# INK-USC/RE-Net

Measured on AMD Instinct MI355X. Metric: RGCN+GRU encoder triples/s at bs=1024 n_hidden=200 (full training step, both directions), higher is better.
Workload: dtype f32; 1 GPU; ICEWS18-shaped synthetic stream (seed 999), n_hidden=200, seq_len=10, batch=1024 per GPU, dropout=0.50, fwd+bwd both directions + clip + Adam; parallelism=dp1, global_batch=1024, nodes=99312, edges=288792

## Files before the change

### include/renet_hip.h

```cpp
#ifndef RENET_HIP_H
#define RENET_HIP_H

#include <stddef.h>
#include <stdint.h>

#ifdef __cplusplus
extern "C" {
#endif

#define RENET_OK 0
#define RENET_ERR_BADARG (-1)
#define RENET_ERR_UNSUPPORTED (-2)
#define RENET_ERR_WORKSPACE (-3)

#define RENET_ABI_VERSION 1
int renet_version(void);

int renet_gather_rows(const float* table, const int32_t* idx, int n, int D, float* out, void* stream);
int renet_segment_add(const float* src, const int32_t* order, const int32_t* seg_ptr,
                      const int32_t* seg_target, int U, int D, float* dst, void* stream);
int renet_segment_add2(const float* src0, const float* src1, const int32_t* order, const int32_t* seg_ptr,
                       const int32_t* seg_target, int U, int D, float* dst0, float* dst1, void* stream);

int renet_rgcn_gather(const float* x, int D, const int32_t* row_ptr, const int32_t* col,
                      const int32_t* etype, const float* scale, const float* W, int T, int type_shift,
                      int transpose_w, const float* addend, float drop_p, uint64_t seed, int relu,
                      float* out, int N, const int32_t* heavy_rows, int n_heavy, int heavy_thresh,
                      int src_limit, int addend_rows, void* stream);

int renet_rgcn_gather_items(const float* x, int D, const int32_t* it_src, const int32_t* it_type,
                            const int32_t* grp_ptr, int n_groups, const int32_t* row_ptr, const int32_t* col,
                            const int32_t* etype, const float* scale, const float* W, int T, int type_shift,
                            int transpose_w, const float* addend, float drop_p, uint64_t seed, int relu,
                            float* out, int N, const int32_t* heavy_rows, int n_heavy, int src_limit,
                            int addend_rows, int pruned, void* stream);

int renet_rgcn_gather_items_table(const float* table, int table_rows, int D, const int32_t* it_src_t,
                                  const int32_t* it_type_t, const int32_t* grp_ptr, int n_groups,
                                  const int32_t* row_ptr, const int32_t* col_t, const int32_t* etype,
                                  const int32_t* row_map, const float* scale, const float* W, int T, int type_shift,
                                  const float* addend_table, float drop_p, uint64_t seed, int relu, float* out, int N,
                                  const int32_t* heavy_rows, int n_heavy, void* stream);

int renet_rgcn_gather_items_bf16(const float* x, int D, const int32_t* it_src, const int32_t* it_type,
                                 const int32_t* grp_ptr, int n_groups, const int32_t* row_ptr, const int32_t* col,
                                 const int32_t* etype, const float* scale, const void* W_bf16, int w_ld, int T,
                                 int type_shift, int transpose_w, const float* addend, float drop_p, uint64_t seed,
                                 int relu, float* out, int N, const int32_t* heavy_rows, int n_heavy, int src_limit,
                                 int addend_rows, int pruned, void* stream);
int renet_rgcn_gather_items_table_bf16(const void* table_bf16, int table_ld, int table_rows, int D,
                                       const int32_t* it_src_t, const int32_t* it_type_t, const int32_t* grp_ptr,
                                       int n_groups, const int32_t* row_ptr, const int32_t* col_t, const int32_t* etype,
                                       const int32_t* row_map, const float* scale, const void* W_bf16, int w_ld, int T,
                                       int type_shift, const float* addend_table, float drop_p, uint64_t seed, int relu,
                                       float* out, int N, const int32_t* heavy_rows, int n_heavy, void* stream);
int renet_compose_table_items(const int32_t* row_map, const int32_t* it_src, const int32_t* it_type, int n_items,
                              const int32_t* col, const int32_t* e_src, int E, int32_t* it_src_t,
                              int32_t* it_type_t, int32_t* col_t, int32_t* e_src_t, void* stream);

int renet_rgcn_bwd_prep(const float* g_out, const float* out, const float* norm, int relu,
                        float drop_p, uint64_t seed, int N, int D, float* gn, float* g_loop,
                        void* stream);
int renet_rgcn_bwd_prep_bounds(const float* g_out, const float* out, const float* norm, int relu,
                               float drop_p, uint64_t seed, int N, int D, float* gn, float* g_loop,
                               float* bound_part, void* stream);

size_t renet_rgcn_bwd_w_workspace(int n_chunks, int D);
int renet_rgcn_bwd_w(const float* x, const float* gn, const int32_t* e_src, const int32_t* e_dst,
                     const int32_t* chunk_ptr, const int32_t* chunk_type, int n_chunks,
                     const int32_t* type_chunk_ptr, int T, int type_shift, int D, float* dW, float beta,
                     float* workspace, size_t workspace_bytes, void* stream);
int renet_rgcn_bwd_w64(const float* x, const float* gn, const int32_t* e_src, const int32_t* e_dst,
                       const int32_t* chunk_ptr, const int32_t* chunk_type, int n_chunks,
                       const int32_t* type_chunk_ptr, int T, int type_shift, int D, float* dW, float beta,
                       float* workspace, size_t workspace_bytes, void* stream);

size_t renet_gemm_workspace(int M, int N, int split_k);
int renet_gemm_f32(int ta, int tb, int M, int N, int K, float alpha, const float* A, int lda,
                   const float* B, int ldb, float beta, float* C, int ldc, const float* bias,
                   int split_k, float* workspace, size_t workspace_bytes, void* stream);

int renet_gemm_f32_split(int ta, int tb, int M, int N, int K, float alpha, const float* A, int lda,
                         const float* B, int ldb, float beta, float* C, int ldc, const float* bias,
                         int split_k, float* workspace, size_t workspace_bytes, void* stream);

int renet_gemm_split_plan(int ta, int tb, int M, int N, int K, const float* A, int lda, const float* B, int ldb,
                          int split_k, int* plan);

int renet_maxabs_blocks(int rows, int cols, int ld);
int renet_maxabs_partials(const float* x, int rows, int cols, int ld, float* part, void* stream);
int renet_maxabs_partials_multi(const void* jobs, int n_jobs, void* stream);
int renet_gemm_f32_h3(int ta, int tb, int M, int N, int K, float alpha, const float* A, int lda, const float* B,
                      int ldb, float beta, float* C, int ldc, const float* bias, int split_k, float* workspace,
                      size_t workspace_bytes, const float* maxA, int nA, const float* maxB, int nB, void* stream);

int renet_gemm_bf16(int ta, int tb, int M, int N, int K, float alpha, const float* A, int lda,
                    const float* B, int ldb, float beta, float* C, int ldc, const float* bias,
                    int split_k, float* workspace, size_t workspace_bytes, void* stream);

size_t renet_bf16_bytes(int R, int C);
int renet_pack_bf16(const float* X, int R, int C, int ldx, void* out, void* stream);
int renet_gemm_bf16s(int a_tr, int b_tr, int M, int N, int K, float alpha, const void* Ap, int lda, const void* Bp,
                     int ldb, float beta, float* C, int ldc, const float* bias, int split_k, float* workspace,
                     size_t workspace_bytes, void* stream);
int renet_bf16_zero_padding(void* P, int rows, int C, int ld, int rows_alloc, void* stream);
int renet_seq_assemble_fwd_bf16(const float* h2, const float* ent, const float* rel, const float* glob,
                                const int32_t* subj_row, const int32_t* row_ent, const int32_t* row_rel,
                                const int32_t* glob_row, int S, int D, float drop_p, uint64_t seed_x,
                                uint64_t seed_xr, void* X, int ldx, void* Xr, int ldxr, int rows_alloc,
                                void* stream);
int renet_softmax_ce_bf16(const float* logits, const int32_t* target, int B, int C, int ld, float grad_scale,
                          float* row_loss, void* dlogits_bf16, int ld16, int rows16, void* stream);
int renet_gru_bwd_layouts_bf16out(int n, const float* const* dh_last, const int32_t* const* step_off, const int* L,
                                  int H, const float* const* Whh, const float* const* saved, void* const* dGi16,
                                  void* const* dGh16, int out_ld, float* workspace, size_t workspace_bytes,
                                  void* stream);
int renet_colsum_bf16(const void* X, int M, int N, int ldx, float* out, float beta, float* workspace,
                      size_t workspace_bytes, void* stream);
int renet_scale_bf16_by_device_scalar(void* x, size_t n, const float* scale, void* stream);

size_t renet_planes_elems(int R, int C);
int renet_pack_planes(const float* X, int R, int C, int ldx, int ones_col, void* out, void* stream);
int renet_gemm_planes(int a_tr, int b_tr, int M, int N, int K, float alpha, const float* alpha_dev, const void* Ap,
                      int lda, size_t a_plane, const void* Bp, int ldb, size_t b_plane, float beta, float* C, int ldc,
                      const float* bias, float* col_out, int split_k, float* workspace, size_t workspace_bytes,
                      void* stream);
int renet_softmax_ce_planes(const float* logits, const int32_t* target, int B, int C, int ld, float grad_scale,
                            float* row_loss, void* dl_planes, size_t plane, int ld16, int rows16, void* stream);

size_t renet_colsum_workspace(int M, int N);
int renet_colsum(const float* X, int M, int N, int ldx, float* out, float beta, float* workspace,
                 size_t workspace_bytes, void* stream);

int renet_scale_by_device_scalar(float* x, size_t n, const float* scale, void* stream);
int renet_scale_by_device_scalar_bound(float* x, size_t n, const float* scale, float bound_in, float* bound_out,
                                       void* stream);

int renet_seq_assemble_fwd(const float* h2, const float* ent, const float* rel, const float* glob,
                           const int32_t* subj_row, const int32_t* row_ent, const int32_t* row_rel,
                           const int32_t* glob_row, int S, int D, float drop_p, uint64_t seed_x,
                           uint64_t seed_xr, float* X, float* Xr, void* stream);
int renet_bound_parts(size_t total4);
int renet_seq_assemble_fwd_bounds(const float* h2, const float* ent, const float* rel, const float* glob,
                                  const int32_t* subj_row, const int32_t* row_ent, const int32_t* row_rel,
                                  const int32_t* glob_row, int S, int D, float drop_p, uint64_t seed_x,
                                  uint64_t seed_xr, float* X, float* Xr, float* partX, float* partXr, void* stream);
int renet_seq_assemble_bwd(const float* dX, const float* dXr, const int32_t* step_off, int L, int S,
                           int B, int D, float drop_p, uint64_t seed_x, uint64_t seed_xr, float* dRows,
                           float* dEntSeq, float* dRelSeq, void* stream);

size_t renet_gru_workspace(int B, int H);
int renet_gru_fwd(const float* Gi, const int32_t* step_off, int L, int H, const float* Whh,
                  const float* bhh, float* h_last, int out_rows, float* saved, float* workspace,
                  size_t workspace_bytes, void* stream);
int renet_gru_bwd(const float* dh_last, const int32_t* step_off, int L, int H, const float* Whh,
                  const float* saved, float* dGi, float* dGh, float* workspace,
                  size_t workspace_bytes, void* stream);
int renet_gru_fwd_multi(int n, const float* const* Gi, const int32_t* step_off, int L, int H,
                        const float* const* Whh, const float* const* bhh, float* const* h_last, int out_rows,
                        float* const* saved, float* workspace, size_t workspace_bytes, void* stream);
int renet_gru_bwd_multi(int n, const float* const* dh_last, const int32_t* step_off, int L, int H,
                        const float* const* Whh, const float* const* saved, float* const* dGi,
                        float* const* dGh, float* workspace, size_t workspace_bytes, void* stream);
int renet_gru_fwd_layouts(int n, const float* const* Gi, const int32_t* const* step_off, const int* L, int H,
                          const float* const* Whh, const float* const* bhh, float* const* h_last,
                          const int* out_rows, float* const* saved, float* workspace, size_t workspace_bytes,
                          void* stream);
int renet_gru_bwd_layouts(int n, const float* const* dh_last, const int32_t* const* step_off, const int* L, int H,
                          const float* const* Whh, const float* const* saved, float* const* dGi,
                          float* const* dGh, float* workspace, size_t workspace_bytes, void* stream);
int renet_gru_bound_parts(int max_rows);
int renet_gru_bwd_layouts_bounds(int n, const float* const* dh_last, const int32_t* const* step_off, const int* L, int H,
                                 const float* const* Whh, const float* const* saved, float* const* dGi,
                                 float* const* dGh, float* const* bounds, float* workspace, size_t workspace_bytes,
                                 void* stream);
int renet_gru_fwd_layouts_f32(int n, const float* const* Gi, const int32_t* const* step_off, const int* L, int H,
                              const float* const* Whh, const float* const* bhh, float* const* h_last,
                              const int* out_rows, float* const* saved, float* workspace, size_t workspace_bytes,
                              void* stream);
int renet_gru_bwd_layouts_f32(int n, const float* const* dh_last, const int32_t* const* step_off, const int* L, int H,
                              const float* const* Whh, const float* const* saved, float* const* dGi,
                              float* const* dGh, float* workspace, size_t workspace_bytes, void* stream);
int renet_gru_fwd_layouts_bf16(int n, const float* const* Gi, const int32_t* const* step_off, const int* L, int H,
                               const float* const* Whh, const float* const* bhh, float* const* h_last,
                               const int* out_rows, float* const* saved, float* workspace, size_t workspace_bytes,
                               void* stream);
int renet_gru_bwd_layouts_bf16(int n, const float* const* dh_last, const int32_t* const* step_off, const int* L, int H,
                               const float* const* Whh, const float* const* saved, float* const* dGi,
                               float* const* dGh, float* workspace, size_t workspace_bytes, void* stream);

int renet_concat3_fwd(const float* a, const int32_t* ia, const float* hmid, const float* c,
                      const int32_t* ic, int B, int D, float drop_p, uint64_t seed, float* feat,
                      void* stream);
int renet_concat3_fwd_bounds(const float* a, const int32_t* ia, const float* hmid, const float* c,
                             const int32_t* ic, int B, int D, float drop_p, uint64_t seed, float* feat,
                             float* bound_part, void* stream);
int renet_concat3_bwd(const float* dfeat, int B, int D, int parts, float drop_p, uint64_t seed,
                      float* da_rows, float* dhmid, float* dc_rows, void* stream);
int renet_dropout(const float* x, size_t n, float drop_p, uint64_t seed, float* y, void* stream);
int renet_softmax_ce(const float* logits, const int32_t* target, int B, int C, int ld,
                     float grad_scale, float* row_loss, float* dlogits, void* stream);

int renet_segment_pool_fwd(const float* h, const int32_t* seg_ptr, int G, int D, int is_max,
                           float* out, int32_t* argmax, void* stream);
int renet_segment_pool_bwd(const float* dout, const int32_t* seg_ptr, const int32_t* argmax, int G,
                           int D, int is_max, int N, float* dh, void* stream);

int renet_nbr_pool_fwd(const float* E, const float* R, const float* P, const float* q, const float* v,
                       const int32_t* nbr, const int32_t* seg_ptr, const int32_t* seg_ptr_host, const int32_t* seg_s,
                       const int32_t* seg_r, const int32_t* seg_q, const int32_t* out_row, int S, int D, int attn,
                       float* out, float* stats, float* w, void* stream);
int renet_nbr_pool_bwd(const float* dOut, const float* out, const float* E, const float* P, const float* q,
                       const float* v, const float* w, const int32_t* nbr, const int32_t* seg_ptr,
                       const int32_t* seg_ptr_host, const int32_t* seg_q, const int32_t* out_row, int S, int D, int attn,
                       float* cE, float* cP, float* dq_rows, float* dv_rows, float* ds_rows, float* dr_rows,
                       void* stream);

size_t renet_adam_workspace(size_t n);
int renet_adam_step(float* p, float* g, float* m, float* v, size_t n, float lr, float beta1, float beta2,
                    float eps, float weight_decay, float max_norm, int step, int zero_grad, float* workspace,
                    size_t workspace_bytes, float* grad_norm_out, void* stream);
int renet_adam_step_scaled(float* p, float* g, float* m, float* v, size_t n, float lr, float beta1, float beta2,
                           float eps, float weight_decay, float max_norm, float grad_scale, int step,
                           int zero_grad, float* workspace, size_t workspace_bytes, float* grad_norm_out,
                           void* stream);

int renet_sumsq_partials(const float* g, size_t n, float* partial, int n_slots, void* stream);
int renet_adam_step_presummed(float* p, float* g, float* m, float* v, size_t n, float lr, float beta1, float beta2,
                              float eps, float weight_decay, float max_norm, float grad_scale, int step, int zero_grad,
                              const float* partial, int n_partial, float* grad_norm_out, void* stream);

int renet_joint_softmax(float* logits, int ld, int n, int R, int N, const float* logits_r, int ld_r,
                        const float* prob_e, void* stream);
size_t renet_topk_workspace(int n);
int renet_topk_positive(const float* x, size_t ldx, int n, int M, int k, float* out_val, int64_t* out_idx,
                        void* workspace, size_t workspace_bytes, void* stream);

int renet_rank_rows(const float* scores, int ld, int n, int C, const int32_t* label, const int32_t* filt_ptr,
                    const int32_t* filt_col, int filtered, int32_t* greater, int32_t* equal, float* row_loss,
                    void* stream);

int renet_rank_rows3(const float* scores, int ld, int n, int C, const int32_t* label, const int32_t* cols_a,
                     const int32_t* start_a, const int32_t* count_a, int len_a, const int32_t* cols_t,
                     const int32_t* start_t, const int32_t* count_t, int len_t, int32_t* counts, float* row_loss,
                     void* stream);

typedef struct {
    const int32_t *q_s, *q_r, *q_o;
    const int32_t* h_first[2];
    const int32_t* h_count[2];
    const int32_t* snap_t[2];
    const int32_t* snap_ptr[2];
    const int32_t* nbr_o[2];
    const int32_t* times;
    const int32_t* trip_ptr;
    const int32_t *trip_s, *trip_r, *trip_o;
    const int32_t* glob_times;
    int T, n_glob, n_facts, num_ent, num_rels;
} RenetStoreDev;

typedef struct {
    int32_t *node_ent, *node_slot, *row_ptr, *col, *etype;
    float* norm;
    int32_t *heavy_rows, *e_src, *e_dst, *chunk_ptr, *chunk_type, *type_chunk_ptr;
    int32_t *e_src2, *e_dst2, *chunk_ptr2, *chunk_type2, *type_chunk_ptr2;
    int32_t *it_src, *it_type, *grp_ptr;
    int32_t *subj_row, *row_seq, *row_ent, *row_rel, *glob_row;
    int32_t *s_sorted, *r_sorted, *rel_label, *ent_label, *perm, *step_off;
    int32_t* plan_order[4];
    int32_t* plan_seg[4];
    int32_t* plan_target[4];
    int32_t* counts;
    int cap_nodes, cap_edges;
    int32_t* seg_ptr;
} RenetBatchOut;

enum {
    RENET_BB_NNZ = 0, RENET_BB_S, RENET_BB_L, RENET_BB_TB, RENET_BB_FACTS, RENET_BB_N, RENET_BB_NA, RENET_BB_E2,
    RENET_BB_E, RENET_BB_NHEAVY, RENET_BB_NHEAVY_OUT, RENET_BB_NCHUNKS, RENET_BB_NCHUNKS2, RENET_BB_NITEMS,
    RENET_BB_NGROUPS, RENET_BB_NGROUPS_OUT, RENET_BB_NSEG0, RENET_BB_NSEG1, RENET_BB_NSEG2, RENET_BB_NSEG3,
    RENET_BB_ERR, RENET_BB_EOUT,
    RENET_BB_STEP_OFF = 24,
    RENET_BB_NCOUNTS = 64
};
enum { RENET_BB_ERR_TIME = 1, RENET_BB_ERR_GLOB = 2, RENET_BB_ERR_NODES = 4, RENET_BB_ERR_EDGES = 8 };

size_t renet_build_batch_workspace(const RenetStoreDev* store, int B, int cap_nodes, int cap_edges);
int renet_build_batch_both(const RenetStoreDev* store, const int32_t* idx_dev, int B, int seq_len, int heavy_thresh,
                           int group_budget, int chunk, const RenetBatchOut* out, void* workspace,
                           size_t workspace_bytes, void* stream);

typedef struct {
    const int32_t* node_ptr;
    const int32_t* node_ent_all;
    const int32_t* trip_ptr;
    const int32_t *trip_ls, *trip_r, *trip_lo;
    int T, n_nodes, n_facts, num_ent, num_rels;
} RenetFullStoreDev;

size_t renet_build_full_graphs_workspace(const RenetFullStoreDev* store, int G, int cap_nodes, int cap_edges);
int renet_build_full_graphs(const RenetFullStoreDev* store, const int32_t* tidx_dev, int G, int heavy_thresh,
                            int group_items, int chunk, RenetBatchOut* out, void* workspace, size_t workspace_bytes,
                            void* stream);

typedef struct {
    const int32_t *s, *r, *group;
    const int32_t *h_first, *h_count;
    const int32_t* step_t;
    const int32_t* nbr_ptr;
    const int32_t* nbr_o;
    const int32_t* times;
    const int32_t* trip_ptr;
    const int32_t *trip_s, *trip_r, *trip_o;
    const int32_t* glob_times;
    const int32_t *by_subj, *subj_sorted;
    int n_steps, n_nbr, T, n_glob, n_facts, num_ent, num_rels;
} RenetGroupedStoreDev;

size_t renet_build_batch_grouped_workspace(const RenetGroupedStoreDev* store, int B, int cap_nodes, int cap_edges);
int renet_build_batch_grouped(const RenetGroupedStoreDev* store, const int32_t* idx_dev, int B, int seq_len,
                              int heavy_thresh, int group_budget, int chunk, const RenetBatchOut* out, void* workspace,
                              size_t workspace_bytes, void* stream);

typedef struct { const int32_t *order, *seg_ptr, *target; int num_segments; } RenetSegPlan;
typedef struct {
    int D, num_ent, T, C2;
    float drop_p;
    const float *ent, *rel;
    const float *w1, *loop1, *w2, *loop2;
    const float *wih, *whh, *bih, *bhh;
    const float *wih_r, *whh_r, *bih_r, *bhh_r;
    const float *lin_w, *lin_b;
    const float *linr_w, *linr_b;
    float *g_ent, *g_rel, *g_w1, *g_loop1, *g_w2, *g_loop2, *g_wih, *g_whh, *g_bih, *g_bhh, *g_wih_r, *g_whh_r, *g_bih_r,
          *g_bhh_r, *g_lin_w, *g_lin_b, *g_linr_w, *g_linr_b;
    const float* glob;
    const void* lin_w_planes;
    size_t lin_w_plane;
    int lin_w_ld;
} RenetStepModel;
typedef struct {
    int N, E, nA, S, B, L, n_items;
    int n_groups, n_groups_out, n_heavy, n_heavy_out, n_chunks, n_chunks2;
    const int32_t* step_off_host;
    const int32_t *node_ent, *row_ptr, *col, *etype;
    const float* norm;
    const int32_t *it_src, *it_type, *grp_ptr, *heavy_rows, *heavy_rows_out;
    const int32_t *it_src_t, *it_type_t, *col_t, *e_src_t;
    const int32_t *e_src, *e_dst, *chunk_ptr, *chunk_type, *type_chunk_ptr;
    const int32_t *e_src2, *e_dst2, *chunk_ptr2, *chunk_type2, *type_chunk_ptr2;
    const int32_t *subj_row, *row_ent, *row_rel, *glob_row, *step_off;
    const int32_t *s_idx, *r_idx, *ent_label, *rel_label;
    RenetSegPlan plan_node_ent, plan_subj_row, plan_s, plan_r;
} RenetStepBatch;
typedef struct {
    uint64_t seed_rgcn1, seed_rgcn2, seed_x, seed_xr, seed_head1, seed_head2;
    float scale_ent, scale_rel;
    void* workspace;
    size_t workspace_bytes;
    void *stream, *side_stream;
} RenetStepRun;
size_t renet_step_workspace(const RenetStepModel* m, const RenetStepBatch* b);
int renet_step_forward(const RenetStepModel* m, const RenetStepBatch* b, const RenetStepRun* r, float* row_loss,
                       int* n_launches);
int renet_step_backward(const RenetStepModel* m, const RenetStepBatch* b, const RenetStepRun* r, const float* g,
                        int defer_side, void* ev_head_done, void* ev_gru_done, int* n_launches);
int renet_add_inplace(float* x, const float* y, size_t n, void* stream);
int renet_zero(float* x, size_t n, void* stream);

int64_t renet_host_filter_edges(const int64_t* trip_ptr, const int64_t* trip_s, const int64_t* trip_r,
                                const int64_t* trip_o, const int64_t* ti, int64_t Tb, int64_t num_ent,
                                const int64_t* keys, const int32_t* new_id, int64_t N, int32_t* table,
                                int64_t* out_ls, int64_t* out_lo, int64_t* out_rr);
int64_t renet_host_filter_edges_sparse(const int64_t* trip_ptr, const int64_t* trip_s, const int64_t* trip_r,
                                       const int64_t* trip_o, const int64_t* by_subj,
                                       const int64_t* subj_sorted, const int64_t* ti, int64_t Tb,
                                       int64_t num_ent, const int64_t* keys, const int32_t* new_id, int64_t N,
                                       int32_t* table, int64_t* out_ls, int64_t* out_lo, int64_t* out_rr);
int64_t renet_host_type_chunks(int64_t E, const int64_t* src, const int64_t* dst, const int64_t* et, int64_t T,
                               int64_t chunk, int64_t n_out, int32_t* e_src, int32_t* e_dst,
                               int32_t* type_chunk_ptr, int32_t* chunk_type, int32_t* chunk_ptr,
                               int64_t* n_chunks);
int64_t renet_host_node_sets(int64_t S, const int64_t* slot_k, const int64_t* subj_ent, const int64_t* nbr_begin,
                             const int64_t* nbr_cnt, const int64_t* nbr_o, int64_t Tb, int64_t num_ent,
                             int32_t* table, int64_t* keys, int64_t* subj_pos, int64_t* new_id,
                             int32_t* node_ent, int64_t* node_slot, int64_t* n_a);
void renet_host_edge_layouts(int64_t n, int64_t E, const int64_t* src, const int64_t* dst, const int64_t* et,
                             int64_t T, int64_t chunk, int64_t heavy, int32_t* col, int32_t* etype,
                             int32_t* row_ptr, float* norm, int32_t* heavy_rows, int64_t* n_heavy,
                             int32_t* e_src, int32_t* e_dst, int32_t* type_chunk_ptr, int32_t* chunk_type,
                             int32_t* chunk_ptr, int64_t* n_chunks);
int64_t renet_host_segplan(const int64_t* idx, int64_t n, int64_t bound, int32_t* order, int32_t* seg_ptr,
                           int32_t* target);
int64_t renet_host_gather_items(int64_t N, const int32_t* row_ptr, const int32_t* col, const int32_t* etype,
                                int64_t heavy, int64_t budget, int64_t n_out, int32_t* it_src, int32_t* it_type,
                                int32_t* grp_ptr, int64_t* n_items, int64_t* n_groups_out);

#ifdef __cplusplus
}
#endif
#endif
```

### re-net_amd/csrc/gru.hip

```cpp
#include "gru_common.h"

namespace {

bool use_f32() {
    static const bool v = renet_env_is("RENET_GEMM", "f32");
    return v;
}

bool use_persistent() { return !renet_env_is("RENET_GRU", "steps"); }

bool fill_offsets(const int32_t* step_off, int L, StepOff& so, int& B) {
    if (L < 1 || L > MAXL || !step_off) return false;
    for (int j = 0; j <= L; ++j) so.off[j] = step_off[j];
    for (int j = L + 1; j <= MAXL; ++j) so.off[j] = step_off[L];
    B = step_off[1] - step_off[0];
    for (int j = 1; j < L; ++j)
        if (step_off[j + 1] - step_off[j] > step_off[j] - step_off[j - 1]) return false;
    return B >= 0;
}

inline size_t align256(size_t x) { return (x + 255) & ~(size_t)255; }
inline int nub(int H) { return (H + 15) / 16; }
inline size_t fwd_plane_bytes(int H) { return (size_t)nub(H) * ((H + 31) / 32) * 9 * 1024; }
inline size_t bwd_t_bytes(int H) { return align256((size_t)3 * H * H * sizeof(float)); }
inline size_t bwd_plane_bytes(int H) { return (size_t)nub(H) * ((3 * H + 31) / 32) * 3 * 1024; }

size_t slice_bytes(int B, int H) {
    size_t m = fwd_plane_bytes(H);
    if (bwd_t_bytes(H) > m) m = bwd_t_bytes(H);
    if (bwd_plane_bytes(H) > m) m = bwd_plane_bytes(H);
    m = align256(m);
    if (B > 0) {
        const size_t rp = (size_t)rows_pad_of(B);
        m += align256((size_t)2 * 3 * rp * kp_of(3 * H) * sizeof(__bf16)) + align256(rp * H * sizeof(float));
    }
    return m;
}

int make_layouts(int n, const int32_t* const* step_off, const int* Ls, const int* rows_in, bool fwd, Layouts& ly,
                 int* B_of) {
    if (n < 1 || n > MAXP) return RENET_ERR_BADARG;
    const int32_t* seen[MAXLAY] = {nullptr, nullptr};
    int nl = 0;
    for (int i = 0; i < MAXLAY; ++i) {
        ly.L[i] = 0; ly.rows[i] = 0;
        for (int j = 0; j <= MAXL; ++j) ly.so[i].off[j] = 0;
    }
    for (int k = 0; k < MAXP; ++k) ly.lay_of[k] = 0;
    static const int rot_mod = renet_env_int("RENET_GRU_ROT", 0, 0, 0x7fffffff);
    ly.rot_mod = rot_mod;
    for (int k = 0; k < n; ++k) {
        int l = -1;
        for (int i = 0; i < nl; ++i)
            if (seen[i] == step_off[k] && ly.L[i] == Ls[k]) l = i;
        if (l < 0) {
            if (nl == MAXLAY) return RENET_ERR_BADARG;
            l = nl++;
            seen[l] = step_off[k];
            ly.L[l] = Ls[k];
            int B = 0;
            if (Ls[k] > 0 && !fill_offsets(step_off[k], Ls[k], ly.so[l], B)) return RENET_ERR_BADARG;
            ly.rows[l] = fwd ? 0 : B;
        }
        const int B = ly.L[l] > 0 ? ly.so[l].off[1] - ly.so[l].off[0] : 0;
        if (fwd) {
            if (rows_in[k] < B) return RENET_ERR_BADARG;
            if (ly.rows[l] != 0 && ly.rows[l] != rows_in[k]) return RENET_ERR_BADARG;
            ly.rows[l] = rows_in[k];
        }
        ly.lay_of[k] = l;
        B_of[k] = B;
    }
    return RENET_OK;
}

StepState carve_state(char* slice, int H, int Bmax, size_t kp) {
    StepState t;
    const size_t rp = (size_t)rows_pad_of(Bmax);
    char* base = slice + align256(slice_bytes(0, H));
    t.plane_stride = rp * kp;
    t.A[0] = reinterpret_cast<__bf16*>(base);
    t.A[1] = t.A[0] + 3 * t.plane_stride;
    t.dh = reinterpret_cast<float*>(base + align256((size_t)2 * 3 * rp * kp_of(3 * H) * sizeof(__bf16)));
    return t;
}

int plane_slot(int k, const float* const* W) {
    for (int i = 0; i < k; ++i)
        if (W[i] == W[k]) return i;
    return k;
}

int max_batch(int n, const int* B_of) {
    int Bmax = 0;
    for (int k = 0; k < n; ++k) Bmax = B_of[k] > Bmax ? B_of[k] : Bmax;
    return Bmax;
}

int gru_fwd_impl(int npl, int n, const float* const* Gi, const int32_t* const* step_off, const int* L, int H,
                 const float* const* Whh, const float* const* bhh, float* const* h_last, const int* out_rows,
                 float* const* saved, float* workspace, size_t workspace_bytes, void* stream) {
    Layouts ly;
    int B_of[MAXP];
    const int e0 = make_layouts(n, step_off, L, out_rows, true, ly, B_of);
    if (e0 != RENET_OK) return e0;
    if (max_rows(ly) == 0) return RENET_OK;
    if (!renet_dim_ok(H) || (npl == 1 && H == 300)) return RENET_ERR_UNSUPPORTED;
    hipStream_t st = (hipStream_t)stream;
    if (npl == 0 || (use_f32() && npl == 3)) {
        FwdProbs ps;
        for (int i = 0; i < MAXP; ++i) {
            const int k = i < n ? i : 0;
            ps.p[i] = {Gi[k], Whh[k], bhh[k], h_last[k], saved[k]};
        }
        return renet_gru_f32_fwd(H, &ps, n, &ly, st);
    }
    const bool steps = npl == 3 && !use_persistent();
    const int Bmax = max_batch(n, B_of);
    const size_t per = slice_bytes(steps ? Bmax : 0, H);
    if (!workspace || workspace_bytes < (size_t)n * per) return RENET_ERR_WORKSPACE;
    char* ws = reinterpret_cast<char*>(workspace);
    FwdProbsB ps;
    for (int i = 0; i < MAXP; ++i) {
        const int k = i < n ? i : 0;
        const int slot = plane_slot(k, Whh);
        bf16x8* planes = reinterpret_cast<bf16x8*>(ws + (size_t)slot * per);
        if (i < n && slot == k) {
            const int e = renet_gru_split_frag(Whh[k], H, H, 3, (size_t)H * H, (size_t)H, 1, planes, st, npl);
            if (e != RENET_OK) return e;
        }
        ps.p[i] = {Gi[k], planes, bhh[k], h_last[k], saved[k]};
    }
    if (steps) {
        StepState stt[MAXP];
        for (int i = 0; i < n; ++i) stt[i] = carve_state(ws + (size_t)i * per, H, Bmax, kp_of(H));
        return renet_gru_steps_fwd(H, n, &ps, &ly, stt, Bmax, st);
    }
    return renet_gru_planes_fwd(H, npl, &ps, n, &ly, st);
}

int gru_bwd_impl(int npl, int n, const float* const* dh_last, const int32_t* const* step_off, const int* L, int H,
                 const float* const* Whh, const float* const* saved, float* const* dGi, float* const* dGh,
                 float* workspace, size_t workspace_bytes, void* stream, int out_ld = 0,
                 float* const* bounds = nullptr) {
    Layouts ly;
    int B_of[MAXP];
    const int e0 = make_layouts(n, step_off, L, nullptr, false, ly, B_of);
    if (e0 != RENET_OK) return e0;
    if (max_rows(ly) == 0) return RENET_OK;
    if (!renet_dim_ok(H) || (npl == 1 && H == 300)) return RENET_ERR_UNSUPPORTED;
    hipStream_t st = (hipStream_t)stream;
    const bool f32 = npl == 0 || (use_f32() && npl == 3);
    const bool steps = npl == 3 && !f32 && !use_persistent();
    if (bounds && (f32 || steps || npl != 3)) return RENET_ERR_UNSUPPORTED;
    const int Bmax = max_batch(n, B_of);
    const size_t per = slice_bytes(steps ? Bmax : 0, H);
    if (!workspace || workspace_bytes < (size_t)n * per) return RENET_ERR_WORKSPACE;
    char* ws = reinterpret_cast<char*>(workspace);
    char* wt[MAXP];
    for (int i = 0; i < MAXP; ++i) {
        const int k = i < n ? i : 0;
        const int slot = plane_slot(k, Whh);
        wt[i] = ws + (size_t)slot * per;
        if (i < n && slot == k) {
            const int e = f32 ? renet_gru_transpose(Whh[k], 3 * H, H, reinterpret_cast<float*>(wt[i]), st)
                              : renet_gru_split_frag(Whh[k], H, 3 * H, 1, 0, 1, (size_t)H, wt[i], st, npl);
            if (e != RENET_OK) return e;
        }
    }
    if (f32) {
        BwdProbs ps;
        for (int i = 0; i < MAXP; ++i) {
            const int k = i < n ? i : 0;
            ps.p[i] = {dh_last[k], reinterpret_cast<float*>(wt[i]), saved[k], dGi[k], dGh[k]};
        }
        return renet_gru_f32_bwd(H, &ps, n, &ly, st);
    }
    BwdProbsB pb;
    for (int i = 0; i < MAXP; ++i) {
        const int k = i < n ? i : 0;
        pb.p[i] = {dh_last[k], reinterpret_cast<bf16x8*>(wt[i]), saved[k], dGi[k], dGh[k], out_ld, bounds ? bounds[k] : nullptr};
    }
    if (steps) {
        StepState stt[MAXP];
        for (int i = 0; i < n; ++i) stt[i] = carve_state(ws + (size_t)i * per, H, Bmax, kp_of(3 * H));
        return renet_gru_steps_bwd(H, n, &pb, &ly, stt, B_of, Bmax, st);
    }
    return renet_gru_planes_bwd(H, npl, out_ld > 0, &pb, n, &ly, st);
}

}

extern "C" {

size_t renet_gru_workspace(int B, int H) { return slice_bytes(B, H); }

#define GRU_FWD_PARAMS                                                                                                \
    int n, const float* const* Gi, const int32_t* const* step_off, const int* L, int H, const float* const* Whh,      \
    const float* const* bhh, float* const* h_last, const int* out_rows, float* const* saved, float* workspace,        \
    size_t workspace_bytes, void* stream
#define GRU_FWD_ARGS n, Gi, step_off, L, H, Whh, bhh, h_last, out_rows, saved, workspace, workspace_bytes, stream
int renet_gru_fwd_layouts(GRU_FWD_PARAMS) { return gru_fwd_impl(3, GRU_FWD_ARGS); }
int renet_gru_fwd_layouts_f32(GRU_FWD_PARAMS) { return gru_fwd_impl(0, GRU_FWD_ARGS); }
int renet_gru_fwd_layouts_bf16(GRU_FWD_PARAMS) { return gru_fwd_impl(1, GRU_FWD_ARGS); }

#define GRU_BWD_PARAMS                                                                                                \
    int n, const float* const* dh_last, const int32_t* const* step_off, const int* L, int H, const float* const* Whh, \
    const float* const* saved, float* const* dGi, float* const* dGh, float* workspace, size_t workspace_bytes,        \
    void* stream
#define GRU_BWD_ARGS n, dh_last, step_off, L, H, Whh, saved, dGi, dGh, workspace, workspace_bytes, stream
int renet_gru_bwd_layouts(GRU_BWD_PARAMS) { return gru_bwd_impl(3, GRU_BWD_ARGS); }
int renet_gru_bwd_layouts_f32(GRU_BWD_PARAMS) { return gru_bwd_impl(0, GRU_BWD_ARGS); }
int renet_gru_bwd_layouts_bf16(GRU_BWD_PARAMS) { return gru_bwd_impl(1, GRU_BWD_ARGS); }

int renet_gru_bound_parts(int max_rows) { return max(1, (max_rows + MT - 1) / MT); }

int renet_gru_bwd_layouts_bounds(int n, const float* const* dh_last, const int32_t* const* step_off, const int* L, int H,
                                 const float* const* Whh, const float* const* saved, float* const* dGi,
                                 float* const* dGh, float* const* bounds, float* workspace, size_t workspace_bytes,
                                 void* stream) {
    if (!bounds) return RENET_ERR_BADARG;
    return gru_bwd_impl(3, n, dh_last, step_off, L, H, Whh, saved, dGi, dGh, workspace, workspace_bytes, stream, 0,
                        bounds);
}

int renet_gru_bwd_layouts_bf16out(int n, const float* const* dh_last, const int32_t* const* step_off, const int* L,
                                  int H, const float* const* Whh, const float* const* saved, void* const* dGi16,
                                  void* const* dGh16, int out_ld, float* workspace, size_t workspace_bytes,
                                  void* stream) {
    if (out_ld < 3 * H) return RENET_ERR_BADARG;
    return gru_bwd_impl(1, n, dh_last, step_off, L, H, Whh, saved, reinterpret_cast<float* const*>(dGi16),
                        reinterpret_cast<float* const*>(dGh16), workspace, workspace_bytes, stream, out_ld);
}

int renet_gru_fwd_multi(int n, const float* const* Gi, const int32_t* step_off, int L, int H,
                        const float* const* Whh, const float* const* bhh, float* const* h_last, int out_rows,
                        float* const* saved, float* workspace, size_t workspace_bytes, void* stream) {
    if (n < 1 || n > MAXP) return RENET_ERR_BADARG;
    const int32_t* so[MAXP];
    int Ls[MAXP], rows[MAXP];
    for (int k = 0; k < n; ++k) { so[k] = step_off; Ls[k] = L; rows[k] = out_rows; }
    return renet_gru_fwd_layouts(n, Gi, so, Ls, H, Whh, bhh, h_last, rows, saved, workspace, workspace_bytes, stream);
}

int renet_gru_fwd(const float* Gi, const int32_t* step_off, int L, int H, const float* Whh,
                  const float* bhh, float* h_last, int out_rows, float* saved, float* workspace,
                  size_t workspace_bytes, void* stream) {
    return renet_gru_fwd_multi(1, &Gi, step_off, L, H, &Whh, &bhh, &h_last, out_rows, &saved, workspace,
                               workspace_bytes, stream);
}

int renet_gru_bwd_multi(int n, const float* const* dh_last, const int32_t* step_off, int L, int H,
                        const float* const* Whh, const float* const* saved, float* const* dGi,
                        float* const* dGh, float* workspace, size_t workspace_bytes, void* stream) {
    if (n < 1 || n > MAXP) return RENET_ERR_BADARG;
    const int32_t* so[MAXP];
    int Ls[MAXP];
    for (int k = 0; k < n; ++k) { so[k] = step_off; Ls[k] = L; }
    return renet_gru_bwd_layouts(n, dh_last, so, Ls, H, Whh, saved, dGi, dGh, workspace, workspace_bytes, stream);
}

int renet_gru_bwd(const float* dh_last, const int32_t* step_off, int L, int H, const float* Whh,
                  const float* saved, float* dGi, float* dGh, float* workspace,
                  size_t workspace_bytes, void* stream) {
    return renet_gru_bwd_multi(1, &dh_last, step_off, L, H, &Whh, &saved, &dGi, &dGh, workspace,
                               workspace_bytes, stream);
}

}
```

### re-net_amd/csrc/step.cpp

```cpp
#include <hip/hip_runtime.h>
#include <algorithm>
#include <cstdint>
#include <cstdlib>
#include <vector>
#include "../../include/renet_hip.h"

namespace {

int auto_split_k(int m, int n, int k) {
    const long tiles = (long)((m + 127) / 128) * ((n + 127) / 128);
    const int ktiles = (k + 31) / 32;
    if (tiles >= 256 || ktiles < 8) return 1;
    const int smax = std::max(1, std::min(128, ktiles / 4));
    const double per_slice = (double)m * (double)n * 2.7e-6;
    int best = 1;
    double best_t = -1.0;
    for (int s = 1; s <= smax; ++s) {
        const long rounds = (tiles * s + 511) / 512;
        const double t = (double)rounds * ((double)ktiles / (double)s + 6.0) + (s > 1 ? per_slice * s : 0.0);
        if (best_t < 0.0 || t < best_t - 1e-9) { best = s; best_t = t; }
    }
    return best;
}

int auto_split_k_planes(int m, int n, int k) {
    const long tiles = (long)((m + 255) / 256) * ((n + 127) / 128);
    const int ktiles = (k + 31) / 32;
    if (tiles >= 128 || ktiles < 8) return 1;
    const int smax = std::max(1, std::min(64, ktiles / 4));
    const double per_slice = (double)m * (double)n * 2.7e-6;
    int best = 1;
    double best_t = -1.0;
    for (int s = 1; s <= smax; ++s) {
        const long rounds = (tiles * s + 255) / 256;
        const double t = (double)rounds * ((double)ktiles / (double)s + 6.0) + (s > 1 ? per_slice * s : 0.0);
        if (best_t < 0.0 || t < best_t - 1e-9) { best = s; best_t = t; }
    }
    return best;
}

inline size_t up(size_t x) { return (x + 255) & ~(size_t)255; }
inline size_t fbytes(size_t rows, size_t cols) { return up(rows * cols * sizeof(float)); }

struct Lay {
    size_t out1, out2, X, Xr, sv0, sv1, feat1, feat2, dl1, dl2, featp1;
    size_t ew, gi0, gi1, hs0, hs1, logits, featp;
    size_t dfeat1, dfeat2, da1, da2, dh1, dh2, dc1, dgi0, dgi1, dgh0, dgh1, dX, dXr, d_rows, d_ent_seq, d_rel_seq, d_h2, gn2,
        gl2, dhN, gn1, gl1, dh1N, gs;
    size_t gru_ws, gemm_ws_main, gemm_ws_side, bwdw_ws, colsum_ws;
    size_t gru_ws_bytes, gemm_ws_bytes, bwdw_ws_bytes, colsum_ws_bytes;
    size_t dl_plane, dl_ld, dl_rows, featp_plane, featp_ld, featp1_plane, featp1_ld, logits_ld;
    size_t total;
};

bool use_planes(const RenetStepModel& m) { return m.lin_w_planes != nullptr; }

Lay layout(const RenetStepModel& m, const RenetStepBatch& b) {
    Lay L{};
    size_t o = 0;
    auto take = [&](size_t bytes) { const size_t at = o; o += up(bytes); return at; };
    const size_t D = m.D, N = b.N, nA = b.nA, S = b.S, B = b.B, NE = m.num_ent, C2 = m.C2;
    const bool pl = use_planes(m);
    L.out1 = take(fbytes(N, D));
    L.out2 = take(fbytes(nA, D));
    L.X = take(fbytes(S, 4 * D));
    L.Xr = take(fbytes(S, 3 * D));
    L.sv0 = take(fbytes(S, 5 * D));
    L.sv1 = take(fbytes(S, 5 * D));
    L.feat1 = take(fbytes(B, 3 * D));
    L.feat2 = take(fbytes(B, 2 * D));
    L.dl2 = take(fbytes(B, C2));
    if (pl) {
        L.dl_rows = (B + 255) & ~(size_t)255;
        L.dl_ld = (NE + 255) & ~(size_t)255;
        L.dl_plane = L.dl_rows * L.dl_ld;
        L.dl1 = take(3 * L.dl_plane * 2);
        L.featp_ld = (3 * D + 255) & ~(size_t)255;
        L.featp_plane = L.dl_rows * L.featp_ld;
        L.featp1_ld = (3 * D + 1 + 255) & ~(size_t)255;
        L.featp1_plane = L.dl_rows * L.featp1_ld;
        L.featp1 = take(3 * L.featp1_plane * 2);
        L.logits_ld = (NE + 3) & ~(size_t)3;
        L.logits = take(fbytes(B, L.logits_ld));
    } else {
        L.dl1 = take(fbytes(B, NE));
        L.logits_ld = NE;
    }
    L.ew = take(fbytes(NE, D));
    L.gi0 = take(fbytes(S, 3 * D));
    L.gi1 = take(fbytes(S, 3 * D));
    L.hs0 = take(fbytes(B, D));
    L.hs1 = take(fbytes(B, D));
    L.dfeat1 = take(fbytes(B, 3 * D));
    L.dfeat2 = take(fbytes(B, 2 * D));
    L.da1 = take(fbytes(B, D));
    L.da2 = take(fbytes(B, D));
    L.dh1 = take(fbytes(B, D));
    L.dh2 = take(fbytes(B, D));
    L.dc1 = take(fbytes(B, D));
    L.dgi0 = take(fbytes(S, 3 * D));
    L.dgi1 = take(fbytes(S, 3 * D));
    L.dgh0 = take(fbytes(S, 3 * D));
    L.dgh1 = take(fbytes(S, 3 * D));
    L.dX = take(fbytes(S, 4 * D));
    L.dXr = take(fbytes(S, 3 * D));
    L.d_rows = take(fbytes(S, D));
    L.d_ent_seq = take(fbytes(B, D));
    L.d_rel_seq = take(fbytes(B, D));
    L.d_h2 = take(fbytes(nA, D));
    L.gn2 = take(fbytes(nA, D));
    L.gl2 = take(fbytes(nA, D));
    L.dhN = take(fbytes(N, D));
    L.gn1 = take(fbytes(N, D));
    L.gl1 = take(fbytes(N, D));
    L.dh1N = take(fbytes(N, D));
    L.gs = take(fbytes(NE, D));
    const int bmax = b.L > 0 ? b.step_off_host[1] - b.step_off_host[0] : 0;
    L.gru_ws_bytes = 2 * renet_gru_workspace(bmax, m.D);
    L.gru_ws = take(std::max<size_t>(L.gru_ws_bytes, 4));
    size_t need = 4;
    auto g_ = [&](int mm, int nn, int kk) { need = std::max(need, renet_gemm_workspace(mm, nn, auto_split_k(mm, nn, kk))); };
    const int Di = m.D, Si = b.S, Bi = b.B, NEi = m.num_ent, nAi = b.nA, C2i = m.C2;
    g_(NEi, Di, Di); g_(nAi, Di, Di); g_(Si, 3 * Di, 4 * Di); g_(Si, 3 * Di, 3 * Di); g_(Bi, NEi, 3 * Di); g_(Bi, C2i, 2 * Di);
    g_(Bi, 3 * Di, NEi); g_(NEi, 3 * Di, Bi); g_(Bi, 2 * Di, C2i); g_(C2i, 2 * Di, Bi);
    g_(3 * Di, 4 * Di, Si); g_(3 * Di, 3 * Di, Si); g_(3 * Di, Di, Si); g_(Si, 3 * Di, 3 * Di); g_(Si, 2 * Di, 3 * Di);
    g_(Di, Di, nAi); g_(Di, Di, NEi);
    if (pl) {
        need = std::max(need, renet_gemm_workspace(Bi, 3 * Di, auto_split_k_planes(Bi, 3 * Di, NEi)));
        need = std::max(need, renet_gemm_workspace(NEi, 3 * Di + 1, auto_split_k_planes(NEi, 3 * Di + 1, Bi)));
        need = std::max(need, renet_gemm_workspace(Bi, NEi, auto_split_k_planes(Bi, NEi, 3 * Di)));
    }
    L.gemm_ws_bytes = need;
    L.gemm_ws_main = take(need);
    L.gemm_ws_side = take(need);
    L.bwdw_ws_bytes = std::max<size_t>(renet_rgcn_bwd_w_workspace(std::max(b.n_chunks, b.n_chunks2), m.D), 4);
    L.bwdw_ws = take(L.bwdw_ws_bytes);
    size_t cs = 4;
    cs = std::max(cs, renet_colsum_workspace(Bi, NEi));
    cs = std::max(cs, renet_colsum_workspace(Bi, C2i));
    cs = std::max(cs, renet_colsum_workspace(Si, 3 * Di));
    L.colsum_ws_bytes = cs;
    L.colsum_ws = take(cs);
    L.total = o;
    return L;
}

bool args_ok(const RenetStepModel* m, const RenetStepBatch* b) {
    if (!m || !b) return false;
    if (!(m->D == 100 || m->D == 200 || m->D == 300 || m->D == 400) || m->num_ent < 1 || m->T < 2 || m->C2 < 1) return false;
    if (b->N < 1 || b->nA < 1 || b->nA > b->N || b->S < 1 || b->B < 1 || b->L < 1 || !b->step_off_host) return false;
    const size_t big = (size_t)std::max(b->N, m->num_ent) * m->D * 4;
    return big < ((size_t)1 << 31);
}

hipEvent_t step_event(int i) {
    thread_local std::vector<hipEvent_t> ev;
    while ((int)ev.size() <= i) {
        hipEvent_t e = nullptr;
        if (hipEventCreateWithFlags(&e, hipEventDisableTiming) != hipSuccess) return nullptr;
        ev.push_back(e);
    }
    return ev[i];
}

struct Streams {
    hipStream_t main, side;
    int next_ev = 0, rc = 0;
    bool two() const { return side != main; }
    void order(hipStream_t first, hipStream_t then) {
        if (!two() || rc) return;
        hipEvent_t e = step_event(next_ev++ & 7);
        if (!e) { rc = (int)hipErrorOutOfMemory; return; }
        hipError_t x = hipEventRecord(e, first);
        if (x == hipSuccess) x = hipStreamWaitEvent(then, e, 0);
        if (x != hipSuccess) rc = (int)x;
    }
    void fork() { order(main, side); }
    void join() { order(side, main); }
};

#define CK(call)                      \
    do {                              \
        const int rc__ = (call);      \
        ++launches;                   \
        if (rc__ != 0) return rc__;   \
    } while (0)

int gemm(hipStream_t st, float* ws, size_t ws_bytes, int ta, int tb, int M, int N, int K, const float* A, int lda, const float* B,
         int ldb, float beta, float* C, int ldc, const float* bias) {
    const int sk = auto_split_k(M, N, K);
    return renet_gemm_f32_split(ta, tb, M, N, K, 1.f, A, lda, B, ldb, beta, C, ldc, bias, sk, sk > 1 ? ws : nullptr,
                                sk > 1 ? ws_bytes : 0, st);
}

}

extern "C" {

size_t renet_step_workspace(const RenetStepModel* m, const RenetStepBatch* b) {
    if (!args_ok(m, b)) return 0;
    return layout(*m, *b).total;
}

int renet_step_forward(const RenetStepModel* mp, const RenetStepBatch* bp, const RenetStepRun* r, float* row_loss,
                       int* n_launches) {
    if (!args_ok(mp, bp) || !r || !r->workspace || !row_loss) return RENET_ERR_BADARG;
    const RenetStepModel& m = *mp;
    const RenetStepBatch& b = *bp;
    const Lay L = layout(m, b);
    if (r->workspace_bytes < L.total) return RENET_ERR_WORKSPACE;
    char* W = (char*)r->workspace;
    auto F = [&](size_t off) { return (float*)(W + off); };
    Streams s{(hipStream_t)r->stream, (hipStream_t)(r->side_stream ? r->side_stream : r->stream)};
    int launches = 0;
    const int D = m.D, N = b.N, nA = b.nA, S = b.S, B = b.B, NE = m.num_ent, T = m.T;
    const float p = m.drop_p;
    const bool pruned = nA < N;
    float* wsm = F(L.gemm_ws_main);
    float* wss = F(L.gemm_ws_side);

    CK(gemm(s.main, wsm, L.gemm_ws_bytes, 0, 0, NE, D, D, m.ent, D, m.loop1, D, 0.f, F(L.ew), D, nullptr));
    CK(renet_rgcn_gather_items_table(m.ent, NE, D, b.it_src_t, b.it_type_t, b.grp_ptr, b.n_groups, b.row_ptr, b.col_t, b.etype,
                                     b.node_ent, b.norm, m.w1, T, 0, F(L.ew), p, r->seed_rgcn1, 1, F(L.out1), N,
                                     b.n_heavy ? b.heavy_rows : nullptr, b.n_heavy, s.main));
    CK(gemm(s.main, wsm, L.gemm_ws_bytes, 0, 0, nA, D, D, F(L.out1), D, m.loop2, D, 0.f, F(L.out2), D, nullptr));
    CK(renet_rgcn_gather_items(F(L.out1), D, b.it_src, b.it_type, b.grp_ptr, pruned ? b.n_groups_out : b.n_groups, b.row_ptr,
                               b.col, b.etype, b.norm, m.w2, T, 0, 0, F(L.out2), p, r->seed_rgcn2, 0, F(L.out2), nA,
                               pruned ? (b.n_heavy_out ? b.heavy_rows_out : nullptr) : (b.n_heavy ? b.heavy_rows : nullptr),
                               pruned ? b.n_heavy_out : b.n_heavy, 0, 0, pruned ? 1 : 0, s.main));
    CK(renet_seq_assemble_fwd(F(L.out2), m.ent, m.rel, m.glob, b.subj_row, b.row_ent, b.row_rel, b.glob_row, S, D, p, r->seed_x,
                              r->seed_xr, F(L.X), F(L.Xr), s.main));
    s.fork();
    CK(gemm(s.side, wss, L.gemm_ws_bytes, 0, 1, S, 3 * D, 3 * D, F(L.Xr), 3 * D, m.wih_r, 3 * D, 0.f, F(L.gi1), 3 * D, m.bih_r));
    CK(gemm(s.main, wsm, L.gemm_ws_bytes, 0, 1, S, 3 * D, 4 * D, F(L.X), 4 * D, m.wih, 4 * D, 0.f, F(L.gi0), 3 * D, m.bih));
    s.join();
    {
        const float* gi[2] = {F(L.gi0), F(L.gi1)};
        const int32_t* so[2] = {b.step_off_host, b.step_off_host};
        const int ls[2] = {b.L, b.L};
        const float* whh[2] = {m.whh, m.whh_r};
        const float* bhh[2] = {m.bhh, m.bhh_r};
        float* hl[2] = {F(L.hs0), F(L.hs1)};
        const int bmax = b.step_off_host[1] - b.step_off_host[0];
        const int rows[2] = {std::max(B, bmax), std::max(B, bmax)};
        float* sv[2] = {F(L.sv0), F(L.sv1)};
        if (rows[0] != B) return RENET_ERR_BADARG;
        CK(renet_gru_fwd_layouts(2, gi, so, ls, D, whh, bhh, hl, rows, sv, F(L.gru_ws), L.gru_ws_bytes, s.main));
    }
    s.fork();
    CK(renet_concat3_fwd(m.ent, b.s_idx, F(L.hs1), nullptr, nullptr, B, D, p, r->seed_head2, F(L.feat2), s.side));
    CK(gemm(s.side, wss, L.gemm_ws_bytes, 0, 1, B, m.C2, 2 * D, F(L.feat2), 2 * D, m.linr_w, 2 * D, 0.f, F(L.dl2), m.C2, m.linr_b));
    CK(renet_softmax_ce(F(L.dl2), b.rel_label, B, m.C2, m.C2, r->scale_rel, row_loss + B, F(L.dl2), s.side));
    CK(renet_concat3_fwd(m.ent, b.s_idx, F(L.hs0), m.rel, b.r_idx, B, D, p, r->seed_head1, F(L.feat1), s.main));
    if (use_planes(m)) {
        CK(renet_pack_planes(F(L.feat1), B, 3 * D, 3 * D, 1, W + L.featp1, s.main));
        const int sk = auto_split_k_planes(B, NE, 3 * D);
        CK(renet_gemm_planes(0, 0, B, NE, 3 * D, 1.f, nullptr, W + L.featp1, (int)L.featp1_ld, L.featp1_plane, m.lin_w_planes,
                             m.lin_w_ld, m.lin_w_plane, 0.f, F(L.logits), (int)L.logits_ld, m.lin_b, nullptr, sk,
                             sk > 1 ? wsm : nullptr, sk > 1 ? L.gemm_ws_bytes : 0, s.main));
        CK(renet_softmax_ce_planes(F(L.logits), b.ent_label, B, NE, (int)L.logits_ld, r->scale_ent, row_loss, W + L.dl1, L.dl_plane,
                                   (int)L.dl_ld, (int)L.dl_rows, s.main));
    } else {
        CK(gemm(s.main, wsm, L.gemm_ws_bytes, 0, 1, B, NE, 3 * D, F(L.feat1), 3 * D, m.lin_w, 3 * D, 0.f, F(L.dl1), NE, m.lin_b));
        CK(renet_softmax_ce(F(L.dl1), b.ent_label, B, NE, NE, r->scale_ent, row_loss, F(L.dl1), s.main));
    }
    s.join();
    if (n_launches) *n_launches = launches;
    return s.rc;
}

int renet_step_backward(const RenetStepModel* mp, const RenetStepBatch* bp, const RenetStepRun* r, const float* g,
                        int defer_side, void* ev_head_done, void* ev_gru_done, int* n_launches) {
    if (!args_ok(mp, bp) || !r || !r->workspace || !g) return RENET_ERR_BADARG;
    const RenetStepModel& m = *mp;
    const RenetStepBatch& b = *bp;
    const Lay L = layout(m, b);
    if (r->workspace_bytes < L.total) return RENET_ERR_WORKSPACE;
    char* W = (char*)r->workspace;
    auto F = [&](size_t off) { return (float*)(W + off); };
    Streams s{(hipStream_t)r->stream, (hipStream_t)(r->side_stream ? r->side_stream : r->stream)};
    int launches = 0;
    const int D = m.D, N = b.N, nA = b.nA, S = b.S, B = b.B, NE = m.num_ent, T = m.T, C2 = m.C2;
    const float p = m.drop_p;
    const bool pruned = nA < N;
    const bool pl = use_planes(m);
    float* wsm = F(L.gemm_ws_main);
    float* wss = F(L.gemm_ws_side);
    float* csw = L.colsum_ws_bytes > 4 ? F(L.colsum_ws) : nullptr;
    auto colsum = [&](const float* X, int M_, int N_, float* out, hipStream_t st) {
        const size_t need = renet_colsum_workspace(M_, N_);
        return renet_colsum(X, M_, N_, N_, out, 1.f, need ? csw : nullptr, need, st);
    };

    if (!pl) CK(renet_scale_by_device_scalar(F(L.dl1), (size_t)B * NE, g, s.main));
    s.fork();
    CK(renet_scale_by_device_scalar(F(L.dl2), (size_t)B * C2, g, s.side));
    CK(gemm(s.side, wss, L.gemm_ws_bytes, 0, 0, B, 2 * D, C2, F(L.dl2), C2, m.linr_w, 2 * D, 0.f, F(L.dfeat2), 2 * D, nullptr));
    CK(gemm(s.side, wss, L.gemm_ws_bytes, 1, 0, C2, 2 * D, B, F(L.dl2), C2, F(L.feat2), 2 * D, 1.f, m.g_linr_w, 2 * D, nullptr));
    CK(colsum(F(L.dl2), B, C2, m.g_linr_b, s.side));
    CK(renet_concat3_bwd(F(L.dfeat2), B, D, 2, p, r->seed_head2, F(L.da2), F(L.dh2), nullptr, s.side));
    if (pl) {
        const int sk1 = auto_split_k_planes(B, 3 * D, NE);
        CK(renet_gemm_planes(0, 1, B, 3 * D, NE, 1.f, g, W + L.dl1, (int)L.dl_ld, L.dl_plane, m.lin_w_planes, m.lin_w_ld,
                             m.lin_w_plane, 0.f, F(L.dfeat1), 3 * D, nullptr, nullptr, sk1, sk1 > 1 ? wsm : nullptr,
                             sk1 > 1 ? L.gemm_ws_bytes : 0, s.main));
        const int sk2 = auto_split_k_planes(NE, 3 * D + 1, B);
        CK(renet_gemm_planes(1, 1, NE, 3 * D + 1, B, 1.f, g, W + L.dl1, (int)L.dl_ld, L.dl_plane, W + L.featp1, (int)L.featp1_ld,
                             L.featp1_plane, 1.f, m.g_lin_w, 3 * D, nullptr, m.g_lin_b, sk2, sk2 > 1 ? wsm : nullptr,
                             sk2 > 1 ? L.gemm_ws_bytes : 0, s.main));
    } else {
        CK(colsum(F(L.dl1), B, NE, m.g_lin_b, s.side));
        CK(gemm(s.main, wsm, L.gemm_ws_bytes, 0, 0, B, 3 * D, NE, F(L.dl1), NE, m.lin_w, 3 * D, 0.f, F(L.dfeat1), 3 * D, nullptr));
        CK(gemm(s.main, wsm, L.gemm_ws_bytes, 1, 0, NE, 3 * D, B, F(L.dl1), NE, F(L.feat1), 3 * D, 1.f, m.g_lin_w, 3 * D, nullptr));
    }
    CK(renet_concat3_bwd(F(L.dfeat1), B, D, 3, p, r->seed_head1, F(L.da1), F(L.dh1), F(L.dc1), s.main));
    s.join();
    if (ev_head_done) {
        const hipError_t e = hipEventRecord((hipEvent_t)ev_head_done, s.main);
        if (e != hipSuccess) return (int)e;
    }
    CK(renet_add_inplace(F(L.da1), F(L.da2), (size_t)B * D, s.main));
    CK(renet_segment_add(F(L.da1), b.plan_s.order, b.plan_s.seg_ptr, b.plan_s.target, b.plan_s.num_segments, D, m.g_ent, s.main));
    CK(renet_segment_add(F(L.dc1), b.plan_r.order, b.plan_r.seg_ptr, b.plan_r.target, b.plan_r.num_segments, D, m.g_rel, s.main));

    {
        const float* dhl[2] = {F(L.dh1), F(L.dh2)};
        const int32_t* so[2] = {b.step_off_host, b.step_off_host};
        const int ls[2] = {b.L, b.L};
        const float* whh[2] = {m.whh, m.whh_r};
        const float* sv[2] = {F(L.sv0), F(L.sv1)};
        float* dgi[2] = {F(L.dgi0), F(L.dgi1)};
        float* dgh[2] = {F(L.dgh0), F(L.dgh1)};
        CK(renet_gru_bwd_layouts(2, dhl, so, ls, D, whh, sv, dgi, dgh, F(L.gru_ws), L.gru_ws_bytes, s.main));
    }
    auto gru_param_grads = [&]() -> int {
        const float* xs[2] = {F(L.X), F(L.Xr)};
        const int in[2] = {4 * D, 3 * D};
        const size_t dgi[2] = {L.dgi0, L.dgi1}, dgh[2] = {L.dgh0, L.dgh1}, sv[2] = {L.sv0, L.sv1};
        float* gwih[2] = {m.g_wih, m.g_wih_r};
        float* gwhh[2] = {m.g_whh, m.g_whh_r};
        float* gbih[2] = {m.g_bih, m.g_bih_r};
        float* gbhh[2] = {m.g_bhh, m.g_bhh_r};
        for (int k = 0; k < 2; ++k) {
            CK(gemm(s.side, wss, L.gemm_ws_bytes, 1, 0, 3 * D, in[k], S, F(dgi[k]), 3 * D, xs[k], in[k], 1.f, gwih[k], in[k], nullptr));
            CK(gemm(s.side, wss, L.gemm_ws_bytes, 1, 0, 3 * D, D, S, F(dgh[k]), 3 * D, F(sv[k]) + 4 * D, 5 * D, 1.f, gwhh[k], D, nullptr));
            CK(colsum(F(dgi[k]), S, 3 * D, gbih[k], s.side));
            CK(colsum(F(dgh[k]), S, 3 * D, gbhh[k], s.side));
        }
        return 0;
    };
    auto gru_done = [&]() -> int {
        if (!ev_gru_done) return 0;
        return (int)hipEventRecord((hipEvent_t)ev_gru_done, s.side);
    };
    {
        s.fork();
        int rc_ = gru_param_grads();
        if (!rc_) rc_ = gru_done();
        if (rc_) return rc_;
    }
    CK(gemm(s.main, wsm, L.gemm_ws_bytes, 0, 0, S, 3 * D, 3 * D, F(L.dgi0), 3 * D, m.wih, 4 * D, 0.f, F(L.dX), 4 * D, nullptr));
    CK(gemm(s.main, wsm, L.gemm_ws_bytes, 0, 0, S, 2 * D, 3 * D, F(L.dgi1), 3 * D, m.wih_r, 3 * D, 0.f, F(L.dXr), 3 * D, nullptr));

    CK(renet_seq_assemble_bwd(F(L.dX), F(L.dXr), b.step_off, b.L, S, B, D, p, r->seed_x, r->seed_xr, F(L.d_rows), F(L.d_ent_seq),
                              F(L.d_rel_seq), s.main));
    CK(renet_zero(F(L.d_h2), (size_t)nA * D, s.main));
    CK(renet_segment_add(F(L.d_rows), b.plan_subj_row.order, b.plan_subj_row.seg_ptr, b.plan_subj_row.target,
                         b.plan_subj_row.num_segments, D, F(L.d_h2), s.main));
    CK(renet_segment_add(F(L.d_ent_seq), b.plan_s.order, b.plan_s.seg_ptr, b.plan_s.target, b.plan_s.num_segments, D, m.g_ent, s.main));
    CK(renet_segment_add(F(L.d_rel_seq), b.plan_r.order, b.plan_r.seg_ptr, b.plan_r.target, b.plan_r.num_segments, D, m.g_rel, s.main));

    const int pair_shift = (T / 2) % T;
    CK(renet_rgcn_bwd_prep(F(L.d_h2), F(L.out2), b.norm, 0, p, r->seed_rgcn2, nA, D, F(L.gn2), F(L.gl2), s.main));
    CK(renet_rgcn_gather_items(F(L.gn2), D, b.it_src, b.it_type, b.grp_ptr, b.n_groups, b.row_ptr, b.col, b.etype, nullptr, m.w2, T,
                               pair_shift, 1, nullptr, 0.f, 0, 0, F(L.dhN), N, b.n_heavy ? b.heavy_rows : nullptr, b.n_heavy,
                               pruned ? nA : 0, 0, pruned ? 1 : 0, s.main));
    CK(gemm(s.main, wsm, L.gemm_ws_bytes, 0, 1, nA, D, D, F(L.gl2), D, m.loop2, D, 1.f, F(L.dhN), D, nullptr));
    s.fork();
    if (pruned)
        CK(renet_rgcn_bwd_w(F(L.out1), F(L.gn2), b.e_src2, b.e_dst2, b.chunk_ptr2, b.chunk_type2, b.n_chunks2, b.type_chunk_ptr2, T,
                            0, D, m.g_w2, 1.f, F(L.bwdw_ws), renet_rgcn_bwd_w_workspace(b.n_chunks2, D), s.side));
    else
        CK(renet_rgcn_bwd_w(F(L.out1), F(L.gn2), b.e_src, b.e_dst, b.chunk_ptr, b.chunk_type, b.n_chunks, b.type_chunk_ptr, T, 0, D,
                            m.g_w2, 1.f, F(L.bwdw_ws), renet_rgcn_bwd_w_workspace(b.n_chunks, D), s.side));
    CK(gemm(s.side, wss, L.gemm_ws_bytes, 1, 0, D, D, nA, F(L.out1), D, F(L.gl2), D, 1.f, m.g_loop2, D, nullptr));

    CK(renet_rgcn_bwd_prep(F(L.dhN), F(L.out1), b.norm, 1, p, r->seed_rgcn1, N, D, F(L.gn1), F(L.gl1), s.main));
    CK(renet_rgcn_gather_items(F(L.gn1), D, b.it_src, b.it_type, b.grp_ptr, b.n_groups, b.row_ptr, b.col, b.etype, nullptr, m.w1, T,
                               pair_shift, 1, nullptr, 0.f, 0, 0, F(L.dh1N), N, b.n_heavy ? b.heavy_rows : nullptr, b.n_heavy, 0, 0,
                               0, s.main));
    s.fork();
    CK(renet_rgcn_bwd_w(m.ent, F(L.gn1), b.e_src_t, b.e_dst, b.chunk_ptr, b.chunk_type, b.n_chunks, b.type_chunk_ptr, T, 0, D,
                        m.g_w1, 1.f, F(L.bwdw_ws), renet_rgcn_bwd_w_workspace(b.n_chunks, D), s.side));
    CK(renet_zero(F(L.gs), (size_t)NE * D, s.main));
    CK(renet_segment_add2(F(L.dh1N), F(L.gl1), b.plan_node_ent.order, b.plan_node_ent.seg_ptr, b.plan_node_ent.target,
                          b.plan_node_ent.num_segments, D, m.g_ent, F(L.gs), s.main));
    CK(gemm(s.main, wsm, L.gemm_ws_bytes, 0, 1, NE, D, D, F(L.gs), D, m.loop1, D, 1.f, m.g_ent, D, nullptr));
    CK(gemm(s.main, wsm, L.gemm_ws_bytes, 1, 0, D, D, NE, m.ent, D, F(L.gs), D, 1.f, m.g_loop1, D, nullptr));
    if (!defer_side) s.join();
    if (n_launches) *n_launches = launches;
    return s.rc;
}

}
```

### re-net_amd/pipeline.py

```python
import multiprocessing as mp
import os

_job = {}


def worker_budget(world=1, cpus=None, cap=24):
    cpus = cpus or os.cpu_count() or 2
    return max(1, min(int(cap), cpus // (2 * max(int(world), 1))))


def _run(step):
    return _job['fn'](step)


class BatchPrefetcher(object):

    def __init__(self, fn, steps, num_workers=None, chunksize=1, threads=False):
        self.fn, self.steps = fn, list(steps)
        self.num_workers = num_workers or max(1, min(32, (os.cpu_count() or 2) // 2))
        self.chunksize = chunksize
        self.threads = threads
        self.pool = None

    def _iter_threads(self):
        from concurrent.futures import ThreadPoolExecutor
        ahead = 2 * self.num_workers
        with ThreadPoolExecutor(self.num_workers) as ex:
            pending = []
            it = iter(self.steps)
            for s in it:
                pending.append(ex.submit(self.fn, s))
                if len(pending) >= ahead:
                    break
            while pending:
                item = pending.pop(0).result()
                nxt = next(it, None)
                if nxt is not None:
                    pending.append(ex.submit(self.fn, nxt))
                yield item

    def __iter__(self):
        if self.num_workers <= 1:
            for s in self.steps:
                yield self.fn(s)
            return
        if self.threads:
            for item in self._iter_threads():
                yield item
            return
        _job['fn'] = self.fn
        ctx = mp.get_context('fork')
        self.pool = ctx.Pool(self.num_workers)
        try:
            for item in self.pool.imap(_run, self.steps, self.chunksize):
                yield item
        finally:
            self.pool.terminate()
            self.pool.join()
            self.pool = None
            _job.pop('fn', None)


class Uploader(object):

    def __init__(self, net):
        import torch
        self.torch = torch
        self.net = net
        self.stream = torch.cuda.Stream()

    def __call__(self, hbatch):
        torch = self.torch
        main = torch.cuda.current_stream()
        with torch.cuda.stream(self.stream):
            prep = self.net.prepare_from_host(hbatch)
        main.wait_stream(self.stream)
        g = prep.g
        ts = [prep.o_idx, prep.s_idx, prep.r_idx]
        if g is not None:
            ts += [g._buf, g.norm, getattr(g, 'glob', None)]
        for pl in (prep.plan_s, prep.plan_r):
            if pl is not None:
                ts += [pl.order, pl.seg_ptr, pl.target]
        for t in ts:
            if t is not None and torch.is_tensor(t) and t.is_cuda:
                t.record_stream(main)
        return prep
```

### re-net_amd/renet_hip.py

```python
import contextlib
import ctypes
import functools
import os
import threading
import weakref

import torch

_HERE = os.path.dirname(os.path.abspath(__file__))
LIB_PATH = os.environ.get('RENET_HIP_LIB', os.path.join(_HERE, 'csrc', 'librenet_hip.so'))

_lib = None

c_int = ctypes.c_int
c_float = ctypes.c_float
c_void_p = ctypes.c_void_p
c_size_t = ctypes.c_size_t
c_u64 = ctypes.c_uint64

_GEMM_ARGS = [c_int, c_int, c_int, c_int, c_int, c_float, c_void_p, c_int, c_void_p, c_int,
              c_float, c_void_p, c_int, c_void_p, c_int, c_void_p, c_size_t, c_void_p]
_RGCN_BWD_W_ARGS = [c_void_p, c_void_p, c_void_p, c_void_p, c_void_p, c_void_p, c_int,
                    c_void_p, c_int, c_int, c_int, c_void_p, c_float, c_void_p, c_size_t, c_void_p]
_GRU_FWD_LAYOUTS_ARGS = [c_int, c_void_p, c_void_p, c_void_p, c_int, c_void_p, c_void_p, c_void_p,
                         c_void_p, c_void_p, c_void_p, c_size_t, c_void_p]
_GRU_BWD_LAYOUTS_ARGS = [c_int, c_void_p, c_void_p, c_void_p, c_int, c_void_p, c_void_p, c_void_p,
                         c_void_p, c_void_p, c_size_t, c_void_p]

_SIGNATURES = {
    'renet_version': (c_int, []),
    'renet_gather_rows': (c_int, [c_void_p, c_void_p, c_int, c_int, c_void_p, c_void_p]),
    'renet_segment_add': (c_int, [c_void_p, c_void_p, c_void_p, c_void_p, c_int, c_int, c_void_p, c_void_p]),
    'renet_segment_add2': (c_int, [c_void_p, c_void_p, c_void_p, c_void_p, c_void_p, c_int, c_int, c_void_p, c_void_p,
                                   c_void_p]),
    'renet_rgcn_gather': (c_int, [c_void_p, c_int, c_void_p, c_void_p, c_void_p, c_void_p, c_void_p, c_int,
                                  c_int, c_int, c_void_p, c_float, c_u64, c_int, c_void_p, c_int, c_void_p,
                                  c_int, c_int, c_int, c_int, c_void_p]),
    'renet_rgcn_gather_items': (c_int, [c_void_p, c_int, c_void_p, c_void_p, c_void_p, c_int, c_void_p, c_void_p,
                                        c_void_p, c_void_p, c_void_p, c_int, c_int, c_int, c_void_p, c_float, c_u64,
                                        c_int, c_void_p, c_int, c_void_p, c_int, c_int, c_int, c_int, c_void_p]),
    'renet_rgcn_gather_items_bf16': (c_int, [c_void_p, c_int, c_void_p, c_void_p, c_void_p, c_int, c_void_p, c_void_p,
                                             c_void_p, c_void_p, c_void_p, c_int, c_int, c_int, c_int, c_void_p,
                                             c_float, c_u64, c_int, c_void_p, c_int, c_void_p, c_int, c_int, c_int,
                                             c_int, c_void_p]),
    'renet_rgcn_gather_items_table_bf16': (c_int, [c_void_p, c_int, c_int, c_int, c_void_p, c_void_p, c_void_p, c_int,
                                                   c_void_p, c_void_p, c_void_p, c_void_p, c_void_p, c_void_p, c_int,
                                                   c_int, c_int, c_void_p, c_float, c_u64, c_int, c_void_p, c_int,
                                                   c_void_p, c_int, c_void_p]),
    'renet_rgcn_gather_items_table': (c_int, [c_void_p, c_int, c_int, c_void_p, c_void_p, c_void_p, c_int, c_void_p,
                                              c_void_p, c_void_p, c_void_p, c_void_p, c_void_p, c_int, c_int, c_void_p,
                                              c_float, c_u64, c_int, c_void_p, c_int, c_void_p, c_int, c_void_p]),
    'renet_compose_table_items': (c_int, [c_void_p, c_void_p, c_void_p, c_int, c_void_p, c_void_p, c_int, c_void_p,
                                          c_void_p, c_void_p, c_void_p, c_void_p]),
    'renet_rgcn_bwd_prep': (c_int, [c_void_p, c_void_p, c_void_p, c_int, c_float, c_u64, c_int, c_int,
                                    c_void_p, c_void_p, c_void_p]),
    'renet_rgcn_bwd_prep_bounds': (c_int, [c_void_p, c_void_p, c_void_p, c_int, c_float, c_u64, c_int, c_int,
                                           c_void_p, c_void_p, c_void_p, c_void_p]),
    'renet_bound_parts': (c_int, [c_size_t]),
    'renet_rgcn_bwd_w_workspace': (c_size_t, [c_int, c_int]),
    'renet_rgcn_bwd_w': (c_int, _RGCN_BWD_W_ARGS),
    'renet_rgcn_bwd_w64': (c_int, _RGCN_BWD_W_ARGS),
    'renet_gemm_workspace': (c_size_t, [c_int, c_int, c_int]),
    'renet_gemm_f32': (c_int, _GEMM_ARGS),
    'renet_gemm_f32_split': (c_int, _GEMM_ARGS),
    'renet_gemm_bf16': (c_int, _GEMM_ARGS),
    'renet_gemm_split_plan': (c_int, [c_int, c_int, c_int, c_int, c_int, c_void_p, c_int, c_void_p, c_int, c_int, c_void_p]),
    'renet_maxabs_blocks': (c_int, [c_int, c_int, c_int]),
    'renet_maxabs_partials_multi': (c_int, [c_void_p, c_int, c_void_p]),
    'renet_maxabs_partials': (c_int, [c_void_p, c_int, c_int, c_int, c_void_p, c_void_p]),
    'renet_gemm_f32_h3': (c_int, [c_int, c_int, c_int, c_int, c_int, c_float, c_void_p, c_int, c_void_p, c_int,
                                  c_float, c_void_p, c_int, c_void_p, c_int, c_void_p, c_size_t, c_void_p, c_int,
                                  c_void_p, c_int, c_void_p]),
    'renet_bf16_bytes': (c_size_t, [c_int, c_int]),
    'renet_pack_bf16': (c_int, [c_void_p, c_int, c_int, c_int, c_void_p, c_void_p]),
    'renet_gemm_bf16s': (c_int, _GEMM_ARGS),
    'renet_bf16_zero_padding': (c_int, [c_void_p, c_int, c_int, c_int, c_int, c_void_p]),
    'renet_seq_assemble_fwd_bf16': (c_int, [c_void_p, c_void_p, c_void_p, c_void_p, c_void_p, c_void_p, c_void_p,
                                            c_void_p, c_int, c_int, c_float, c_u64, c_u64, c_void_p, c_int, c_void_p,
                                            c_int, c_int, c_void_p]),
    'renet_softmax_ce_bf16': (c_int, [c_void_p, c_void_p, c_int, c_int, c_int, c_float, c_void_p, c_void_p, c_int, c_int,
                                      c_void_p]),
    'renet_gru_bwd_layouts_bf16out': (c_int, [c_int, c_void_p, c_void_p, c_void_p, c_int, c_void_p, c_void_p, c_void_p,
                                              c_void_p, c_int, c_void_p, c_size_t, c_void_p]),
    'renet_colsum_bf16': (c_int, [c_void_p, c_int, c_int, c_int, c_void_p, c_float, c_void_p, c_size_t, c_void_p]),
    'renet_scale_bf16_by_device_scalar': (c_int, [c_void_p, c_size_t, c_void_p, c_void_p]),
    'renet_planes_elems': (c_size_t, [c_int, c_int]),
    'renet_pack_planes': (c_int, [c_void_p, c_int, c_int, c_int, c_int, c_void_p, c_void_p]),
    'renet_gemm_planes': (c_int, [c_int, c_int, c_int, c_int, c_int, c_float, c_void_p, c_void_p, c_int, c_size_t,
                                  c_void_p, c_int, c_size_t, c_float, c_void_p, c_int, c_void_p, c_void_p, c_int,
                                  c_void_p, c_size_t, c_void_p]),
    'renet_softmax_ce_planes': (c_int, [c_void_p, c_void_p, c_int, c_int, c_int, c_float, c_void_p, c_void_p, c_size_t,
                                        c_int, c_int, c_void_p]),
    'renet_step_workspace': (c_size_t, [c_void_p, c_void_p]),
    'renet_step_forward': (c_int, [c_void_p, c_void_p, c_void_p, c_void_p, c_void_p]),
    'renet_step_backward': (c_int, [c_void_p, c_void_p, c_void_p, c_void_p, c_int, c_void_p, c_void_p, c_void_p]),
    'renet_add_inplace': (c_int, [c_void_p, c_void_p, c_size_t, c_void_p]),
    'renet_zero': (c_int, [c_void_p, c_size_t, c_void_p]),
    'renet_colsum_workspace': (c_size_t, [c_int, c_int]),
    'renet_colsum': (c_int, [c_void_p, c_int, c_int, c_int, c_void_p, c_float, c_void_p, c_size_t, c_void_p]),
    'renet_scale_by_device_scalar': (c_int, [c_void_p, c_size_t, c_void_p, c_void_p]),
    'renet_scale_by_device_scalar_bound': (c_int, [c_void_p, c_size_t, c_void_p, c_float, c_void_p, c_void_p]),
    'renet_seq_assemble_fwd': (c_int, [c_void_p, c_void_p, c_void_p, c_void_p, c_void_p, c_void_p, c_void_p,
                                       c_void_p, c_int, c_int, c_float, c_u64, c_u64, c_void_p, c_void_p,
                                       c_void_p]),
    'renet_seq_assemble_fwd_bounds': (c_int, [c_void_p, c_void_p, c_void_p, c_void_p, c_void_p, c_void_p, c_void_p,
                                              c_void_p, c_int, c_int, c_float, c_u64, c_u64, c_void_p, c_void_p,
                                              c_void_p, c_void_p, c_void_p]),
    'renet_seq_assemble_bwd': (c_int, [c_void_p, c_void_p, c_void_p, c_int, c_int, c_int, c_int, c_float,
                                       c_u64, c_u64, c_void_p, c_void_p, c_void_p, c_void_p]),
    'renet_gru_workspace': (c_size_t, [c_int, c_int]),
    'renet_gru_fwd': (c_int, [c_void_p, c_void_p, c_int, c_int, c_void_p, c_void_p, c_void_p, c_int, c_void_p,
                              c_void_p, c_size_t, c_void_p]),
    'renet_gru_bwd': (c_int, [c_void_p, c_void_p, c_int, c_int, c_void_p, c_void_p, c_void_p, c_void_p,
                              c_void_p, c_size_t, c_void_p]),
    'renet_gru_fwd_multi': (c_int, [c_int, c_void_p, c_void_p, c_int, c_int, c_void_p, c_void_p, c_void_p,
                                    c_int, c_void_p, c_void_p, c_size_t, c_void_p]),
    'renet_gru_bwd_multi': (c_int, [c_int, c_void_p, c_void_p, c_int, c_int, c_void_p, c_void_p, c_void_p,
                                    c_void_p, c_void_p, c_size_t, c_void_p]),
    'renet_gru_fwd_layouts': (c_int, _GRU_FWD_LAYOUTS_ARGS),
    'renet_gru_bwd_layouts': (c_int, _GRU_BWD_LAYOUTS_ARGS),
    'renet_gru_bound_parts': (c_int, [c_int]),
    'renet_gru_bwd_layouts_bounds': (c_int, [c_int, c_void_p, c_void_p, c_void_p, c_int, c_void_p, c_void_p, c_void_p,
                                             c_void_p, c_void_p, c_void_p, c_size_t, c_void_p]),
    'renet_gru_fwd_layouts_f32': (c_int, _GRU_FWD_LAYOUTS_ARGS),
    'renet_gru_bwd_layouts_f32': (c_int, _GRU_BWD_LAYOUTS_ARGS),
    'renet_gru_fwd_layouts_bf16': (c_int, _GRU_FWD_LAYOUTS_ARGS),
    'renet_gru_bwd_layouts_bf16': (c_int, _GRU_BWD_LAYOUTS_ARGS),
    'renet_concat3_fwd': (c_int, [c_void_p, c_void_p, c_void_p, c_void_p, c_void_p, c_int, c_int, c_float,
                                  c_u64, c_void_p, c_void_p]),
    'renet_concat3_fwd_bounds': (c_int, [c_void_p, c_void_p, c_void_p, c_void_p, c_void_p, c_int, c_int, c_float,
                                         c_u64, c_void_p, c_void_p, c_void_p]),
    'renet_concat3_bwd': (c_int, [c_void_p, c_int, c_int, c_int, c_float, c_u64, c_void_p, c_void_p,
                                  c_void_p, c_void_p]),
    'renet_dropout': (c_int, [c_void_p, c_size_t, c_float, c_u64, c_void_p, c_void_p]),
    'renet_softmax_ce': (c_int, [c_void_p, c_void_p, c_int, c_int, c_int, c_float, c_void_p, c_void_p,
                                 c_void_p]),
    'renet_joint_softmax': (c_int, [c_void_p, c_int, c_int, c_int, c_int, c_void_p, c_int, c_void_p, c_void_p]),
    'renet_rank_rows': (c_int, [c_void_p, c_int, c_int, c_int, c_void_p, c_void_p, c_void_p, c_int, c_void_p, c_void_p,
                                c_void_p, c_void_p]),
    'renet_rank_rows3': (c_int, [c_void_p, c_int, c_int, c_int, c_void_p, c_void_p, c_void_p, c_void_p, c_int, c_void_p,
                                 c_void_p, c_void_p, c_int, c_void_p, c_void_p, c_void_p]),
    'renet_topk_workspace': (c_size_t, [c_int]),
    'renet_topk_positive': (c_int, [c_void_p, c_size_t, c_int, c_int, c_int, c_void_p, c_void_p, c_void_p, c_size_t,
                                    c_void_p]),
    'renet_build_batch_workspace': (c_size_t, [c_void_p, c_int, c_int, c_int]),
    'renet_build_batch_both': (c_int, [c_void_p, c_void_p, c_int, c_int, c_int, c_int, c_int, c_void_p, c_void_p, c_size_t,
                                       c_void_p]),
    'renet_build_full_graphs_workspace': (c_size_t, [c_void_p, c_int, c_int, c_int]),
    'renet_build_full_graphs': (c_int, [c_void_p, c_void_p, c_int, c_int, c_int, c_int, c_void_p, c_void_p, c_size_t,
                                        c_void_p]),
    'renet_build_batch_grouped_workspace': (c_size_t, [c_void_p, c_int, c_int, c_int]),
    'renet_build_batch_grouped': (c_int, [c_void_p, c_void_p, c_int, c_int, c_int, c_int, c_int, c_void_p, c_void_p, c_size_t,
                                          c_void_p]),
    'renet_adam_workspace': (c_size_t, [c_size_t]),
    'renet_adam_step': (c_int, [c_void_p, c_void_p, c_void_p, c_void_p, c_size_t, c_float, c_float, c_float, c_float,
                                c_float, c_float, c_int, c_int, c_void_p, c_size_t, c_void_p, c_void_p]),
    'renet_adam_step_scaled': (c_int, [c_void_p, c_void_p, c_void_p, c_void_p, c_size_t, c_float, c_float, c_float,
                                       c_float, c_float, c_float, c_float, c_int, c_int, c_void_p, c_size_t, c_void_p,
                                       c_void_p]),
    'renet_sumsq_partials': (c_int, [c_void_p, c_size_t, c_void_p, c_int, c_void_p]),
    'renet_adam_step_presummed': (c_int, [c_void_p, c_void_p, c_void_p, c_void_p, c_size_t, c_float, c_float, c_float,
                                          c_float, c_float, c_float, c_float, c_int, c_int, c_void_p, c_int, c_void_p,
                                          c_void_p]),
    'renet_host_filter_edges': (ctypes.c_int64, [c_void_p] * 5 + [ctypes.c_int64, ctypes.c_int64, c_void_p, c_void_p,
                                                 ctypes.c_int64, c_void_p, c_void_p, c_void_p, c_void_p]),
    'renet_host_filter_edges_sparse': (ctypes.c_int64, [c_void_p] * 7 + [ctypes.c_int64, ctypes.c_int64, c_void_p,
                                                        c_void_p, ctypes.c_int64, c_void_p, c_void_p, c_void_p,
                                                        c_void_p]),
    'renet_host_node_sets': (ctypes.c_int64, [ctypes.c_int64] + [c_void_p] * 5 + [ctypes.c_int64, ctypes.c_int64]
                             + [c_void_p] * 7),
    'renet_host_type_chunks': (ctypes.c_int64, [ctypes.c_int64, c_void_p, c_void_p, c_void_p, ctypes.c_int64,
                                                ctypes.c_int64, ctypes.c_int64] + [c_void_p] * 6),
    'renet_host_edge_layouts': (None, [ctypes.c_int64, ctypes.c_int64, c_void_p, c_void_p, c_void_p, ctypes.c_int64,
                                       ctypes.c_int64, ctypes.c_int64] + [c_void_p] * 12),
    'renet_host_segplan': (ctypes.c_int64, [c_void_p, ctypes.c_int64, ctypes.c_int64, c_void_p, c_void_p, c_void_p]),
    'renet_host_gather_items': (ctypes.c_int64, [ctypes.c_int64, c_void_p, c_void_p, c_void_p, ctypes.c_int64,
                                                 ctypes.c_int64, ctypes.c_int64] + [c_void_p] * 5),
    'renet_segment_pool_fwd': (c_int, [c_void_p, c_void_p, c_int, c_int, c_int, c_void_p, c_void_p, c_void_p]),
    'renet_segment_pool_bwd': (c_int, [c_void_p, c_void_p, c_void_p, c_int, c_int, c_int, c_int, c_void_p,
                                       c_void_p]),
    'renet_nbr_pool_fwd': (c_int, [c_void_p] * 12 + [c_int, c_int, c_int, c_void_p, c_void_p, c_void_p, c_void_p]),
    'renet_nbr_pool_bwd': (c_int, [c_void_p] * 12 + [c_int, c_int, c_int] + [c_void_p] * 7),
}

EXPORTS = sorted(_SIGNATURES)


class RenetHipError(RuntimeError):
    pass


class _Bound(object):
    """The bound entry points (attribute per symbol)."""


def _exact_arity(fn, name, n):
    def call(*a):
        if len(a) != n:
            raise RenetHipError('%s takes %d arguments, %d given' % (name, n, len(a)))
        return fn(*a)
    call.__name__ = name
    return call


def lib():
    global _lib
    if _lib is None:
        if not os.path.isfile(LIB_PATH):
            raise RenetHipError('librenet_hip.so not built (%s); run `python re-net_amd/build.py` '
                                '-- there is no fallback path' % LIB_PATH)
        L = ctypes.CDLL(LIB_PATH)
        ns = _Bound()
        for name, (res, args) in _SIGNATURES.items():
            fn = getattr(L, name)
            fn.restype = res
            fn.argtypes = args
            setattr(ns, name, _exact_arity(fn, name, len(args)))
        if ns.renet_version() != 1:
            raise RenetHipError('ABI version mismatch')
        ns._cdll = L
        _lib = ns
    return _lib


def _check(rc, what):
    if rc != 0:
        raise RenetHipError('%s failed with code %d' % (what, rc))


def _dev_ptr(dtype, default_name, t, name=None):
    if t is None:
        return None
    if not (t.is_cuda and t.dtype == dtype and t.is_contiguous()):
        raise RenetHipError('%s must be a contiguous %s device tensor' % (name or default_name, str(dtype)[6:]))
    return t.data_ptr()


_f32 = functools.partial(_dev_ptr, torch.float32, 'tensor')
_i32 = functools.partial(_dev_ptr, torch.int32, 'index')


_raw_stream = getattr(torch._C, '_cuda_getCurrentRawStream', None)


def _stream():
    if _raw_stream is not None:
        return _raw_stream(torch.cuda.current_device())
    return torch.cuda.current_stream().cuda_stream


class KernelTimer(object):

    def __init__(self):
        self.recs = {}

    def begin(self):
        e = torch.cuda.Event(enable_timing=True)
        e.record()
        return e

    def end(self, name, e0, flops=0.0, nbytes=0.0, tag=None):
        e1 = torch.cuda.Event(enable_timing=True)
        e1.record()
        self.recs.setdefault(name, []).append((e0, e1, flops, nbytes, tag))

    def summary(self):
        torch.cuda.synchronize()
        out = {}
        for name, rs in self.recs.items():
            out[name] = {'calls': len(rs), 'ms': sum(r[0].elapsed_time(r[1]) for r in rs),
                         'flops': sum(r[2] for r in rs), 'bytes': sum(r[3] for r in rs)}
        return out

    def by_tag(self, name):
        torch.cuda.synchronize()
        out = {}
        for r in self.recs.get(name, []):
            o = out.setdefault(r[4], {'calls': 0, 'ms': 0.0, 'flops': 0.0})
            o['calls'] += 1
            o['ms'] += r[0].elapsed_time(r[1])
            o['flops'] += r[2]
        return out


_timer = None


def _timed():
    return _timer.begin() if _timer is not None else None


def _timed_end(t0, name, flops=0.0, nbytes=0.0, tag=None):
    if t0 is not None:
        _timer.end(name, t0, flops=flops, nbytes=nbytes, tag=tag)

GLUE = ('softmax_ce_planes', 'gather_rows', 'segment_add', 'segment_add2', 'compose_table_items', 'rgcn_bwd_prep', 'colsum',
        'scale_by_device_scalar', 'seq_assemble_fwd', 'seq_assemble_fwd_bf16', 'softmax_ce_bf16', 'seq_assemble_bwd',
        'concat3_fwd', 'concat3_bwd', 'dropout', 'softmax_ce', 'adam_step', 'segment_pool_fwd', 'segment_pool_bwd',
        'pack_bf16_glue')
_glue_saved = {}


def _timed_glue(name, fn):
    @functools.wraps(fn)
    def call(*a, **k):
        t = _timer
        if t is None:
            return fn(*a, **k)
        e0 = t.begin()
        try:
            return fn(*a, **k)
        finally:
            t.end('glue:' + name, e0)
    return call


def set_timer(t, glue=False):
    global _timer
    _timer = t
    g = globals()
    for name, fn in _glue_saved.items():
        g[name] = fn
    _glue_saved.clear()
    if t is not None and glue:
        for name in GLUE:
            if name in g and callable(g[name]):
                _glue_saved[name] = g[name]
                g[name] = _timed_glue(name, g[name])


def gather_rows(table, idx, out=None):
    n, d = idx.numel(), table.shape[1]
    if out is None:
        out = torch.empty(n, d, device=table.device, dtype=torch.float32)
    _check(lib().renet_gather_rows(_f32(table), _i32(idx), n, d, _f32(out), _stream()), 'gather_rows')
    return out


def segment_add(src, plan, dst):
    _check(lib().renet_segment_add(_f32(src), _i32(plan.order), _i32(plan.seg_ptr), _i32(plan.target),
                                   plan.num_segments, src.shape[1], _f32(dst), _stream()), 'segment_add')
    return dst


def segment_add2(src0, src1, plan, dst0, dst1):
    _check(lib().renet_segment_add2(_f32(src0), _f32(src1), _i32(plan.order), _i32(plan.seg_ptr), _i32(plan.target),
                                    plan.num_segments, src0.shape[1], _f32(dst0), _f32(dst1), _stream()), 'segment_add2')


def _heavy(rows):
    return (_i32(rows), rows.numel()) if rows is not None else (None, 0)


def _gather_timed_end(t0, name, n_edges, n_rows, d, weight, has_addend, x_bytes=4, w_bytes=4):
    if t0 is not None:
        _timed_end(t0, name, nbytes=float(gather_bytes(n_edges, n_rows, d, weight.numel(), has_addend, x_bytes, w_bytes)),
                   tag=float(gather_bytes(n_edges, n_rows, d, weight.numel(), False, x_bytes, w_bytes)))


def rgcn_gather(x, row_ptr, col, etype, scale, weight, type_shift, transpose_w, addend, drop_p, seed,
                relu, out, heavy_rows=None, heavy_thresh=0, src_limit=0, addend_rows=0, n_edges=None):
    d = x.shape[1]
    t0 = _timed()
    _check(lib().renet_rgcn_gather(_f32(x), d, _i32(row_ptr), _i32(col), _i32(etype), _f32(scale),
                                   _f32(weight), weight.shape[0], type_shift, int(transpose_w),
                                   _f32(addend), float(drop_p), int(seed), int(relu), _f32(out),
                                   out.shape[0], *_heavy(heavy_rows), int(heavy_thresh),
                                   int(src_limit), int(addend_rows), _stream()), 'rgcn_gather')
    if t0 is not None:
        e = col.numel() if n_edges is None else int(n_edges)
        _timed_end(t0, 'rgcn_gather' if n_edges is None else 'rgcn_gather_pruned',
                   nbytes=float(gather_bytes(e, out.shape[0], d, weight.numel(), addend is not None)))
    return out


def gather_bytes(n_edges, n_rows, d, weight_numel, has_addend, x_bytes=4, w_bytes=4):
    return (n_edges * (d * x_bytes + 8) + n_rows * (d * 4 + 8) + weight_numel * w_bytes +
            (n_rows * d * 4 if has_addend else 0))


def _item_args(it_src, it_type, g, n_groups, col):
    return (_i32(it_src), _i32(it_type), _i32(g.grp_ptr), int(n_groups), _i32(g.row_ptr), _i32(col), _i32(g.etype))


def rgcn_gather_items(x, g, weight, type_shift, transpose_w, addend, drop_p, seed, relu, out, use_norm=True,
                      pruned=False, src_limit=0, addend_rows=0, w16=None):
    d = x.shape[1]
    n_rows = out.shape[0]
    prefix = n_rows < g.N
    n_groups = g.n_groups_out if prefix else g.n_groups
    heavy = g.heavy_rows_out if prefix else g.heavy_rows
    if max(x.numel(), out.numel()) * 4 >= (1 << 31):
        return rgcn_gather(x, g.row_ptr, g.col, g.etype, g.norm if use_norm else None, weight, type_shift,
                           transpose_w, addend, drop_p, seed, relu, out, heavy, g.heavy_thresh, src_limit,
                           addend_rows, n_edges=g.E_out if pruned else None)
    t0 = _timed()
    head = (_f32(x), d) + _item_args(g.it_src, g.it_type, g, n_groups, g.col) + (_f32(g.norm) if use_norm else None,)
    tail = (weight.shape[0], int(type_shift), int(transpose_w), _f32(addend), float(drop_p), int(seed), int(relu),
            _f32(out), n_rows) + _heavy(heavy) + (int(src_limit), int(addend_rows), int(pruned), _stream())
    if w16 is not None:
        _check(lib().renet_rgcn_gather_items_bf16(*head, w16.p.data_ptr(), w16.p.shape[1], *tail),
               'rgcn_gather_items_bf16')
    else:
        _check(lib().renet_rgcn_gather_items(*head, _f32(weight), *tail), 'rgcn_gather_items')
    _gather_timed_end(t0, 'rgcn_gather_%s_%s' % ('bwdh' if transpose_w else 'fwd', 'pruned' if pruned else 'full'),
                      g.E_out if pruned else g.E, n_rows, d, weight, addend is not None, 4, 2 if w16 is not None else 4)
    return out


def gather_weight_bf16(weight):
    if current_mode() != 'bf16s' or os.environ.get('RENET_BF16_GATHER', '1') == '0':
        return None
    if weight.numel() * 2 >= (1 << 31):
        return None
    return _as_bf16(weight)[0]


def compose_table_items(g):
    ni, e = g.it_src.numel(), g.col.numel()
    buf = torch.empty(2 * ni + 2 * e + 16, device=g.col.device, dtype=torch.int32)
    a0, a1, a2 = (ni + 3) & ~3, 2 * ((ni + 3) & ~3), 2 * ((ni + 3) & ~3) + ((e + 3) & ~3)
    it_src_t, it_type_t, col_t, e_src_t = buf[:ni], buf[a0:a0 + ni], buf[a1:a1 + e], buf[a2:a2 + e]
    _check(lib().renet_compose_table_items(_i32(g.node_ent), _i32(g.it_src), _i32(g.it_type), ni, _i32(g.col),
                                           _i32(g.e_src), e, it_src_t.data_ptr(), it_type_t.data_ptr(),
                                           col_t.data_ptr(), e_src_t.data_ptr(), _stream()), 'compose_table_items')
    return it_src_t, it_type_t, col_t, e_src_t


def rgcn_gather_items_table(table, g, weight, type_shift, addend_table, drop_p, seed, relu, out, table16=None,
                            w16=None):
    d = table.shape[1]
    n_rows = out.shape[0]
    it_src_t, it_type_t, col_t, _ = g.table_items()
    b16 = table16 is not None and w16 is not None
    t0 = _timed()
    items = (table.shape[0], d) + _item_args(it_src_t, it_type_t, g, g.n_groups, col_t) + (_i32(g.node_ent), _f32(g.norm))
    tail = (weight.shape[0], int(type_shift), _f32(addend_table), float(drop_p), int(seed), int(relu), _f32(out),
            n_rows) + _heavy(g.heavy_rows) + (_stream(),)
    if b16:
        _check(lib().renet_rgcn_gather_items_table_bf16(table16.p.data_ptr(), table16.p.shape[1], *items,
                                                        w16.p.data_ptr(), w16.p.shape[1], *tail),
               'rgcn_gather_items_table_bf16')
    else:
        _check(lib().renet_rgcn_gather_items_table(_f32(table), *items, _f32(weight), *tail), 'rgcn_gather_items_table')
    eb = 2 if b16 else 4
    _gather_timed_end(t0, 'rgcn_gather_fwd_full', g.E, n_rows, d, weight, addend_table is not None, eb, eb)
    return out


def rgcn_bwd_prep(g_out, out, norm, relu, drop_p, seed, gn, g_loop):
    n, d = g_out.shape
    args = (_f32(g_out), _f32(out), _f32(norm), int(relu), float(drop_p), int(seed), n, d, _f32(gn), _f32(g_loop))
    if _fused_bounds(g_loop):
        _call_with_bounds('rgcn_bwd_prep_bounds', args, n * (d // 4), (g_loop,))
        return
    _check(lib().renet_rgcn_bwd_prep(*args, _stream()), 'rgcn_bwd_prep')


def rgcn_bwd_w(x, gn, e_src, e_dst, chunk_ptr, chunk_type, n_chunks, type_chunk_ptr, num_types, type_shift,
               dW, beta=0.0):
    d = x.shape[1]
    big = max(x.numel(), gn.numel()) * 4 >= (1 << 31) or os.environ.get('RENET_BWDW_64') == '1'
    nbytes = lib().renet_rgcn_bwd_w_workspace(n_chunks, d)
    ws = torch.empty(max(nbytes // 4, 1), device=x.device, dtype=torch.float32)
    t0 = _timed()
    fn = lib().renet_rgcn_bwd_w64 if big else lib().renet_rgcn_bwd_w
    _check(fn(_f32(x), _f32(gn), _i32(e_src), _i32(e_dst), _i32(chunk_ptr), _i32(chunk_type), n_chunks,
              _i32(type_chunk_ptr), num_types, type_shift, d, _f32(dW), float(beta), ws.data_ptr(), nbytes, _stream()),
           'rgcn_bwd_w')
    _timed_end(t0, 'rgcn_bwd_w', nbytes=float(e_src.numel() * (2 * d * 4 + 8) + dW.numel() * 4))
    return dW


def _ld(t):
    if t.dim() != 2 or t.stride(1) != 1:
        raise RenetHipError('GEMM operands must be 2-D with unit inner stride')
    return t.stride(0)


def gemm_split_plan(ta, tb, m, n, k, lda=None, ldb=None, split_k=1, a_ptr=0, b_ptr=0):
    lda = (m if ta else k) if lda is None else lda
    ldb = (k if tb else n) if ldb is None else ldb
    out = (ctypes.c_int * 8)()
    _check(lib().renet_gemm_split_plan(int(ta), int(tb), m, n, k, a_ptr, lda, b_ptr, ldb, split_k,
                                       ctypes.cast(out, ctypes.c_void_p)), 'renet_gemm_split_plan')
    names = {0: 'fused', 1: 'two_phase_128', 2: 'two_phase_256', 3: 'weight_resident', 4: 'bf16'}
    return {'kernel': names[out[0]], 'raw': bool(out[1]), 'xcd_order': out[2], 'grid': (out[3], out[4], out[5]),
            'split_k': out[6]}


def auto_split_k(m, n, k):
    return _split_k_model(m, n, k, tile_m=128, slots=512, full=256, smax=128)


def _split_k_model(m, n, k, tile_m, slots, full, smax):
    tiles = ((m + tile_m - 1) // tile_m) * ((n + 127) // 128)
    ktiles = (k + 31) // 32
    if tiles >= full or ktiles < 8:
        return 1
    per_slice = m * n * 2.7e-6
    best, best_t = 1, None
    for s in range(1, max(1, min(smax, ktiles // 4)) + 1):
        rounds = (tiles * s + slots - 1) // slots
        t = rounds * (ktiles / float(s) + 6.0) + (per_slice * s if s > 1 else 0.0)
        if best_t is None or t < best_t - 1e-9:
            best, best_t = s, t
    return best


def _gemm_front(what, m, n, k, k2, out, beta, split_k, device, n_out=None, planes=False):
    if k != k2:
        raise RenetHipError('%s inner dimensions differ: %d vs %d' % (what, k, k2))
    if out is None:
        if beta != 0.0:
            raise RenetHipError('beta != 0 needs an output tensor')
        out = torch.empty(m, n if n_out is None else n_out, device=device, dtype=torch.float32)
    if split_k is None:
        split_k = (auto_split_k_planes if planes else auto_split_k)(m, n, k)
    ws, ws_bytes = None, 0
    if split_k > 1:
        ws_bytes = lib().renet_gemm_workspace(m, n, split_k)
        ws = torch.empty(ws_bytes // 4, device=device, dtype=torch.float32)
    return out, split_k, ws, ws_bytes


def _gemm_timed_end(t0, ta, tb, m, n, k, split_k):
    if t0 is not None:
        _timed_end(t0, 'gemm_f32', flops=2.0 * m * n * k, tag=(int(ta), int(tb), m, n, k, split_k))


GEMM_MODE = os.environ.get('RENET_GEMM', 'bf16x6')

_mode_override = threading.local()
_PER_MODEL_MODES = ('bf16x6', 'f16x3', 'f32')


def current_mode():
    return getattr(_mode_override, 'mode', None) or GEMM_MODE


@contextlib.contextmanager
def gemm_mode(mode):
    if mode is None or mode == current_mode():
        yield
        return
    if mode not in _PER_MODEL_MODES or GEMM_MODE not in _PER_MODEL_MODES:
        raise RenetHipError('gemm_mode(%r): only %s can be chosen per model, and only in a process whose default is one '
                            'of them (RENET_GEMM=%s)' % (mode, ' / '.join(_PER_MODEL_MODES), GEMM_MODE))
    old = getattr(_mode_override, 'mode', None)
    _mode_override.mode = mode
    try:
        yield
    finally:
        _mode_override.mode = old


class BF16Mat(object):
    __slots__ = ('p', 'R', 'C')

    def __init__(self, p, R, C):
        self.p, self.R, self.C = p, R, C

    @property
    def shape(self):
        return (self.R, self.C)


def bf16_empty(r, c, device):
    return BF16Mat(torch.empty((r + 255) & ~255, (c + 255) & ~255, device=device, dtype=torch.bfloat16), r, c)


def pack_bf16(x):
    if not (x.is_cuda and x.dtype == torch.float32 and x.dim() == 2 and x.stride(1) == 1):
        raise RenetHipError('pack_bf16 needs a 2-D float32 device tensor with unit inner stride')
    r, c = x.shape
    rp, cp = (r + 255) & ~255, (c + 255) & ~255
    p = torch.empty(rp, cp, device=x.device, dtype=torch.bfloat16)
    t0 = _timed()
    _check(lib().renet_pack_bf16(x.data_ptr(), r, c, x.stride(0), p.data_ptr(), _stream()), 'pack_bf16')
    _timed_end(t0, 'pack_bf16', nbytes=float(r * c * 4 + rp * cp * 2))
    return BF16Mat(p, r, c)


class _StreamGuard(object):
    __slots__ = ('stream', 'event')

    def __init__(self, device):
        self.stream = torch.cuda.current_stream(device)
        self.event = torch.cuda.Event()
        self.event.record(self.stream)

    def wait(self, device):
        cur = torch.cuda.current_stream(device)
        if cur != self.stream:
            cur.wait_event(self.event)


class _Weight(object):
    __slots__ = ('shape', 'ref', 'bf16', 'planes', 'maxima')

    def __init__(self):
        self.bf16 = self.planes = self.maxima = None


_weights = {}
_weight_epoch = [0]


def register_weights(tensors):
    for t in tensors:
        if t.dim() == 2 and t.is_contiguous():
            rec = _weights.setdefault(t.data_ptr(), _Weight())
            rec.shape, rec.ref = tuple(t.shape), weakref.ref(t)


def unregister_weights(tensors):
    for t in tensors:
        _weights.pop(t.data_ptr(), None)


def weights_changed():
    _weight_epoch[0] += 1


def _weight_stamp(t):
    return (_weight_epoch[0], t._version)


def _registered(x, whole=False):
    rec = _weights.get(x.data_ptr())
    if rec is None or x.dim() != 2:
        return None
    if whole:
        return rec if tuple(x.shape) == rec.shape and x.is_contiguous() else None
    rows, cols = rec.shape
    return rec if x.stride(1) == 1 and x.stride(0) == cols and x.shape[0] <= rows and x.shape[1] <= cols else None


def _whole(x, rec):
    return torch.as_strided(x, rec.shape, (rec.shape[1], 1))


def _derived(rec, form, x, make, guarded=True):
    ent, stamp = getattr(rec, form), _weight_stamp(x)
    if ent is None or ent[0] != stamp:
        ent = (stamp, make(), _StreamGuard(x.device) if guarded else None)
        setattr(rec, form, ent)
    if ent[2] is not None:
        ent[2].wait(x.device)
    return ent[1]


def _as_bf16(x):
    if isinstance(x, BF16Mat):
        return x, x.R, x.C
    rec = _registered(x)
    if rec is not None:
        return _derived(rec, 'bf16', x, lambda: pack_bf16(_whole(x, rec)), guarded=False), x.shape[0], x.shape[1]
    m = pack_bf16(x)
    return m, m.R, m.C


PLANES = os.environ.get('RENET_PLANES', '1') != '0'
PLANES_MIN_CLASSES = int(os.environ.get('RENET_PLANES_MIN_CLASSES', '2048'))


class PlanesMat(object):
    __slots__ = ('p', 'R', 'C')

    def __init__(self, p, R, C):
        self.p, self.R, self.C = p, R, C

    @property
    def shape(self):
        return (self.R, self.C)

    @property
    def plane(self):
        return self.p.shape[1] * self.p.shape[2]


def planes_to_dense(m):
    rp, cp = m.p.shape[1], m.p.shape[2]
    dev = m.p.device
    r = torch.arange(rp, device=dev).view(-1, 1)
    c = torch.arange(cp, device=dev).view(1, -1)
    i, j, tc = r & 15, c & 15, c >> 4
    idx = ((r >> 4) * (cp // 16) + tc) * 256 + (i ^ ((tc & 1) << 2)) * 16 + ((j >> 3) ^ ((i >> 3) & 1)) * 8 + (j & 7)
    return m.p.reshape(3, -1)[:, idx.reshape(-1)].reshape(3, rp, cp).float()


def planes_empty(r, c, device, zero=False):
    rp, cp = (r + 255) & ~255, (c + 255) & ~255
    mk = torch.zeros if zero else torch.empty
    return PlanesMat(mk(3, rp, cp, device=device, dtype=torch.bfloat16), r, c)


def pack_planes(x, ones_col=False):
    if not (x.is_cuda and x.dtype == torch.float32 and x.dim() == 2 and x.stride(1) == 1):
        raise RenetHipError('pack_planes needs a 2-D float32 device tensor with unit inner stride')
    r, c = x.shape
    m = planes_empty(r, c + (1 if ones_col else 0), x.device)
    t0 = _timed()
    _check(lib().renet_pack_planes(x.data_ptr(), r, c, x.stride(0), int(bool(ones_col)), m.p.data_ptr(), _stream()),
           'pack_planes')
    _timed_end(t0, 'pack_planes', nbytes=float(r * c * 4 + 3 * m.plane * 2))
    return m


def weight_planes(w):
    rec = _registered(w, whole=True)
    return _derived(rec, 'planes', w, lambda: pack_planes(w)) if rec is not None else pack_planes(w)


def note_weight_planes(w, mat):
    rec = _registered(w, whole=True)
    if rec is not None:
        rec.planes = (_weight_stamp(w), mat, _StreamGuard(w.device))


def use_planes(weight, n_classes):
    return (PLANES and current_mode() == 'bf16x6' and weight.is_cuda and n_classes >= PLANES_MIN_CLASSES and
            weight.dim() == 2 and weight.is_contiguous())


def auto_split_k_planes(m, n, k):
    return _split_k_model(m, n, k, tile_m=256, slots=256, full=128, smax=64)


def gemm_planes(a, b, ta=False, tb=False, out=None, bias=None, alpha=1.0, alpha_dev=None, beta=0.0, col_out=None,
                split_k=None):
    if not (isinstance(a, PlanesMat) and isinstance(b, PlanesMat)):
        raise RenetHipError('gemm_planes needs PlanesMat operands')
    m, k = (a.C, a.R) if ta else (a.R, a.C)
    n, k2 = (b.R, b.C) if tb else (b.C, b.R)
    n_main = n - 1 if col_out is not None else n
    out, split_k, ws, ws_bytes = _gemm_front('gemm_planes', m, n, k, k2, out, beta, split_k, a.p.device, n_out=n_main,
                                             planes=True)
    if tuple(out.shape) != (m, n_main):
        raise RenetHipError('gemm_planes: output shape %r, expected %r' % (tuple(out.shape), (m, n_main)))
    if col_out is not None and (col_out.numel() != m or not col_out.is_contiguous()):
        raise RenetHipError('gemm_planes: col_out must be a contiguous vector of M floats')
    t0 = _timed()
    _check(lib().renet_gemm_planes(int(ta), int(not tb), m, n, k, float(alpha), _f32(alpha_dev), a.p.data_ptr(),
                                   a.p.shape[2], a.plane, b.p.data_ptr(), b.p.shape[2], b.plane, float(beta),
                                   out.data_ptr(), _ld(out), _f32(bias), _f32(col_out), split_k, _f32(ws), ws_bytes,
                                   _stream()), 'gemm_planes')
    _gemm_timed_end(t0, ta, tb, m, n_main, k, split_k)
    return out


def softmax_ce_planes(logits, target, grad_scale, row_loss=None):
    b, c = logits.shape
    if row_loss is None:
        row_loss = torch.empty(b, device=logits.device, dtype=torch.float32)
    dl = planes_empty(b, c, logits.device)
    _check(lib().renet_softmax_ce_planes(logits.data_ptr(), _i32(target), b, c, _ld(logits), float(grad_scale),
                                         _f32(row_loss), dl.p.data_ptr(), dl.plane, dl.p.shape[2], dl.p.shape[1],
                                         _stream()), 'softmax_ce_planes')
    return row_loss, dl


class F32Op(object):
    __slots__ = ('t', 'part', 'n')

    def __init__(self, t, part=None, n=0):
        self.t, self.part, self.n = t, part, n

    @property
    def shape(self):
        return self.t.shape

    def bound(self):
        if self.part is None:
            self.part, self.n = _weight_or_measured_max(self.t)
        return self.part, self.n


def is_handle(x):
    return isinstance(x, (BF16Mat, F32Op, PlanesMat))


def maxabs_partials(x):
    if not (x.is_cuda and x.dtype == torch.float32 and x.dim() == 2 and x.stride(1) == 1):
        raise RenetHipError('maxabs_partials needs a 2-D float32 device tensor with unit inner stride')
    rows, cols = x.shape
    n = lib().renet_maxabs_blocks(rows, cols, _ld(x))
    part = torch.empty(n, device=x.device, dtype=torch.float32)
    t0 = _timed()
    _check(lib().renet_maxabs_partials(x.data_ptr(), rows, cols, _ld(x), part.data_ptr(), _stream()),
           'maxabs_partials')
    _timed_end(t0, 'maxabs', nbytes=float(rows * cols * 4))
    return part, n


_weight_jobs = {'key': None, 'table': None, 'parts': {}}


def _measure_all_weights(device):
    live = {p: rec.ref() for p, rec in _weights.items()}
    ptrs = sorted(p for p, t in live.items() if t is not None and t.is_cuda and t.device == device
                  and t.numel() % 4 == 0 and p % 16 == 0 and t.data_ptr() == p)
    key = (tuple(ptrs), str(device))
    if _weight_jobs['key'] != key:
        rows, parts = [], {}
        for p in ptrs:
            shp = _weights[p].shape
            nb = lib().renet_maxabs_blocks(shp[0], shp[1], shp[1])
            part = torch.empty(nb, device=device, dtype=torch.float32)
            parts[p] = (part, nb)
            rows.append([p, shp[0] * shp[1] // 4, part.data_ptr(), nb])
        _weight_jobs.update(key=key, parts=parts,
                            table=torch.tensor(rows, dtype=torch.int64).to(device) if rows else None)
    if _weight_jobs['table'] is None:
        return
    t0 = _timed()
    _check(lib().renet_maxabs_partials_multi(_weight_jobs['table'].data_ptr(), len(ptrs), _stream()),
           'maxabs_partials_multi')
    if t0 is not None:
        _timed_end(t0, 'maxabs', nbytes=float(sum(_weights[p].shape[0] * _weights[p].shape[1] * 4 for p in ptrs)))
    guard = _StreamGuard(device)
    for p, bound in _weight_jobs['parts'].items():
        _weights[p].maxima = (_weight_stamp(live[p]), bound, guard)


def prefetch_weight_bounds(device):
    if current_mode() == 'f16x3' and _weights:
        _measure_all_weights(device)


def _weight_or_measured_max(x):
    rec = _registered(x)
    if rec is None:
        return maxabs_partials(x)
    if rec.maxima is None or rec.maxima[0][0] != _weight_epoch[0]:
        _measure_all_weights(x.device)
    return _derived(rec, 'maxima', x, lambda: maxabs_partials(_whole(x, rec)))


def _f32op(x, bound=None):
    if isinstance(x, F32Op):
        return x
    return F32Op(x, bound, 1) if bound is not None else F32Op(x)


_const_bounds = {}


def const_bound(value, device):
    key = (float(value), str(device))
    ent = _const_bounds.get(key)
    if ent is None:
        t = torch.full((1,), float(value), device=device, dtype=torch.float32)
        ent = (t, _StreamGuard(device) if t.is_cuda else None)
        _const_bounds[key] = ent
    if ent[1] is not None:
        ent[1].wait(device)
    return ent[0]


def operand_like(x, other):
    if current_mode() != 'f16x3' or not isinstance(other, F32Op):
        return operand(x)
    part, n = other.bound()
    return F32Op(x, part, n)


def _skinny_shape(ta, m, n, k, a, b, split_k):
    return (not ta and split_k == 1 and n <= 256 and 16 <= k <= 208 and k % 4 == 0 and m >= 256 and
            a.stride(0) % 4 == 0 and a.data_ptr() % 16 == 0 and b.data_ptr() % 16 == 0 and
            os.environ.get('RENET_GEMM_SKINNY', '1') != '0')


def _fused_bounds(t):
    return current_mode() == 'f16x3' and t.is_cuda and t.numel() > 0 and os.environ.get('RENET_FUSED_BOUNDS', '1') != '0'


def _note_bound(t, part, n):
    t._renet_bound = (part, n)


def _call_with_bounds(entry, args, elems, outs):
    nparts = lib().renet_bound_parts(elems)
    parts = torch.empty(len(outs), nparts, device=outs[0].device, dtype=torch.float32)
    _check(getattr(lib(), 'renet_' + entry)(*args, *[p.data_ptr() for p in parts], _stream()), entry)
    for t, p in zip(outs, parts):
        _note_bound(t, p, nparts)


_lazy_shells = {}


def lazy_shell(mat, device):
    x = torch.empty(mat.R, mat.C, device=device, dtype=torch.float32)
    x._renet_bf16 = mat
    key = (x.data_ptr(), (mat.R, mat.C))
    _lazy_shells[key] = mat
    weakref.finalize(x, _drop_lazy_shell, key, mat)
    return x


def _drop_lazy_shell(key, mat):
    if _lazy_shells.get(key) is mat:
        del _lazy_shells[key]


def operand(x, bound=None):
    if isinstance(x, (BF16Mat, F32Op)):
        return x
    lazy = getattr(x, '_renet_bf16', None)
    if lazy is None:
        lazy = _lazy_shells.pop((x.data_ptr(), tuple(x.shape)), None)
    else:
        _lazy_shells.pop((x.data_ptr(), tuple(x.shape)), None)
    if lazy is not None:
        return lazy
    if current_mode() == 'bf16s':
        return pack_bf16(x)
    if current_mode() == 'f16x3' and x.is_cuda and x.dim() == 2:
        noted = getattr(x, '_renet_bound', None)
        if noted is not None and bound is None:
            return F32Op(x, noted[0], noted[1])
        return _f32op(x, bound)
    return x


def gemm_bf16s(a, b, ta=False, tb=False, out=None, bias=None, alpha=1.0, beta=0.0, split_k=None):
    def prep(x, k_axis):
        m, r, c = _as_bf16(x)
        klen, kfull = (r, m.R) if k_axis == 0 else (c, m.C)
        if klen != kfull and (klen % 64) != 0:
            m = pack_bf16(x)
            r, c = m.R, m.C
        return m, r, c
    pa, ar, ac = prep(a, 0 if ta else 1)
    pb, br, bc = prep(b, 1 if tb else 0)
    m, k = (ac, ar) if ta else (ar, ac)
    n, k2 = (br, bc) if tb else (bc, br)
    out, split_k, ws, ws_bytes = _gemm_front('gemm', m, n, k, k2, out, beta, split_k, pa.p.device)
    t0 = _timed()
    _check(lib().renet_gemm_bf16s(int(ta), int(not tb), m, n, k, float(alpha), pa.p.data_ptr(), pa.p.shape[1],
                                  pb.p.data_ptr(), pb.p.shape[1], float(beta), out.data_ptr(), _ld(out), _f32(bias),
                                  split_k, _f32(ws), ws_bytes, _stream()), 'gemm_bf16s')
    _gemm_timed_end(t0, ta, tb, m, n, k, split_k)
    return out


def gemm(a, b, ta=False, tb=False, out=None, bias=None, alpha=1.0, beta=0.0, split_k=None, mode=None):
    if (mode or current_mode()) == 'bf16s' or isinstance(a, BF16Mat) or isinstance(b, BF16Mat):
        return gemm_bf16s(a, b, ta=ta, tb=tb, out=out, bias=bias, alpha=alpha, beta=beta, split_k=split_k)
    md = mode or current_mode()
    opa, opb = a, b
    if isinstance(a, F32Op):
        a = a.t
    if isinstance(b, F32Op):
        b = b.t
    if not (a.is_cuda and b.is_cuda and a.dtype == torch.float32 and b.dtype == torch.float32):
        raise RenetHipError('gemm operands must be float32 device tensors')
    m, k = (a.shape[1], a.shape[0]) if ta else (a.shape[0], a.shape[1])
    k2, n = (b.shape[1], b.shape[0]) if tb else (b.shape[0], b.shape[1])
    out, split_k, ws, ws_bytes = _gemm_front('gemm', m, n, k, k2, out, beta, split_k, a.device)
    if md == 'f16x3' and _skinny_shape(ta, m, n, k, a, b, split_k):
        md = 'bf16x6'
    if md == 'f16x3':
        (pa, na), (pb, nb) = _f32op(opa).bound(), _f32op(opb).bound()
    t0 = _timed()
    if md == 'f16x3':
        _check(lib().renet_gemm_f32_h3(int(ta), int(tb), m, n, k, float(alpha), a.data_ptr(), _ld(a), b.data_ptr(),
                                       _ld(b), float(beta), out.data_ptr(), _ld(out), _f32(bias), split_k, _f32(ws),
                                       ws_bytes, pa.data_ptr(), na, pb.data_ptr(), nb, _stream()),
               'gemm_f32_h3')
    else:
        fn = lib().renet_gemm_f32_split if md == 'bf16x6' else lib().renet_gemm_bf16 if md == 'bf16' else \
            lib().renet_gemm_f32
        _check(fn(int(ta), int(tb), m, n, k, float(alpha), a.data_ptr(), _ld(a), b.data_ptr(),
                  _ld(b), float(beta), out.data_ptr(), _ld(out), _f32(bias), split_k, _f32(ws),
                  ws_bytes, _stream()), 'gemm_f32')
    _gemm_timed_end(t0, ta, tb, m, n, k, split_k)
    return out


def colsum(x, out=None, beta=0.0):
    fn, what, t = (lib().renet_colsum_bf16, 'colsum_bf16', x.p) if isinstance(x, BF16Mat) else \
        (lib().renet_colsum, 'colsum', x)
    m, n = x.shape
    if out is None:
        if beta != 0.0:
            raise RenetHipError('beta != 0 needs an output tensor')
        out = torch.empty(n, device=t.device, dtype=torch.float32)
    nbytes = lib().renet_colsum_workspace(m, n)
    ws = torch.empty(nbytes // 4, device=t.device, dtype=torch.float32) if nbytes else None
    _check(fn(t.data_ptr(), m, n, _ld(t), _f32(out), float(beta), _f32(ws), nbytes, _stream()), what)
    return out


def scale_by_device_scalar(x, g, bound_in=None):
    if bound_in is not None and not isinstance(x, BF16Mat):
        if not x.is_contiguous():
            raise RenetHipError('scale_by_device_scalar needs a contiguous tensor')
        out = torch.empty(1, device=x.device, dtype=torch.float32)
        _check(lib().renet_scale_by_device_scalar_bound(_f32(x), x.numel(), _f32(g), float(bound_in), out.data_ptr(),
                                                        _stream()), 'scale_by_device_scalar_bound')
        return out
    if isinstance(x, BF16Mat):
        _check(lib().renet_scale_bf16_by_device_scalar(x.p.data_ptr(), x.p.numel(), _f32(g), _stream()),
               'scale_bf16_by_device_scalar')
        return x
    if not x.is_contiguous():
        raise RenetHipError('scale_by_device_scalar needs a contiguous tensor')
    _check(lib().renet_scale_by_device_scalar(_f32(x), x.numel(), _f32(g), _stream()), 'scale_by_device_scalar')
    return x


def seq_assemble_fwd(h2, ent, rel, glob, subj_row, row_ent, row_rel, glob_row, drop_p, seed_x, seed_xr):
    s, d = subj_row.numel(), h2.shape[1]
    x = torch.empty(s, 4 * d, device=h2.device, dtype=torch.float32)
    xr = torch.empty(s, 3 * d, device=h2.device, dtype=torch.float32)
    args = (_f32(h2), _f32(ent), _f32(rel), _f32(glob), _i32(subj_row), _i32(row_ent), _i32(row_rel), _i32(glob_row), s, d,
            float(drop_p), int(seed_x), int(seed_xr), _f32(x), _f32(xr))
    if _fused_bounds(x):
        _call_with_bounds('seq_assemble_fwd_bounds', args, s * d, (x, xr))
    else:
        _check(lib().renet_seq_assemble_fwd(*args, _stream()), 'seq_assemble_fwd')
    return x, xr


def seq_assemble_fwd_bf16(h2, ent, rel, glob, subj_row, row_ent, row_rel, glob_row, drop_p, seed_x, seed_xr):
    s, d = subj_row.numel(), h2.shape[1]
    x, xr = bf16_empty(s, 4 * d, h2.device), bf16_empty(s, 3 * d, h2.device)
    _check(lib().renet_seq_assemble_fwd_bf16(_f32(h2), _f32(ent), _f32(rel), _f32(glob), _i32(subj_row), _i32(row_ent),
                                             _i32(row_rel), _i32(glob_row), s, d, float(drop_p), int(seed_x),
                                             int(seed_xr), x.p.data_ptr(), x.p.shape[1], xr.p.data_ptr(),
                                             xr.p.shape[1], x.p.shape[0], _stream()), 'seq_assemble_fwd_bf16')
    return x, xr


def softmax_ce_bf16(logits, target, grad_scale, row_loss=None):
    b, c = logits.shape
    if row_loss is None:
        row_loss = torch.empty(b, device=logits.device, dtype=torch.float32)
    dl = bf16_empty(b, c, logits.device)
    _check(lib().renet_softmax_ce_bf16(logits.data_ptr(), _i32(target), b, c, _ld(logits), float(grad_scale),
                                       _f32(row_loss), dl.p.data_ptr(), dl.p.shape[1], min((b + 63) & ~63, dl.p.shape[0]),
                                       _stream()), 'softmax_ce_bf16')
    return row_loss, dl


def seq_assemble_bwd(dx, dxr, step_off, num_steps, num_seq, d, drop_p, seed_x, seed_xr):
    s = dx.shape[0]
    d_rows = torch.empty(s, d, device=dx.device, dtype=torch.float32)
    d_ent = torch.empty(num_seq, d, device=dx.device, dtype=torch.float32)
    d_rel = torch.empty(num_seq, d, device=dx.device, dtype=torch.float32)
    _check(lib().renet_seq_assemble_bwd(_f32(dx), _f32(dxr), _i32(step_off), num_steps, s, num_seq, d,
                                        float(drop_p), int(seed_x), int(seed_xr), _f32(d_rows), _f32(d_ent),
                                        _f32(d_rel), _stream()), 'seq_assemble_bwd')
    return d_rows, d_ent, d_rel


def gru_fwd(gi, step_off_host, hdim, w_hh, b_hh, out_rows=0):
    hs, svs = gru_fwd_layouts([gi], [step_off_host], hdim, [w_hh], [b_hh], [out_rows])
    return hs[0], svs[0]


def gru_bwd(dh_last, step_off_host, hdim, w_hh, saved):
    d_gis, d_ghs = gru_bwd_layouts([dh_last], [step_off_host], hdim, [w_hh], [saved])
    return d_gis[0], d_ghs[0]


def _ptrs(tensors):
    return (ctypes.c_void_p * len(tensors))(*[t.data_ptr() for t in tensors])


def _offs(step_offs):
    return ((ctypes.c_void_p * len(step_offs))(*[ctypes.cast(o, c_void_p).value for o in step_offs]),
            (ctypes.c_int * len(step_offs))(*[len(o) - 1 for o in step_offs]))


def _seqs(o):
    return (o[1] - o[0]) if len(o) > 1 else 0


_GRU_SUFFIX = {'bf16s': '_bf16', 'f32': '_f32'}


def _gru_call(n, step_offs, hdim, operands):
    for t in operands:
        _f32(t)
    bmax = max([_seqs(o) for o in step_offs] + [0])
    nbytes = n * lib().renet_gru_workspace(int(bmax), hdim)
    ws = torch.empty(max(nbytes // 4, 1), device=operands[0].device, dtype=torch.float32)
    return (bmax, ws, nbytes) + _offs(step_offs)


def _gru_timed_end(t0, hdim, packed):
    if t0 is not None:
        _timed_end(t0, 'gru_recurrence', flops=sum(2.0 * 3 * hdim * hdim * t.shape[0] for t in packed))


def gru_fwd_multi(gis, step_off_host, hdim, w_hhs, b_hhs, out_rows=0):
    L = len(step_off_host) - 1
    out_rows = max(int(out_rows), _seqs(step_off_host))
    dev = gis[0].device
    hs = [torch.empty(out_rows, hdim, device=dev, dtype=torch.float32) for _ in gis]
    svs = [torch.empty(g.shape[0], 5 * hdim, device=dev, dtype=torch.float32) for g in gis]
    _, ws, nbytes, _, _ = _gru_call(len(gis), [step_off_host], hdim, list(gis) + list(w_hhs) + list(b_hhs))
    t0 = _timed()
    _check(lib().renet_gru_fwd_multi(len(gis), _ptrs(gis), ctypes.cast(step_off_host, c_void_p), L, hdim,
                                     _ptrs(w_hhs), _ptrs(b_hhs), _ptrs(hs), out_rows, _ptrs(svs), ws.data_ptr(),
                                     nbytes, _stream()), 'gru_fwd_multi')
    _gru_timed_end(t0, hdim, gis)
    return hs, svs


def gru_bwd_multi(dh_lasts, step_off_host, hdim, w_hhs, saveds):
    L = len(step_off_host) - 1
    n = len(dh_lasts)
    dev = saveds[0].device
    d_gis = [torch.empty(s.shape[0], 3 * hdim, device=dev, dtype=torch.float32) for s in saveds]
    d_ghs = [torch.empty(s.shape[0], 3 * hdim, device=dev, dtype=torch.float32) for s in saveds]
    _, ws, nbytes, _, _ = _gru_call(n, [step_off_host], hdim, list(dh_lasts) + list(w_hhs) + list(saveds))
    t0 = _timed()
    _check(lib().renet_gru_bwd_multi(n, _ptrs(dh_lasts), ctypes.cast(step_off_host, c_void_p), L, hdim,
                                     _ptrs(w_hhs), _ptrs(saveds), _ptrs(d_gis), _ptrs(d_ghs), ws.data_ptr(),
                                     nbytes, _stream()), 'gru_bwd_multi')
    _gru_timed_end(t0, hdim, saveds)
    return d_gis, d_ghs


def gru_fwd_layouts(gis, step_offs, hdim, w_hhs, b_hhs, out_rows):
    n = len(gis)
    dev = gis[0].device
    rows = [max(int(r), _seqs(o)) for r, o in zip(out_rows, step_offs)]
    hs = [torch.empty(r, hdim, device=dev, dtype=torch.float32) for r in rows]
    svs = [torch.empty(g.shape[0], 5 * hdim, device=dev, dtype=torch.float32) for g in gis]
    _, ws, nbytes, so, ls = _gru_call(n, step_offs, hdim, list(gis) + list(w_hhs) + list(b_hhs))
    fn = getattr(lib(), 'renet_gru_fwd_layouts' + _GRU_SUFFIX.get(current_mode(), ''))
    t0 = _timed()
    _check(fn(n, _ptrs(gis), so, ls, hdim, _ptrs(w_hhs), _ptrs(b_hhs), _ptrs(hs), (ctypes.c_int * n)(*rows),
              _ptrs(svs), ws.data_ptr(), nbytes, _stream()), 'gru_fwd_layouts')
    _gru_timed_end(t0, hdim, gis)
    return hs, svs


def gru_bwd_layouts(dh_lasts, step_offs, hdim, w_hhs, saveds, out_bf16=False):
    n = len(dh_lasts)
    dev = saveds[0].device
    if out_bf16:
        if current_mode() != 'bf16s':
            raise RenetHipError('bf16 GRU gradients exist in bf16-storage mode only')
        d_gis = [bf16_empty(s_.shape[0], 3 * hdim, dev) for s_ in saveds]
        d_ghs = [bf16_empty(s_.shape[0], 3 * hdim, dev) for s_ in saveds]
        lds = {m.p.shape[1] for m in d_gis + d_ghs}
        assert len(lds) == 1
        for m in d_gis + d_ghs:
            _check(lib().renet_bf16_zero_padding(m.p.data_ptr(), m.R, m.C, m.p.shape[1], m.p.shape[0], _stream()),
                   'bf16_zero_padding')
    else:
        d_gis = [torch.empty(s.shape[0], 3 * hdim, device=dev, dtype=torch.float32) for s in saveds]
        d_ghs = [torch.empty(s.shape[0], 3 * hdim, device=dev, dtype=torch.float32) for s in saveds]
    bmax, ws, nbytes, so, ls = _gru_call(n, step_offs, hdim, list(dh_lasts) + list(w_hhs) + list(saveds))
    head = (n, _ptrs(dh_lasts), so, ls, hdim, _ptrs(w_hhs), _ptrs(saveds))
    tail = (ws.data_ptr(), nbytes, _stream())
    t0 = _timed()
    rc = -2
    if out_bf16:
        rc = lib().renet_gru_bwd_layouts_bf16out(*head, _ptrs([m.p for m in d_gis]), _ptrs([m.p for m in d_ghs]),
                                                 lds.pop(), *tail)
        _check(rc, 'gru_bwd_layouts_bf16out')
    elif _fused_bounds(d_gis[0]) and bmax > 0:
        nparts = lib().renet_gru_bound_parts(int(bmax))
        parts = torch.empty(n, nparts, device=dev, dtype=torch.float32)
        rc = lib().renet_gru_bwd_layouts_bounds(*head, _ptrs(d_gis), _ptrs(d_ghs),
                                                _ptrs([parts[k] for k in range(n)]), *tail)
        if rc == 0:
            for k in range(n):
                _note_bound(d_gis[k], parts[k], nparts)
        elif rc != -2:
            _check(rc, 'gru_bwd_layouts_bounds')
    if rc == -2:
        fn = getattr(lib(), 'renet_gru_bwd_layouts' + _GRU_SUFFIX.get(current_mode(), ''))
        _check(fn(*head, _ptrs(d_gis), _ptrs(d_ghs), *tail), 'gru_bwd_layouts')
    _gru_timed_end(t0, hdim, saveds)
    return d_gis, d_ghs


def concat3_fwd(a, ia, hmid, c, ic, drop_p, seed):
    b, d = hmid.shape
    parts = 3 if c is not None else 2
    feat = torch.empty(b, parts * d, device=hmid.device, dtype=torch.float32)
    args = (_f32(a), _i32(ia), _f32(hmid), _f32(c), _i32(ic), b, d, float(drop_p), int(seed), _f32(feat))
    if _fused_bounds(feat):
        _call_with_bounds('concat3_fwd_bounds', args, b * parts * (d // 4), (feat,))
    else:
        _check(lib().renet_concat3_fwd(*args, _stream()), 'concat3_fwd')
    return feat


def concat3_bwd(dfeat, d, parts, drop_p, seed):
    b = dfeat.shape[0]
    da = torch.empty(b, d, device=dfeat.device, dtype=torch.float32)
    dh = torch.empty(b, d, device=dfeat.device, dtype=torch.float32)
    dc = torch.empty(b, d, device=dfeat.device, dtype=torch.float32) if parts == 3 else None
    _check(lib().renet_concat3_bwd(_f32(dfeat), b, d, parts, float(drop_p), int(seed), _f32(da), _f32(dh),
                                   _f32(dc), _stream()), 'concat3_bwd')
    return da, dh, dc


def dropout(x, drop_p, seed):
    y = torch.empty_like(x)
    _check(lib().renet_dropout(_f32(x), x.numel(), float(drop_p), int(seed), _f32(y), _stream()), 'dropout')
    return y


def softmax_ce(logits, target, grad_scale, want_grad, row_loss=None):
    b, c = logits.shape
    if row_loss is None:
        row_loss = torch.empty(b, device=logits.device, dtype=torch.float32)
    _check(lib().renet_softmax_ce(logits.data_ptr(), _i32(target), b, c, _ld(logits), float(grad_scale),
                                  _f32(row_loss), logits.data_ptr() if want_grad else None, _stream()),
           'softmax_ce')
    return row_loss


def rank_rows(scores, label, filt_ptr=None, filt_col=None, filtered=True, want_loss=True):
    if not (scores.is_cuda and scores.dtype == torch.float32 and scores.dim() == 2):
        raise RenetHipError('rank_rows needs a 2-D float32 device tensor')
    n, c = scores.shape
    if label.numel() != n or (filt_ptr is not None and (filt_col is None or filt_ptr.numel() != n + 1)):
        raise RenetHipError('rank_rows: shape mismatch')
    counts = torch.empty(2, n, device=scores.device, dtype=torch.int32)
    row_loss = torch.empty(n, device=scores.device, dtype=torch.float32) if want_loss else None
    t0 = _timed()
    _check(lib().renet_rank_rows(scores.data_ptr(), max(_ld(scores), c) if n == 1 else _ld(scores), n, c, _i32(label),
                                 _i32(filt_ptr), _i32(filt_col), int(bool(filtered)), counts[0].data_ptr(),
                                 counts[1].data_ptr(), _f32(row_loss), _stream()), 'rank_rows')
    _timed_end(t0, 'rank_rows', nbytes=float(n * c * 4))
    return counts, row_loss


def rank_rows3(scores, label, cols_a, start_a, count_a, cols_t, start_t, count_t, want_loss=True):
    if not (scores.is_cuda and scores.dtype == torch.float32 and scores.dim() == 2):
        raise RenetHipError('rank_rows3 needs a 2-D float32 device tensor')
    n, c = scores.shape
    lists = []
    for cols, start, count in ((cols_a, start_a, count_a), (cols_t, start_t, count_t)):
        if cols is None and start is None and count is None:
            lists += [None, None, None, 0]
            continue
        if cols is None or start is None or count is None or start.numel() != n or count.numel() != n:
            raise RenetHipError('rank_rows3: a filter list is (cols, start [n], count [n])')
        lists += [_i32(cols), _i32(start), _i32(count), cols.numel()] if cols.numel() else [None, None, None, 0]
    if label.numel() != n:
        raise RenetHipError('rank_rows3: shape mismatch')
    counts = torch.empty(6, n, device=scores.device, dtype=torch.int32)
    row_loss = torch.empty(n, device=scores.device, dtype=torch.float32) if want_loss else None
    t0 = _timed()
    _check(lib().renet_rank_rows3(scores.data_ptr(), max(_ld(scores), c) if n == 1 else _ld(scores), n, c, _i32(label),
                                  *lists, counts.data_ptr(), _f32(row_loss), _stream()), 'rank_rows3')
    _timed_end(t0, 'rank_rows3', nbytes=float(n * c * 4))
    return counts, row_loss


def joint_softmax(logits, num_rels, logits_r, prob_e):
    nr, n_ent = logits.shape
    n = nr // num_rels
    if nr != n * num_rels or tuple(logits_r.shape) != (n, num_rels) or prob_e.numel() != n:
        raise RenetHipError('joint_softmax: shape mismatch')
    _check(lib().renet_joint_softmax(logits.data_ptr(), _ld(logits), n, num_rels, n_ent, logits_r.data_ptr(),
                                     _ld(logits_r), _f32(prob_e), _stream()), 'joint_softmax')
    return logits


def topk_positive(x, k):
    if not (x.is_cuda and x.dtype == torch.float32 and x.dim() == 2 and x.stride(1) == 1):
        raise RenetHipError('topk_positive needs a 2-D float32 device tensor with unit inner stride')
    n, m = x.shape
    vals = torch.empty(n, k, device=x.device, dtype=torch.float32)
    idx = torch.empty(n, k, device=x.device, dtype=torch.int64)
    nbytes = lib().renet_topk_workspace(n)
    ws = torch.empty(nbytes // 4 + 1, device=x.device, dtype=torch.int32)
    _check(lib().renet_topk_positive(x.data_ptr(), x.stride(0) if n > 1 else m, n, m, int(k), vals.data_ptr(),
                                     idx.data_ptr(), ws.data_ptr(), nbytes, _stream()), 'topk_positive')
    return vals, idx


def segment_pool_fwd(h, seg_ptr, num_graphs, is_max):
    d = h.shape[1]
    out = torch.empty(num_graphs, d, device=h.device, dtype=torch.float32)
    arg = torch.empty(num_graphs, d, device=h.device, dtype=torch.int32)
    _check(lib().renet_segment_pool_fwd(_f32(h), _i32(seg_ptr), num_graphs, d, int(is_max), _f32(out),
                                        _i32(arg), _stream()), 'segment_pool_fwd')
    return out, arg


def segment_pool_bwd(dout, seg_ptr, arg, num_graphs, is_max, n):
    d = dout.shape[1]
    dh = torch.empty(n, d, device=dout.device, dtype=torch.float32)
    _check(lib().renet_segment_pool_bwd(_f32(dout), _i32(seg_ptr), _i32(arg), num_graphs, d, int(is_max), n,
                                        _f32(dh), _stream()), 'segment_pool_bwd')
    return dh


def _host_i32(a):
    if a.dtype.name != 'int32' or not a.flags['C_CONTIGUOUS']:
        raise RenetHipError('host index arrays must be contiguous int32')
    return a.ctypes.data_as(c_void_p)


def nbr_pool_fwd(e, r, p, q, v, nb):
    attn = p is not None
    d = e.shape[1]
    out = torch.empty(nb.S, (3 if attn else 2) * d, device=e.device, dtype=torch.float32)
    stats = torch.empty(nb.S, 2, device=e.device, dtype=torch.float32) if attn else None
    w = torch.empty(nb.nnz, device=e.device, dtype=torch.float32) if attn else None
    t0 = _timed()
    _check(lib().renet_nbr_pool_fwd(_f32(e), _f32(r) if attn else None, _f32(p), _f32(q) if attn else None,
                                    _f32(v) if attn else None, _i32(nb.nbr), _i32(nb.seg_ptr), _host_i32(nb.seg_ptr_host),
                                    _i32(nb.seg_s), _i32(nb.seg_r), _i32(nb.seg_q), _i32(nb.out_row), nb.S, d, int(attn),
                                    _f32(out), _f32(stats), _f32(w), _stream()), 'nbr_pool_fwd')
    _timed_end(t0, 'nbr_pool_fwd', nbytes=float(nb.nnz * d * 4 * (2 if attn else 1) + out.numel() * 4))
    return out, stats, w


def nbr_pool_bwd(dout, out, e, p, q, v, w, nb):
    attn = p is not None
    d = e.shape[1]

    def rows(n, on=True):
        return torch.empty(n, d, device=e.device, dtype=torch.float32) if on else None
    ce, cp = rows(nb.nnz), rows(nb.nnz, attn)
    dq, dv, ds, dr = rows(nb.S, attn), rows(nb.S, attn), rows(nb.S), rows(nb.S, attn)
    t0 = _timed()
    _check(lib().renet_nbr_pool_bwd(_f32(dout), _f32(out) if attn else None, _f32(e), _f32(p), _f32(q) if attn else None,
                                    _f32(v) if attn else None, _f32(w), _i32(nb.nbr), _i32(nb.seg_ptr),
                                    _host_i32(nb.seg_ptr_host), _i32(nb.seg_q), _i32(nb.out_row), nb.S, d, int(attn),
                                    _f32(ce), _f32(cp), _f32(dq), _f32(dv), _f32(ds), _f32(dr), _stream()), 'nbr_pool_bwd')
    _timed_end(t0, 'nbr_pool_bwd', nbytes=float(nb.nnz * d * 4 * (4 if attn else 1) + dout.numel() * 4))
    return ce, cp, dq, dv, ds, dr


def sumsq_partials(g, partial, slot0, n_slots):
    _check(lib().renet_sumsq_partials(_f32(g), g.numel(), partial.data_ptr() + 4 * slot0, int(n_slots), _stream()),
           'sumsq_partials')


def adam_step(p, g, m, v, lr, beta1, beta2, eps, weight_decay, max_norm, step, zero_grad=True, norm_out=None,
              grad_scale=1.0, presummed=None):
    n = p.numel()
    if presummed is not None:
        part, n_part = presummed
        _check(lib().renet_adam_step_presummed(_f32(p), _f32(g), _f32(m), _f32(v), n, float(lr), float(beta1), float(beta2),
                                               float(eps), float(weight_decay), float(max_norm), float(grad_scale),
                                               int(step), int(zero_grad), _f32(part), int(n_part), _f32(norm_out),
                                               _stream()), 'adam_step_presummed')
        return
    nbytes = lib().renet_adam_workspace(n)
    ws = torch.empty(nbytes // 4, device=p.device, dtype=torch.float32)
    _check(lib().renet_adam_step_scaled(_f32(p), _f32(g), _f32(m), _f32(v), n, float(lr), float(beta1), float(beta2),
                                        float(eps), float(weight_decay), float(max_norm), float(grad_scale), int(step),
                                        int(zero_grad), ws.data_ptr(), nbytes, _f32(norm_out), _stream()), 'adam_step')
```

### re-net_amd/step_plan.py

```python
import ctypes
import os
import weakref

import torch
from torch.autograd import Function

import ops
import renet_hip as K

ENABLED = os.environ.get('RENET_STEP_PLAN', '1') != '0'

_cache = weakref.WeakKeyDictionary()


def _slot(net):
    c = _cache.get(net)
    if c is None:
        c = _cache[net] = {}
    return c

_P = ctypes.c_void_p
_I = ctypes.c_int


class SegPlanC(ctypes.Structure):
    _fields_ = [('order', _P), ('seg_ptr', _P), ('target', _P), ('num_segments', _I)]


_PARAMS = ('ent', 'rel', 'w1', 'loop1', 'w2', 'loop2', 'wih', 'whh', 'bih', 'bhh', 'wih_r', 'whh_r', 'bih_r', 'bhh_r', 'lin_w',
           'lin_b', 'linr_w', 'linr_b')


class StepModelC(ctypes.Structure):
    _fields_ = [('D', _I), ('num_ent', _I), ('T', _I), ('C2', _I), ('drop_p', ctypes.c_float)] + \
               [(n, _P) for n in _PARAMS] + [('g_' + n, _P) for n in _PARAMS] + \
               [('glob', _P), ('lin_w_planes', _P), ('lin_w_plane', ctypes.c_size_t), ('lin_w_ld', _I)]


_BATCH_INTS = ('N', 'E', 'nA', 'S', 'B', 'L', 'n_items', 'n_groups', 'n_groups_out', 'n_heavy', 'n_heavy_out', 'n_chunks',
               'n_chunks2')
_BATCH_PTRS = ('step_off_host', 'node_ent', 'row_ptr', 'col', 'etype', 'norm', 'it_src', 'it_type', 'grp_ptr', 'heavy_rows',
               'heavy_rows_out', 'it_src_t', 'it_type_t', 'col_t', 'e_src_t', 'e_src', 'e_dst', 'chunk_ptr', 'chunk_type',
               'type_chunk_ptr', 'e_src2', 'e_dst2', 'chunk_ptr2', 'chunk_type2', 'type_chunk_ptr2', 'subj_row', 'row_ent',
               'row_rel', 'glob_row', 'step_off', 's_idx', 'r_idx', 'ent_label', 'rel_label')


class StepBatchC(ctypes.Structure):
    _fields_ = [(n, _I) for n in _BATCH_INTS] + [(n, _P) for n in _BATCH_PTRS] + \
               [('plan_node_ent', SegPlanC), ('plan_subj_row', SegPlanC), ('plan_s', SegPlanC), ('plan_r', SegPlanC)]


class StepRunC(ctypes.Structure):
    _fields_ = [('seed_rgcn1', ctypes.c_uint64), ('seed_rgcn2', ctypes.c_uint64), ('seed_x', ctypes.c_uint64),
                ('seed_xr', ctypes.c_uint64), ('seed_head1', ctypes.c_uint64), ('seed_head2', ctypes.c_uint64),
                ('scale_ent', ctypes.c_float), ('scale_rel', ctypes.c_float), ('workspace', _P),
                ('workspace_bytes', ctypes.c_size_t), ('stream', _P), ('side_stream', _P)]


def model_params(net):
    c = _slot(net).get('params')
    if c is not None and c[0] is net._parameters.get('ent_embeds') and c[14] is net.linear._parameters.get('weight'):
        return c
    a, e, er = net.aggregator, net.encoder, net.encoder_r
    c = (net.ent_embeds, net.rel_embeds, a.rgcn1.weight, a.rgcn1.loop_weight, a.rgcn2.weight, a.rgcn2.loop_weight,
         e.weight_ih_l0, e.weight_hh_l0, e.bias_ih_l0, e.bias_hh_l0, er.weight_ih_l0, er.weight_hh_l0, er.bias_ih_l0,
         er.bias_hh_l0, net.linear.weight, net.linear.bias, net.linear_r.weight, net.linear_r.bias)
    _slot(net)['params'] = c
    _slot(net).pop('model', None)
    return c


def _grad_ok(p):
    g = p.grad
    return g is not None and g.is_cuda and g.dtype == torch.float32 and g.is_contiguous() and g.shape == p.shape


def _pointers(params):
    return tuple(p.data_ptr() for p in params), tuple(p.grad.data_ptr() if p.grad is not None else 0 for p in params)


def eligible(net, prep, row_tap=None):
    if not ENABLED or prep is None or K._timer is not None or ops.debug_tap is not None or not torch.is_grad_enabled():
        return False
    if K.current_mode() != 'bf16x6' or os.environ.get('RENET_GRU', '') == 'steps':
        return False
    g = prep.g
    if g is None or not hasattr(g, 'grp_ptr') or getattr(g, 'nA', None) is None:
        return False
    ps = model_params(net)
    ptrs = _pointers(ps)
    ent = _slot(net).get('model')
    if ent is None or ent[0] != ptrs:
        if not all(p.is_cuda and p.dtype == torch.float32 and p.is_contiguous() and p.requires_grad and
                   (p.grad is None or _grad_ok(p)) for p in ps):
            return False
        _slot(net)['model'] = (ptrs, None)
    d = net.h_dim
    return max(g.N, net.ent_embeds.shape[0]) * d * 4 < (1 << 31) and g.S > 0 and g.L > 0


def _model_struct(net, params, planes):
    ptrs = _pointers(params)
    ent = _slot(net).get('model')
    m = ent[1] if (ent is not None and ent[0] == ptrs) else None
    if m is None:
        m = StepModelC()
        m.D, m.num_ent, m.T, m.C2 = net.h_dim, net.ent_embeds.shape[0], net.rel_embeds.shape[0], net.linear_r.weight.shape[0]
        for n, pp, gp in zip(_PARAMS, ptrs[0], ptrs[1]):
            setattr(m, n, pp)
            setattr(m, 'g_' + n, gp or None)
        _slot(net)['model'] = (ptrs, m)
    m.drop_p = float(net.drop_p) if net.training else 0.0
    if planes is not None:
        m.lin_w_planes, m.lin_w_plane, m.lin_w_ld = planes.p.data_ptr(), planes.plane, planes.p.shape[2]
    else:
        m.lin_w_planes, m.lin_w_plane, m.lin_w_ld = None, 0, 0
    return m


def _batch_struct(prep):
    ent = getattr(prep, '_step_batch', None)
    if ent is not None:
        return ent[0]
    g = prep.g
    b = StepBatchC()
    it_src_t, it_type_t, col_t, e_src_t = g.table_items()
    heavy, heavy_out = g.heavy_rows, getattr(g, 'heavy_rows_out', None)
    vals = dict(N=g.N, E=g.E, nA=g.nA, S=g.S, B=prep.b, L=g.L, n_items=g.it_src.numel(), n_groups=g.n_groups,
                n_groups_out=g.n_groups_out, n_heavy=heavy.numel() if heavy is not None else 0,
                n_heavy_out=heavy_out.numel() if heavy_out is not None else 0, n_chunks=g.n_chunks, n_chunks2=g.n_chunks2)
    for n, v in vals.items():
        setattr(b, n, int(v))
    tens = dict(node_ent=g.node_ent, row_ptr=g.row_ptr, col=g.col, etype=g.etype, norm=g.norm, it_src=g.it_src,
                it_type=g.it_type, grp_ptr=g.grp_ptr, heavy_rows=heavy, heavy_rows_out=heavy_out, it_src_t=it_src_t,
                it_type_t=it_type_t, col_t=col_t, e_src_t=e_src_t, e_src=g.e_src, e_dst=g.e_dst, chunk_ptr=g.chunk_ptr,
                chunk_type=g.chunk_type, type_chunk_ptr=g.type_chunk_ptr, e_src2=g.e_src2, e_dst2=g.e_dst2,
                chunk_ptr2=g.chunk_ptr2, chunk_type2=g.chunk_type2, type_chunk_ptr2=g.type_chunk_ptr2, subj_row=g.subj_row,
                row_ent=g.row_ent, row_rel=g.row_rel, glob_row=g.glob_row, step_off=g.step_off, s_idx=prep.s_idx,
                r_idx=prep.r_idx, ent_label=prep.o_idx, rel_label=prep.r_label)
    for n, t in tens.items():
        if t is not None:
            if n == 'norm':
                K._f32(t, n)
            else:
                K._i32(t, n)
            setattr(b, n, t.data_ptr())
    b.step_off_host = ctypes.cast(prep.step_off, _P).value
    plans = []
    for n in ('plan_node_ent', 'plan_subj_row', 'plan_s', 'plan_r'):
        p = getattr(prep, n, None) if n in ('plan_s', 'plan_r') else getattr(g, n)
        if p is None:
            p = getattr(g, n)
        c = SegPlanC(K._i32(p.order), K._i32(p.seg_ptr), K._i32(p.target), int(p.num_segments))
        setattr(b, n, c)
        plans.append(p)
    prep._step_batch = (b, tens, plans, (it_src_t, it_type_t, col_t, e_src_t))
    return b


_events = {}
_hook_streams = {}


def _side_stream(device):
    if not (ops.SIDE_STREAM and device.type == 'cuda'):
        return None
    key = device.index if device.index is not None else torch.cuda.current_device()
    st = ops._side_streams.get(key)
    if st is None:
        st = ops._side_streams[key] = torch.cuda.Stream(device=device)
    return st


def _head_event(device, which=0):
    key = (device.index if device.index is not None else torch.cuda.current_device(), which)
    ev = _events.get(key)
    if ev is None:
        ev = torch.cuda.Event()
        ev.record()
        _events[key] = ev
        _hook_streams[key] = torch.cuda.Stream(device=device)
    return ev, _hook_streams[key]


class StepFn(Function):

    @staticmethod
    def forward(ctx, net, prep, row_tap, *params):
        dev = net.ent_embeds.device
        g = prep.g
        p = float(net.drop_p) if net.training else 0.0
        with ops.shared_graph_seeds(getattr(prep, 'sharded', False) or ops.SHARED_GRAPH_SEEDS):
            s_r1 = ops.next_seed(graph_site=True) if p > 0 else 0
            s_r2 = ops.next_seed(graph_site=True) if p > 0 else 0
            s_x, s_xr = (ops.next_seed(), ops.next_seed()) if p > 0 else (0, 0)
        s_h1, s_h2 = (ops.next_seed(), ops.next_seed()) if p > 0 else (0, 0)
        planes = K.weight_planes(params[14]) if K.use_planes(params[14], params[14].shape[0]) else None
        m = _model_struct(net, params, planes)
        m.glob = K._f32(g.glob, 'global embeddings')
        b = _batch_struct(prep)
        lib = K.lib()
        nbytes = lib.renet_step_workspace(ctypes.addressof(m), ctypes.addressof(b))
        if nbytes == 0:
            raise K.RenetHipError('renet_step_workspace rejected the model / batch')
        ws = torch.empty(nbytes, device=dev, dtype=torch.uint8)
        scale = 2.0 * getattr(prep, 'share', 1.0)
        bb = prep.b
        s1, s2 = float(scale) / bb, float(scale) * 0.1 / bb
        rl = torch.empty(2 * bb, device=dev, dtype=torch.float32)
        side = _side_stream(dev)
        r = StepRunC(int(s_r1), int(s_r2), int(s_x), int(s_xr), int(s_h1), int(s_h2), s1, s2, ws.data_ptr(), nbytes,
                     K._stream(), side.cuda_stream if side is not None else None)
        nl = ctypes.c_int(0)
        K._check(lib.renet_step_forward(ctypes.addressof(m), ctypes.addressof(b), ctypes.addressof(r), rl.data_ptr(),
                                        ctypes.addressof(nl)), 'renet_step_forward')
        ctx.net, ctx.prep, ctx.m, ctx.b, ctx.r, ctx.ws, ctx.planes = net, prep, m, b, r, ws, planes
        ctx.consumed = False
        ctx.launches = nl.value
        ctx.gemm_mode = K.current_mode()
        ctx.side = side
        net.aggregator.last_batch = g
        StepFn.last_launches = [nl.value, 0]
        if row_tap is not None:
            row_tap.append((rl.detach(), s1, s2))
        return torch.dot(rl, ops._loss_weight_vector(bb, s1, s2, dev))

    @staticmethod
    def backward(ctx, g):
        if ctx.consumed:
            raise RuntimeError('StepFn: the saved CE gradients were consumed by the first backward pass; a second pass over '
                               'the same graph is not supported')
        ctx.consumed = True
        params = model_params(ctx.net)
        m, b, r = ctx.m, ctx.b, ctx.r
        missing = [i for i, p in enumerate(params) if not _grad_ok(p)]
        fresh = [None] * len(params)
        if missing:
            if any(params[i].grad is not None for i in missing):
                raise RuntimeError('StepFn: a parameter has an unusable .grad (non-contiguous / wrong dtype); set '
                                   'RENET_STEP_PLAN=0')
            offs, tot = [], 0
            for i in missing:
                offs.append(tot)
                tot += (params[i].numel() + 3) & ~3
            flat = torch.zeros(tot, device=params[0].device, dtype=torch.float32)
            for i, o in zip(missing, offs):
                fresh[i] = flat[o:o + params[i].numel()].view_as(params[i])
        for i, (n, p) in enumerate(zip(_PARAMS, params)):
            setattr(m, 'g_' + n, (fresh[i] if fresh[i] is not None else p.grad).data_ptr())
        dev = ctx.net.ent_embeds.device
        side = ctx.side
        r.stream = K._stream()
        r.side_stream = side.cuda_stream if side is not None else None
        defer = bool(ops.DEFER_WEIGHT_GRADS and side is not None and not missing)
        lin_w, lin_b = params[14], params[15]
        hooked = (ops.hooks_wanted(lin_w) or ops.hooks_wanted(lin_b)) and not missing
        ev = hs = ev2 = hs2 = None
        if hooked:
            ev, hs = _head_event(dev)
        gru_params = params[6:14]
        hooked_gru = not missing and any(ops.hooks_wanted(p) for p in gru_params)
        if hooked_gru:
            ev2, hs2 = _head_event(dev, 1)
        g = g.contiguous()
        nl = ctypes.c_int(0)
        lib = K.lib()
        K._check(lib.renet_step_backward(ctypes.addressof(m), ctypes.addressof(b), ctypes.addressof(r), K._f32(g),
                                         int(defer), ev.cuda_event if ev is not None else None,
                                         ev2.cuda_event if ev2 is not None else None, ctypes.addressof(nl)),
                 'renet_step_backward')
        StepFn.last_launches[1] = nl.value
        if hooked_gru:
            hs2.wait_event(ev2)
            with torch.cuda.stream(hs2):
                for p in gru_params:
                    ops.grad_done(p)
        if hooked:
            hs.wait_event(ev)
            with torch.cuda.stream(hs):
                ops.grad_done(lin_w)
                ops.grad_done(lin_b)
        keep = (ctx.ws, ctx.prep, ctx.planes, m, b, g)
        if defer:
            ops._deferred.append((torch.cuda.current_stream(dev), side, keep))
        ctx.ws = None
        return (None, None, None) + tuple(fresh)


StepFn.last_launches = [0, 0]
```

Before: 386,500 triples/s.

## Prepare GRU weight planes on an aux stream and overlap backward head work

Adds a third auxiliary stream to the fused training step. The GRU recurrent-weight fragment planes (forward and backward) are now split once per step on the aux stream, overlapping the RGCN GEMMs, instead of being rebuilt inside each GRU call. The backward head gradient scatter and concat work also moves onto the aux stream, with event marks replacing the fixed ring of ordering events. The data-loader pool freezes the garbage collector before forking. The cost is extra events and workspace, plus more complex cross-stream dependencies that could introduce ordering bugs.

```diff
diff --git a/include/renet_hip.h b/include/renet_hip.h
--- a/include/renet_hip.h
+++ b/include/renet_hip.h
@@ -188,6 +188,16 @@
 int renet_gru_bwd_layouts_bf16(int n, const float* const* dh_last, const int32_t* const* step_off, const int* L, int H,
                                const float* const* Whh, const float* const* saved, float* const* dGi,
                                float* const* dGh, float* workspace, size_t workspace_bytes, void* stream);
+size_t renet_gru_planes_bytes(int H);
+int renet_gru_prepare_planes(int n, int H, const float* const* Whh, void* fwd_planes, void* bwd_planes,
+                             size_t planes_bytes, void* stream);
+int renet_gru_fwd_layouts_prepared(int n, const float* const* Gi, const int32_t* const* step_off, const int* L, int H,
+                                   const float* const* Whh, const float* const* bhh, float* const* h_last,
+                                   const int* out_rows, float* const* saved, const void* fwd_planes, size_t planes_bytes,
+                                   void* stream);
+int renet_gru_bwd_layouts_prepared(int n, const float* const* dh_last, const int32_t* const* step_off, const int* L, int H,
+                                   const float* const* Whh, const float* const* saved, float* const* dGi,
+                                   float* const* dGh, const void* bwd_planes, size_t planes_bytes, void* stream);
 
 int renet_concat3_fwd(const float* a, const int32_t* ia, const float* hmid, const float* c,
                       const int32_t* ic, int B, int D, float drop_p, uint64_t seed, float* feat,
@@ -359,6 +369,7 @@
     void* workspace;
     size_t workspace_bytes;
     void *stream, *side_stream;
+    void* aux_stream;
 } RenetStepRun;
 size_t renet_step_workspace(const RenetStepModel* m, const RenetStepBatch* b);
 int renet_step_forward(const RenetStepModel* m, const RenetStepBatch* b, const RenetStepRun* r, float* row_loss,
diff --git a/re-net_amd/csrc/gru.hip b/re-net_amd/csrc/gru.hip
--- a/re-net_amd/csrc/gru.hip
+++ b/re-net_amd/csrc/gru.hip
@@ -97,9 +97,18 @@
     return Bmax;
 }
 
+int split_fwd(const float* Whh, int H, void* planes, hipStream_t st, int npl) {
+    return renet_gru_split_frag(Whh, H, H, 3, (size_t)H * H, (size_t)H, 1, planes, st, npl);
+}
+int split_bwd(const float* Whh, int H, void* planes, hipStream_t st, int npl) {
+    return renet_gru_split_frag(Whh, H, 3 * H, 1, 0, 1, (size_t)H, planes, st, npl);
+}
+
+bool planes_preparable(int npl) { return npl != 0 && !(use_f32() && npl == 3) && !(npl == 3 && !use_persistent()); }
+
 int gru_fwd_impl(int npl, int n, const float* const* Gi, const int32_t* const* step_off, const int* L, int H,
                  const float* const* Whh, const float* const* bhh, float* const* h_last, const int* out_rows,
-                 float* const* saved, float* workspace, size_t workspace_bytes, void* stream) {
+                 float* const* saved, float* workspace, size_t workspace_bytes, void* stream, bool prepared = false) {
     Layouts ly;
     int B_of[MAXP];
     const int e0 = make_layouts(n, step_off, L, out_rows, true, ly, B_of);
@@ -107,6 +116,7 @@
     if (max_rows(ly) == 0) return RENET_OK;
     if (!renet_dim_ok(H) || (npl == 1 && H == 300)) return RENET_ERR_UNSUPPORTED;
     hipStream_t st = (hipStream_t)stream;
+    if (prepared && !planes_preparable(npl)) return RENET_ERR_UNSUPPORTED;
     if (npl == 0 || (use_f32() && npl == 3)) {
         FwdProbs ps;
         for (int i = 0; i < MAXP; ++i) {
@@ -125,8 +135,8 @@
         const int k = i < n ? i : 0;
         const int slot = plane_slot(k, Whh);
         bf16x8* planes = reinterpret_cast<bf16x8*>(ws + (size_t)slot * per);
-        if (i < n && slot == k) {
-            const int e = renet_gru_split_frag(Whh[k], H, H, 3, (size_t)H * H, (size_t)H, 1, planes, st, npl);
+        if (i < n && slot == k && !prepared) {
+            const int e = split_fwd(Whh[k], H, planes, st, npl);
             if (e != RENET_OK) return e;
         }
         ps.p[i] = {Gi[k], planes, bhh[k], h_last[k], saved[k]};
@@ -142,7 +152,7 @@
 int gru_bwd_impl(int npl, int n, const float* const* dh_last, const int32_t* const* step_off, const int* L, int H,
                  const float* const* Whh, const float* const* saved, float* const* dGi, float* const* dGh,
                  float* workspace, size_t workspace_bytes, void* stream, int out_ld = 0,
-                 float* const* bounds = nullptr) {
+                 float* const* bounds = nullptr, bool prepared = false) {
     Layouts ly;
     int B_of[MAXP];
     const int e0 = make_layouts(n, step_off, L, nullptr, false, ly, B_of);
@@ -152,6 +162,7 @@
     hipStream_t st = (hipStream_t)stream;
     const bool f32 = npl == 0 || (use_f32() && npl == 3);
     const bool steps = npl == 3 && !f32 && !use_persistent();
+    if (prepared && !planes_preparable(npl)) return RENET_ERR_UNSUPPORTED;
     if (bounds && (f32 || steps || npl != 3)) return RENET_ERR_UNSUPPORTED;
     const int Bmax = max_batch(n, B_of);
     const size_t per = slice_bytes(steps ? Bmax : 0, H);
@@ -162,9 +173,9 @@
         const int k = i < n ? i : 0;
         const int slot = plane_slot(k, Whh);
         wt[i] = ws + (size_t)slot * per;
-        if (i < n && slot == k) {
+        if (i < n && slot == k && !prepared) {
             const int e = f32 ? renet_gru_transpose(Whh[k], 3 * H, H, reinterpret_cast<float*>(wt[i]), st)
-                              : renet_gru_split_frag(Whh[k], H, 3 * H, 1, 0, 1, (size_t)H, wt[i], st, npl);
+                              : split_bwd(Whh[k], H, wt[i], st, npl);
             if (e != RENET_OK) return e;
         }
     }
@@ -213,6 +224,41 @@
 int renet_gru_bwd_layouts_f32(GRU_BWD_PARAMS) { return gru_bwd_impl(0, GRU_BWD_ARGS); }
 int renet_gru_bwd_layouts_bf16(GRU_BWD_PARAMS) { return gru_bwd_impl(1, GRU_BWD_ARGS); }
 
+size_t renet_gru_planes_bytes(int H) { return slice_bytes(0, H); }
+
+int renet_gru_prepare_planes(int n, int H, const float* const* Whh, void* fwd_planes, void* bwd_planes,
+                             size_t planes_bytes, void* stream) {
+    if (n < 1 || n > MAXP || !Whh || (!fwd_planes && !bwd_planes)) return RENET_ERR_BADARG;
+    if (!renet_dim_ok(H) || !planes_preparable(3)) return RENET_ERR_UNSUPPORTED;
+    const size_t per = slice_bytes(0, H);
+    if (planes_bytes < (size_t)n * per) return RENET_ERR_WORKSPACE;
+    hipStream_t st = (hipStream_t)stream;
+    for (int k = 0; k < n; ++k) {
+        if (plane_slot(k, Whh) != k) continue;
+        int e = fwd_planes ? split_fwd(Whh[k], H, reinterpret_cast<char*>(fwd_planes) + (size_t)k * per, st, 3) : RENET_OK;
+        if (e == RENET_OK && bwd_planes) e = split_bwd(Whh[k], H, reinterpret_cast<char*>(bwd_planes) + (size_t)k * per, st, 3);
+        if (e != RENET_OK) return e;
+    }
+    return RENET_OK;
+}
+
+int renet_gru_fwd_layouts_prepared(int n, const float* const* Gi, const int32_t* const* step_off, const int* L, int H,
+                                   const float* const* Whh, const float* const* bhh, float* const* h_last,
+                                   const int* out_rows, float* const* saved, const void* fwd_planes, size_t planes_bytes,
+                                   void* stream) {
+    if (!fwd_planes) return RENET_ERR_BADARG;
+    return gru_fwd_impl(3, n, Gi, step_off, L, H, Whh, bhh, h_last, out_rows, saved,
+                        reinterpret_cast<float*>(const_cast<void*>(fwd_planes)), planes_bytes, stream, true);
+}
+
+int renet_gru_bwd_layouts_prepared(int n, const float* const* dh_last, const int32_t* const* step_off, const int* L, int H,
+                                   const float* const* Whh, const float* const* saved, float* const* dGi,
+                                   float* const* dGh, const void* bwd_planes, size_t planes_bytes, void* stream) {
+    if (!bwd_planes) return RENET_ERR_BADARG;
+    return gru_bwd_impl(3, n, dh_last, step_off, L, H, Whh, saved, dGi, dGh,
+                        reinterpret_cast<float*>(const_cast<void*>(bwd_planes)), planes_bytes, stream, 0, nullptr, true);
+}
+
 int renet_gru_bound_parts(int max_rows) { return max(1, (max_rows + MT - 1) / MT); }
 
 int renet_gru_bwd_layouts_bounds(int n, const float* const* dh_last, const int32_t* const* step_off, const int* L, int H,
diff --git a/re-net_amd/csrc/step.cpp b/re-net_amd/csrc/step.cpp
--- a/re-net_amd/csrc/step.cpp
+++ b/re-net_amd/csrc/step.cpp
@@ -47,8 +47,8 @@
     size_t ew, gi0, gi1, hs0, hs1, logits, featp;
     size_t dfeat1, dfeat2, da1, da2, dh1, dh2, dc1, dgi0, dgi1, dgh0, dgh1, dX, dXr, d_rows, d_ent_seq, d_rel_seq, d_h2, gn2,
         gl2, dhN, gn1, gl1, dh1N, gs;
-    size_t gru_ws, gemm_ws_main, gemm_ws_side, bwdw_ws, colsum_ws;
-    size_t gru_ws_bytes, gemm_ws_bytes, bwdw_ws_bytes, colsum_ws_bytes;
+    size_t gru_pl_f, gru_pl_b, gemm_ws_main, gemm_ws_side, gemm_ws_aux, bwdw_ws, bwdw_ws_aux, colsum_ws;
+    size_t gru_pl_bytes, gemm_ws_bytes, gemm_ws_aux_bytes, bwdw_ws_bytes, colsum_ws_bytes;
     size_t dl_plane, dl_ld, dl_rows, featp_plane, featp_ld, featp1_plane, featp1_ld, logits_ld;
     size_t total;
 };
@@ -115,9 +115,9 @@
     L.gl1 = take(fbytes(N, D));
     L.dh1N = take(fbytes(N, D));
     L.gs = take(fbytes(NE, D));
-    const int bmax = b.L > 0 ? b.step_off_host[1] - b.step_off_host[0] : 0;
-    L.gru_ws_bytes = 2 * renet_gru_workspace(bmax, m.D);
-    L.gru_ws = take(std::max<size_t>(L.gru_ws_bytes, 4));
+    L.gru_pl_bytes = 2 * renet_gru_planes_bytes(m.D);
+    L.gru_pl_f = take(std::max<size_t>(L.gru_pl_bytes, 4));
+    L.gru_pl_b = take(std::max<size_t>(L.gru_pl_bytes, 4));
     size_t need = 4;
     auto g_ = [&](int mm, int nn, int kk) { need = std::max(need, renet_gemm_workspace(mm, nn, auto_split_k(mm, nn, kk))); };
     const int Di = m.D, Si = b.S, Bi = b.B, NEi = m.num_ent, nAi = b.nA, C2i = m.C2;
@@ -133,8 +133,12 @@
     L.gemm_ws_bytes = need;
     L.gemm_ws_main = take(need);
     L.gemm_ws_side = take(need);
+    L.gemm_ws_aux_bytes = std::max<size_t>(std::max(renet_gemm_workspace(Di, Di, auto_split_k(Di, Di, NEi)),
+                                                    renet_gemm_workspace(Di, Di, auto_split_k(Di, Di, nAi))), 4);
+    L.gemm_ws_aux = take(L.gemm_ws_aux_bytes);
     L.bwdw_ws_bytes = std::max<size_t>(renet_rgcn_bwd_w_workspace(std::max(b.n_chunks, b.n_chunks2), m.D), 4);
     L.bwdw_ws = take(L.bwdw_ws_bytes);
+    L.bwdw_ws_aux = take(L.bwdw_ws_bytes);
     size_t cs = 4;
     cs = std::max(cs, renet_colsum_workspace(Bi, NEi));
     cs = std::max(cs, renet_colsum_workspace(Bi, C2i));
@@ -163,17 +167,32 @@
     return ev[i];
 }
 
+struct Mark { hipEvent_t e; hipStream_t on; };
+
 struct Streams {
-    hipStream_t main, side;
+    hipStream_t main, side, aux;
     int next_ev = 0, rc = 0;
-    bool two() const { return side != main; }
+    explicit Streams(const RenetStepRun& r) {
+        main = (hipStream_t)r.stream;
+        side = r.side_stream ? (hipStream_t)r.side_stream : main;
+        aux = (r.aux_stream && r.aux_stream != r.stream) ? (hipStream_t)r.aux_stream : side;
+    }
+    bool one() const { return side == main && aux == main; }
+    Mark mark(hipStream_t on) {
+        if (one() || rc) return {nullptr, on};
+        hipEvent_t e = step_event(next_ev++);
+        if (!e) { rc = (int)hipErrorOutOfMemory; return {nullptr, on}; }
+        const hipError_t x = hipEventRecord(e, on);
+        if (x != hipSuccess) { rc = (int)x; return {nullptr, on}; }
+        return {e, on};
+    }
+    void wait(hipStream_t then, const Mark& m) {
+        if (!m.e || m.on == then || rc) return;
+        const hipError_t x = hipStreamWaitEvent(then, m.e, 0);
+        if (x != hipSuccess) rc = (int)x;
+    }
     void order(hipStream_t first, hipStream_t then) {
-        if (!two() || rc) return;
-        hipEvent_t e = step_event(next_ev++ & 7);
-        if (!e) { rc = (int)hipErrorOutOfMemory; return; }
-        hipError_t x = hipEventRecord(e, first);
-        if (x == hipSuccess) x = hipStreamWaitEvent(then, e, 0);
-        if (x != hipSuccess) rc = (int)x;
+        if (first != then) wait(then, mark(first));
     }
     void fork() { order(main, side); }
     void join() { order(side, main); }
@@ -211,7 +230,7 @@
     if (r->workspace_bytes < L.total) return RENET_ERR_WORKSPACE;
     char* W = (char*)r->workspace;
     auto F = [&](size_t off) { return (float*)(W + off); };
-    Streams s{(hipStream_t)r->stream, (hipStream_t)(r->side_stream ? r->side_stream : r->stream)};
+    Streams s(*r);
     int launches = 0;
     const int D = m.D, N = b.N, nA = b.nA, S = b.S, B = b.B, NE = m.num_ent, T = m.T;
     const float p = m.drop_p;
@@ -219,6 +238,10 @@
     float* wsm = F(L.gemm_ws_main);
     float* wss = F(L.gemm_ws_side);
 
+    const float* whh[2] = {m.whh, m.whh_r};
+    s.order(s.main, s.aux);
+    CK(renet_gru_prepare_planes(2, D, whh, W + L.gru_pl_f, W + L.gru_pl_b, L.gru_pl_bytes, s.aux));
+    const Mark planes_ready = s.mark(s.aux);
     CK(gemm(s.main, wsm, L.gemm_ws_bytes, 0, 0, NE, D, D, m.ent, D, m.loop1, D, 0.f, F(L.ew), D, nullptr));
     CK(renet_rgcn_gather_items_table(m.ent, NE, D, b.it_src_t, b.it_type_t, b.grp_ptr, b.n_groups, b.row_ptr, b.col_t, b.etype,
                                      b.node_ent, b.norm, m.w1, T, 0, F(L.ew), p, r->seed_rgcn1, 1, F(L.out1), N,
@@ -238,14 +261,14 @@
         const float* gi[2] = {F(L.gi0), F(L.gi1)};
         const int32_t* so[2] = {b.step_off_host, b.step_off_host};
         const int ls[2] = {b.L, b.L};
-        const float* whh[2] = {m.whh, m.whh_r};
         const float* bhh[2] = {m.bhh, m.bhh_r};
         float* hl[2] = {F(L.hs0), F(L.hs1)};
         const int bmax = b.step_off_host[1] - b.step_off_host[0];
         const int rows[2] = {std::max(B, bmax), std::max(B, bmax)};
         float* sv[2] = {F(L.sv0), F(L.sv1)};
         if (rows[0] != B) return RENET_ERR_BADARG;
-        CK(renet_gru_fwd_layouts(2, gi, so, ls, D, whh, bhh, hl, rows, sv, F(L.gru_ws), L.gru_ws_bytes, s.main));
+        s.wait(s.main, planes_ready);
+        CK(renet_gru_fwd_layouts_prepared(2, gi, so, ls, D, whh, bhh, hl, rows, sv, W + L.gru_pl_f, L.gru_pl_bytes, s.main));
     }
     s.fork();
     CK(renet_concat3_fwd(m.ent, b.s_idx, F(L.hs1), nullptr, nullptr, B, D, p, r->seed_head2, F(L.feat2), s.side));
@@ -278,7 +301,7 @@
     if (r->workspace_bytes < L.total) return RENET_ERR_WORKSPACE;
     char* W = (char*)r->workspace;
     auto F = [&](size_t off) { return (float*)(W + off); };
-    Streams s{(hipStream_t)r->stream, (hipStream_t)(r->side_stream ? r->side_stream : r->stream)};
+    Streams s(*r);
     int launches = 0;
     const int D = m.D, N = b.N, nA = b.nA, S = b.S, B = b.B, NE = m.num_ent, T = m.T, C2 = m.C2;
     const float p = m.drop_p;
@@ -291,6 +314,9 @@
         const size_t need = renet_colsum_workspace(M_, N_);
         return renet_colsum(X, M_, N_, N_, out, 1.f, need ? csw : nullptr, need, st);
     };
+    auto seg = [&](const float* src, const RenetSegPlan& pn, float* dst, hipStream_t st) {
+        return renet_segment_add(src, pn.order, pn.seg_ptr, pn.target, pn.num_segments, D, dst, st);
+    };
 
     if (!pl) CK(renet_scale_by_device_scalar(F(L.dl1), (size_t)B * NE, g, s.main));
     s.fork();
@@ -298,30 +324,40 @@
     CK(gemm(s.side, wss, L.gemm_ws_bytes, 0, 0, B, 2 * D, C2, F(L.dl2), C2, m.linr_w, 2 * D, 0.f, F(L.dfeat2), 2 * D, nullptr));
     CK(gemm(s.side, wss, L.gemm_ws_bytes, 1, 0, C2, 2 * D, B, F(L.dl2), C2, F(L.feat2), 2 * D, 1.f, m.g_linr_w, 2 * D, nullptr));
     CK(colsum(F(L.dl2), B, C2, m.g_linr_b, s.side));
+    if (!pl) CK(colsum(F(L.dl1), B, NE, m.g_lin_b, s.side));
     CK(renet_concat3_bwd(F(L.dfeat2), B, D, 2, p, r->seed_head2, F(L.da2), F(L.dh2), nullptr, s.side));
+    const Mark rel_head = s.mark(s.side);
     if (pl) {
         const int sk1 = auto_split_k_planes(B, 3 * D, NE);
         CK(renet_gemm_planes(0, 1, B, 3 * D, NE, 1.f, g, W + L.dl1, (int)L.dl_ld, L.dl_plane, m.lin_w_planes, m.lin_w_ld,
                              m.lin_w_plane, 0.f, F(L.dfeat1), 3 * D, nullptr, nullptr, sk1, sk1 > 1 ? wsm : nullptr,
                              sk1 > 1 ? L.gemm_ws_bytes : 0, s.main));
+    } else {
+        CK(gemm(s.main, wsm, L.gemm_ws_bytes, 0, 0, B, 3 * D, NE, F(L.dl1), NE, m.lin_w, 3 * D, 0.f, F(L.dfeat1), 3 * D, nullptr));
+    }
+    s.order(s.main, s.aux);
+    CK(renet_zero(F(L.d_h2), (size_t)nA * D, s.aux));
+    CK(renet_concat3_bwd(F(L.dfeat1), B, D, 3, p, r->seed_head1, F(L.da1), F(L.dh1), F(L.dc1), s.aux));
+    const Mark ent_head = s.mark(s.aux);
+    s.wait(s.aux, rel_head);
+    CK(renet_add_inplace(F(L.da1), F(L.da2), (size_t)B * D, s.aux));
+    CK(seg(F(L.da1), b.plan_s, m.g_ent, s.aux));
+    CK(seg(F(L.dc1), b.plan_r, m.g_rel, s.aux));
+    if (pl) {
         const int sk2 = auto_split_k_planes(NE, 3 * D + 1, B);
         CK(renet_gemm_planes(1, 1, NE, 3 * D + 1, B, 1.f, g, W + L.dl1, (int)L.dl_ld, L.dl_plane, W + L.featp1, (int)L.featp1_ld,
                              L.featp1_plane, 1.f, m.g_lin_w, 3 * D, nullptr, m.g_lin_b, sk2, sk2 > 1 ? wsm : nullptr,
                              sk2 > 1 ? L.gemm_ws_bytes : 0, s.main));
     } else {
-        CK(colsum(F(L.dl1), B, NE, m.g_lin_b, s.side));
-        CK(gemm(s.main, wsm, L.gemm_ws_bytes, 0, 0, B, 3 * D, NE, F(L.dl1), NE, m.lin_w, 3 * D, 0.f, F(L.dfeat1), 3 * D, nullptr));
         CK(gemm(s.main, wsm, L.gemm_ws_bytes, 1, 0, NE, 3 * D, B, F(L.dl1), NE, F(L.feat1), 3 * D, 1.f, m.g_lin_w, 3 * D, nullptr));
-    }
-    CK(renet_concat3_bwd(F(L.dfeat1), B, D, 3, p, r->seed_head1, F(L.da1), F(L.dh1), F(L.dc1), s.main));
-    s.join();
+        s.wait(s.main, rel_head);
+    }
     if (ev_head_done) {
         const hipError_t e = hipEventRecord((hipEvent_t)ev_head_done, s.main);
         if (e != hipSuccess) return (int)e;
     }
-    CK(renet_add_inplace(F(L.da1), F(L.da2), (size_t)B * D, s.main));
-    CK(renet_segment_add(F(L.da1), b.plan_s.order, b.plan_s.seg_ptr, b.plan_s.target, b.plan_s.num_segments, D, m.g_ent, s.main));
-    CK(renet_segment_add(F(L.dc1), b.plan_r.order, b.plan_r.seg_ptr, b.plan_r.target, b.plan_r.num_segments, D, m.g_rel, s.main));
+    s.wait(s.main, ent_head);
+    s.wait(s.main, rel_head);
 
     {
         const float* dhl[2] = {F(L.dh1), F(L.dh2)};
@@ -331,7 +367,7 @@
         const float* sv[2] = {F(L.sv0), F(L.sv1)};
         float* dgi[2] = {F(L.dgi0), F(L.dgi1)};
         float* dgh[2] = {F(L.dgh0), F(L.dgh1)};
-        CK(renet_gru_bwd_layouts(2, dhl, so, ls, D, whh, sv, dgi, dgh, F(L.gru_ws), L.gru_ws_bytes, s.main));
+        CK(renet_gru_bwd_layouts_prepared(2, dhl, so, ls, D, whh, sv, dgi, dgh, W + L.gru_pl_b, L.gru_pl_bytes, s.main));
     }
     auto gru_param_grads = [&]() -> int {
         const float* xs[2] = {F(L.X), F(L.Xr)};
@@ -364,40 +400,47 @@
 
     CK(renet_seq_assemble_bwd(F(L.dX), F(L.dXr), b.step_off, b.L, S, B, D, p, r->seed_x, r->seed_xr, F(L.d_rows), F(L.d_ent_seq),
                               F(L.d_rel_seq), s.main));
-    CK(renet_zero(F(L.d_h2), (size_t)nA * D, s.main));
-    CK(renet_segment_add(F(L.d_rows), b.plan_subj_row.order, b.plan_subj_row.seg_ptr, b.plan_subj_row.target,
-                         b.plan_subj_row.num_segments, D, F(L.d_h2), s.main));
-    CK(renet_segment_add(F(L.d_ent_seq), b.plan_s.order, b.plan_s.seg_ptr, b.plan_s.target, b.plan_s.num_segments, D, m.g_ent, s.main));
-    CK(renet_segment_add(F(L.d_rel_seq), b.plan_r.order, b.plan_r.seg_ptr, b.plan_r.target, b.plan_r.num_segments, D, m.g_rel, s.main));
+    s.order(s.main, s.aux);
+    CK(seg(F(L.d_ent_seq), b.plan_s, m.g_ent, s.aux));
+    CK(seg(F(L.d_rel_seq), b.plan_r, m.g_rel, s.aux));
+    const Mark emb_seq = s.mark(s.aux);
+    CK(seg(F(L.d_rows), b.plan_subj_row, F(L.d_h2), s.main));
 
     const int pair_shift = (T / 2) % T;
     CK(renet_rgcn_bwd_prep(F(L.d_h2), F(L.out2), b.norm, 0, p, r->seed_rgcn2, nA, D, F(L.gn2), F(L.gl2), s.main));
+    s.order(s.main, s.aux);
+    if (pruned)
+        CK(renet_rgcn_bwd_w(F(L.out1), F(L.gn2), b.e_src2, b.e_dst2, b.chunk_ptr2, b.chunk_type2, b.n_chunks2, b.type_chunk_ptr2, T,
+                            0, D, m.g_w2, 1.f, F(L.bwdw_ws_aux), renet_rgcn_bwd_w_workspace(b.n_chunks2, D), s.aux));
+    else
+        CK(renet_rgcn_bwd_w(F(L.out1), F(L.gn2), b.e_src, b.e_dst, b.chunk_ptr, b.chunk_type, b.n_chunks, b.type_chunk_ptr, T, 0, D,
+                            m.g_w2, 1.f, F(L.bwdw_ws_aux), renet_rgcn_bwd_w_workspace(b.n_chunks, D), s.aux));
+    CK(gemm(s.aux, F(L.gemm_ws_aux), L.gemm_ws_aux_bytes, 1, 0, D, D, nA, F(L.out1), D, F(L.gl2), D, 1.f, m.g_loop2, D, nullptr));
     CK(renet_rgcn_gather_items(F(L.gn2), D, b.it_src, b.it_type, b.grp_ptr, b.n_groups, b.row_ptr, b.col, b.etype, nullptr, m.w2, T,
                                pair_shift, 1, nullptr, 0.f, 0, 0, F(L.dhN), N, b.n_heavy ? b.heavy_rows : nullptr, b.n_heavy,
                                pruned ? nA : 0, 0, pruned ? 1 : 0, s.main));
     CK(gemm(s.main, wsm, L.gemm_ws_bytes, 0, 1, nA, D, D, F(L.gl2), D, m.loop2, D, 1.f, F(L.dhN), D, nullptr));
+
+    CK(renet_rgcn_bwd_prep(F(L.dhN), F(L.out1), b.norm, 1, p, r->seed_rgcn1, N, D, F(L.gn1), F(L.gl1), s.main));
     s.fork();
-    if (pruned)
-        CK(renet_rgcn_bwd_w(F(L.out1), F(L.gn2), b.e_src2, b.e_dst2, b.chunk_ptr2, b.chunk_type2, b.n_chunks2, b.type_chunk_ptr2, T,
-                            0, D, m.g_w2, 1.f, F(L.bwdw_ws), renet_rgcn_bwd_w_workspace(b.n_chunks2, D), s.side));
-    else
-        CK(renet_rgcn_bwd_w(F(L.out1), F(L.gn2), b.e_src, b.e_dst, b.chunk_ptr, b.chunk_type, b.n_chunks, b.type_chunk_ptr, T, 0, D,
-                            m.g_w2, 1.f, F(L.bwdw_ws), renet_rgcn_bwd_w_workspace(b.n_chunks, D), s.side));
-    CK(gemm(s.side, wss, L.gemm_ws_bytes, 1, 0, D, D, nA, F(L.out1), D, F(L.gl2), D, 1.f, m.g_loop2, D, nullptr));
-
-    CK(renet_rgcn_bwd_prep(F(L.dhN), F(L.out1), b.norm, 1, p, r->seed_rgcn1, N, D, F(L.gn1), F(L.gl1), s.main));
+    CK(renet_rgcn_bwd_w(m.ent, F(L.gn1), b.e_src_t, b.e_dst, b.chunk_ptr, b.chunk_type, b.n_chunks, b.type_chunk_ptr, T, 0, D,
+                        m.g_w1, 1.f, F(L.bwdw_ws), renet_rgcn_bwd_w_workspace(b.n_chunks, D), s.side));
+    s.order(s.main, s.aux);
+    CK(renet_zero(F(L.gs), (size_t)NE * D, s.aux));
+    CK(seg(F(L.gl1), b.plan_node_ent, F(L.gs), s.aux));
+    const Mark gs_ready = s.mark(s.aux);
+    CK(gemm(s.aux, F(L.gemm_ws_aux), L.gemm_ws_aux_bytes, 1, 0, D, D, NE, m.ent, D, F(L.gs), D, 1.f, m.g_loop1, D, nullptr));
     CK(renet_rgcn_gather_items(F(L.gn1), D, b.it_src, b.it_type, b.grp_ptr, b.n_groups, b.row_ptr, b.col, b.etype, nullptr, m.w1, T,
                                pair_shift, 1, nullptr, 0.f, 0, 0, F(L.dh1N), N, b.n_heavy ? b.heavy_rows : nullptr, b.n_heavy, 0, 0,
                                0, s.main));
-    s.fork();
-    CK(renet_rgcn_bwd_w(m.ent, F(L.gn1), b.e_src_t, b.e_dst, b.chunk_ptr, b.chunk_type, b.n_chunks, b.type_chunk_ptr, T, 0, D,
-                        m.g_w1, 1.f, F(L.bwdw_ws), renet_rgcn_bwd_w_workspace(b.n_chunks, D), s.side));
-    CK(renet_zero(F(L.gs), (size_t)NE * D, s.main));
-    CK(renet_segment_add2(F(L.dh1N), F(L.gl1), b.plan_node_ent.order, b.plan_node_ent.seg_ptr, b.plan_node_ent.target,
-                          b.plan_node_ent.num_segments, D, m.g_ent, F(L.gs), s.main));
+    s.wait(s.main, emb_seq);
+    CK(seg(F(L.dh1N), b.plan_node_ent, m.g_ent, s.main));
+    s.wait(s.main, gs_ready);
     CK(gemm(s.main, wsm, L.gemm_ws_bytes, 0, 1, NE, D, D, F(L.gs), D, m.loop1, D, 1.f, m.g_ent, D, nullptr));
-    CK(gemm(s.main, wsm, L.gemm_ws_bytes, 1, 0, D, D, NE, m.ent, D, F(L.gs), D, 1.f, m.g_loop1, D, nullptr));
-    if (!defer_side) s.join();
+    if (!defer_side) {
+        s.join();
+        s.order(s.aux, s.main);
+    }
     if (n_launches) *n_launches = launches;
     return s.rc;
 }
diff --git a/re-net_amd/pipeline.py b/re-net_amd/pipeline.py
--- a/re-net_amd/pipeline.py
+++ b/re-net_amd/pipeline.py
@@ -1,3 +1,4 @@
+import gc
 import multiprocessing as mp
 import os
 
@@ -11,6 +12,10 @@
 
 def _run(step):
     return _job['fn'](step)
+
+
+def _worker_init():
+    gc.freeze()
 
 
 class BatchPrefetcher(object):
@@ -50,7 +55,12 @@
             return
         _job['fn'] = self.fn
         ctx = mp.get_context('fork')
-        self.pool = ctx.Pool(self.num_workers)
+        gc.collect()
+        gc.freeze()
+        try:
+            self.pool = ctx.Pool(self.num_workers, initializer=_worker_init)
+        finally:
+            gc.unfreeze()
         try:
             for item in self.pool.imap(_run, self.steps, self.chunksize):
                 yield item
diff --git a/re-net_amd/renet_hip.py b/re-net_amd/renet_hip.py
--- a/re-net_amd/renet_hip.py
+++ b/re-net_amd/renet_hip.py
@@ -126,6 +126,10 @@
     'renet_gru_bwd_layouts_f32': (c_int, _GRU_BWD_LAYOUTS_ARGS),
     'renet_gru_fwd_layouts_bf16': (c_int, _GRU_FWD_LAYOUTS_ARGS),
     'renet_gru_bwd_layouts_bf16': (c_int, _GRU_BWD_LAYOUTS_ARGS),
+    'renet_gru_planes_bytes': (c_size_t, [c_int]),
+    'renet_gru_prepare_planes': (c_int, [c_int, c_int, c_void_p, c_void_p, c_void_p, c_size_t, c_void_p]),
+    'renet_gru_fwd_layouts_prepared': (c_int, _GRU_FWD_LAYOUTS_ARGS),
+    'renet_gru_bwd_layouts_prepared': (c_int, _GRU_BWD_LAYOUTS_ARGS),
     'renet_concat3_fwd': (c_int, [c_void_p, c_void_p, c_void_p, c_void_p, c_void_p, c_int, c_int, c_float,
                                   c_u64, c_void_p, c_void_p]),
     'renet_concat3_fwd_bounds': (c_int, [c_void_p, c_void_p, c_void_p, c_void_p, c_void_p, c_int, c_int, c_float,
@@ -1083,10 +1087,12 @@
 _GRU_SUFFIX = {'bf16s': '_bf16', 'f32': '_f32'}
 
 
-def _gru_call(n, step_offs, hdim, operands):
+def _gru_call(n, step_offs, hdim, operands, planes=None):
     for t in operands:
         _f32(t)
     bmax = max([_seqs(o) for o in step_offs] + [0])
+    if planes is not None:
+        return (bmax, planes, planes.numel()) + _offs(step_offs)
     nbytes = n * lib().renet_gru_workspace(int(bmax), hdim)
     ws = torch.empty(max(nbytes // 4, 1), device=operands[0].device, dtype=torch.float32)
     return (bmax, ws, nbytes) + _offs(step_offs)
@@ -1127,14 +1133,28 @@
     return d_gis, d_ghs
 
 
-def gru_fwd_layouts(gis, step_offs, hdim, w_hhs, b_hhs, out_rows):
+def gru_prepare_planes(hdim, w_hhs):
+    n = len(w_hhs)
+    nbytes = n * lib().renet_gru_planes_bytes(hdim)
+    fwd = torch.empty(nbytes, device=w_hhs[0].device, dtype=torch.uint8)
+    bwd = torch.empty(nbytes, device=w_hhs[0].device, dtype=torch.uint8)
+    for w in w_hhs:
+        _f32(w)
+    _check(lib().renet_gru_prepare_planes(n, hdim, _ptrs(w_hhs), fwd.data_ptr(), bwd.data_ptr(), nbytes, _stream()),
+           'gru_prepare_planes')
+    return fwd, bwd
+
+
+def gru_fwd_layouts(gis, step_offs, hdim, w_hhs, b_hhs, out_rows, planes=None):
     n = len(gis)
     dev = gis[0].device
     rows = [max(int(r), _seqs(o)) for r, o in zip(out_rows, step_offs)]
     hs = [torch.empty(r, hdim, device=dev, dtype=torch.float32) for r in rows]
     svs = [torch.empty(g.shape[0], 5 * hdim, device=dev, dtype=torch.float32) for g in gis]
-    _, ws, nbytes, so, ls = _gru_call(n, step_offs, hdim, list(gis) + list(w_hhs) + list(b_hhs))
+    _, ws, nbytes, so, ls = _gru_call(n, step_offs, hdim, list(gis) + list(w_hhs) + list(b_hhs), planes)
     fn = getattr(lib(), 'renet_gru_fwd_layouts' + _GRU_SUFFIX.get(current_mode(), ''))
+    if planes is not None:
+        fn = lib().renet_gru_fwd_layouts_prepared
     t0 = _timed()
     _check(fn(n, _ptrs(gis), so, ls, hdim, _ptrs(w_hhs), _ptrs(b_hhs), _ptrs(hs), (ctypes.c_int * n)(*rows),
               _ptrs(svs), ws.data_ptr(), nbytes, _stream()), 'gru_fwd_layouts')
@@ -1142,7 +1162,7 @@
     return hs, svs
 
 
-def gru_bwd_layouts(dh_lasts, step_offs, hdim, w_hhs, saveds, out_bf16=False):
+def gru_bwd_layouts(dh_lasts, step_offs, hdim, w_hhs, saveds, out_bf16=False, planes=None):
     n = len(dh_lasts)
     dev = saveds[0].device
     if out_bf16:
@@ -1158,12 +1178,15 @@
     else:
         d_gis = [torch.empty(s.shape[0], 3 * hdim, device=dev, dtype=torch.float32) for s in saveds]
         d_ghs = [torch.empty(s.shape[0], 3 * hdim, device=dev, dtype=torch.float32) for s in saveds]
-    bmax, ws, nbytes, so, ls = _gru_call(n, step_offs, hdim, list(dh_lasts) + list(w_hhs) + list(saveds))
+    bmax, ws, nbytes, so, ls = _gru_call(n, step_offs, hdim, list(dh_lasts) + list(w_hhs) + list(saveds), planes)
     head = (n, _ptrs(dh_lasts), so, ls, hdim, _ptrs(w_hhs), _ptrs(saveds))
     tail = (ws.data_ptr(), nbytes, _stream())
     t0 = _timed()
     rc = -2
-    if out_bf16:
+    if planes is not None:
+        rc = lib().renet_gru_bwd_layouts_prepared(*head, _ptrs(d_gis), _ptrs(d_ghs), *tail)
+        _check(rc, 'gru_bwd_layouts_prepared')
+    elif out_bf16:
         rc = lib().renet_gru_bwd_layouts_bf16out(*head, _ptrs([m.p for m in d_gis]), _ptrs([m.p for m in d_ghs]),
                                                  lds.pop(), *tail)
         _check(rc, 'gru_bwd_layouts_bf16out')
diff --git a/re-net_amd/step_plan.py b/re-net_amd/step_plan.py
--- a/re-net_amd/step_plan.py
+++ b/re-net_amd/step_plan.py
@@ -54,7 +54,7 @@
     _fields_ = [('seed_rgcn1', ctypes.c_uint64), ('seed_rgcn2', ctypes.c_uint64), ('seed_x', ctypes.c_uint64),
                 ('seed_xr', ctypes.c_uint64), ('seed_head1', ctypes.c_uint64), ('seed_head2', ctypes.c_uint64),
                 ('scale_ent', ctypes.c_float), ('scale_rel', ctypes.c_float), ('workspace', _P),
-                ('workspace_bytes', ctypes.c_size_t), ('stream', _P), ('side_stream', _P)]
+                ('workspace_bytes', ctypes.c_size_t), ('stream', _P), ('side_stream', _P), ('aux_stream', _P)]
 
 
 def model_params(net):
@@ -162,13 +162,17 @@
 _hook_streams = {}
 
 
-def _side_stream(device):
+_aux_streams = {}
+
+
+def _extra_stream(device, aux=False):
     if not (ops.SIDE_STREAM and device.type == 'cuda'):
         return None
+    pool = _aux_streams if aux else ops._side_streams
     key = device.index if device.index is not None else torch.cuda.current_device()
-    st = ops._side_streams.get(key)
+    st = pool.get(key)
     if st is None:
-        st = ops._side_streams[key] = torch.cuda.Stream(device=device)
+        st = pool[key] = torch.cuda.Stream(device=device)
     return st
 
 
@@ -208,9 +212,10 @@
         bb = prep.b
         s1, s2 = float(scale) / bb, float(scale) * 0.1 / bb
         rl = torch.empty(2 * bb, device=dev, dtype=torch.float32)
-        side = _side_stream(dev)
+        side, aux = _extra_stream(dev), _extra_stream(dev, aux=True)
         r = StepRunC(int(s_r1), int(s_r2), int(s_x), int(s_xr), int(s_h1), int(s_h2), s1, s2, ws.data_ptr(), nbytes,
-                     K._stream(), side.cuda_stream if side is not None else None)
+                     K._stream(), side.cuda_stream if side is not None else None,
+                     aux.cuda_stream if aux is not None else None)
         nl = ctypes.c_int(0)
         K._check(lib.renet_step_forward(ctypes.addressof(m), ctypes.addressof(b), ctypes.addressof(r), rl.data_ptr(),
                                         ctypes.addressof(nl)), 'renet_step_forward')
@@ -218,7 +223,7 @@
         ctx.consumed = False
         ctx.launches = nl.value
         ctx.gemm_mode = K.current_mode()
-        ctx.side = side
+        ctx.side, ctx.aux = side, aux
         net.aggregator.last_batch = g
         StepFn.last_launches = [nl.value, 0]
         if row_tap is not None:
@@ -249,9 +254,10 @@
         for i, (n, p) in enumerate(zip(_PARAMS, params)):
             setattr(m, 'g_' + n, (fresh[i] if fresh[i] is not None else p.grad).data_ptr())
         dev = ctx.net.ent_embeds.device
-        side = ctx.side
+        side, aux = ctx.side, ctx.aux
         r.stream = K._stream()
         r.side_stream = side.cuda_stream if side is not None else None
+        r.aux_stream = aux.cuda_stream if aux is not None else None
         defer = bool(ops.DEFER_WEIGHT_GRADS and side is not None and not missing)
         lin_w, lin_b = params[14], params[15]
         hooked = (ops.hooks_wanted(lin_w) or ops.hooks_wanted(lin_b)) and not missing
@@ -282,7 +288,10 @@
                 ops.grad_done(lin_b)
         keep = (ctx.ws, ctx.prep, ctx.planes, m, b, g)
         if defer:
-            ops._deferred.append((torch.cuda.current_stream(dev), side, keep))
+            main = torch.cuda.current_stream(dev)
+            ops._deferred.append((main, side, keep))
+            if aux is not None:
+                ops._deferred.append((main, aux, keep))
         ctx.ws = None
         return (None, None, None) + tuple(fresh)
 
```

Result: no change. 388,800 triples/s, median of 6 (+0.6%).
